# GinZhu/RDST

Hardware: AMD Instinct MI355X
Metric: SR patches/sec fwd+bwd, RDST-E1 x4 64->256 (higher is better)
Workload: dtype bf16; 1 GPU; RDST-E1 x4 (RDST_E1_OASIS_example_SRx4.ini), 1x64x64 LR patches -> 256x256, step = fwd + L1 + bwd + flat-bucket grad all-reduce + Adam; global_batch=32, per_gpu_batch=32, parallelism=dp1, hip_graph=True, grad_bucket_bytes=17859844

## Files before the change

rdst_amd/_lib.py:

```python
from __future__ import annotations

import ctypes as C
import os
import re

_HERE = os.path.dirname(os.path.abspath(__file__))
LIB_PATH = os.environ.get("RDST_HIP_LIB") or os.path.join(_HERE, "librdst_hip.so")
_INCLUDE = os.path.join(os.path.dirname(_HERE), "include")
HEADER_PATH = os.path.join(_INCLUDE, "rdst_hip.h")
_SIDE_HEADERS = {"DATA": os.path.join(_INCLUDE, "rdst_hip_data.h"),
                 "LRC": os.path.join(_INCLUDE, "rdst_hip_consistency.h"),
                 "MSSSIM": os.path.join(_INCLUDE, "rdst_hip_msssim.h"),
                 "NOISE": os.path.join(_INCLUDE, "rdst_hip_noise.h")}

_SCALARS = {"int": C.c_int, "int64_t": C.c_int64, "float": C.c_float, "double": C.c_double, "size_t": C.c_size_t}
_FIELD_SCALARS = {**_SCALARS, "int32_t": C.c_int32}
_RETURNS = {"int": C.c_int, "size_t": C.c_size_t, "const char*": C.c_char_p}
_POINTEES = {*_FIELD_SCALARS, "void", "char", "uint8_t", "unsigned long long"}


def _ctype(text, scalars, structs, where):
    ty = re.sub(r"\s*\*", "*", " ".join(text.split()))
    if ty == "int*":
        return C.POINTER(C.c_int)
    if ty.endswith("*") and ty[:-1].removeprefix("const ") in _POINTEES | set(structs):
        return C.c_void_p
    if ty in scalars or ty in structs:
        return scalars.get(ty) or structs[ty]
    raise RuntimeError(f"rdst_amd: include/rdst_hip.h: type '{ty}' is not in the binding's type map, in: {where}")


def _struct(name, body, structs):
    fields = []
    for stmt in filter(None, (" ".join(s.split()) for s in body.split(";"))):
        first, *more = (d.strip() for d in stmt.split(","))
        m = re.fullmatch(r"(.+?)\s*\b(\w+)\s*(?:\[\s*(\d+)\s*\])?", first)
        rest = [re.fullmatch(r"()(\w+)\s*(?:\[\s*(\d+)\s*\])?", d) for d in more]
        if m is None or None in rest or (more and "*" in m[1]):
            raise RuntimeError(f"rdst_amd: include/rdst_hip.h: cannot read the field '{stmt}' of struct {name}")
        base = _ctype(m[1], _FIELD_SCALARS, structs, f"struct {name} {{ {stmt}; }}")
        fields += [(d[2], base * int(d[3]) if d[3] else base) for d in (m, *rest)]
    return type(name, (C.Structure,), {"_fields_": fields})


def parse_header(text):
    text = re.sub(r"/\*.*?\*/|//[^\n]*", " ", text, flags=re.S)
    constants, lines = {}, []
    for line in text.splitlines():
        if not line.lstrip().startswith("#"):
            lines.append(line)
        elif m := re.fullmatch(r"\s*#\s*define\s+RDST_(\w+)\s+(\d+|\(\s*-\s*\d+\s*\))\s*", line):
            constants[m[1]] = int(re.sub(r"[()\s]", "", m[2]))
    body = re.sub(r'extern\s+"C"\s*\{(.*)\}', r"\1", "\n".join(lines), flags=re.S)
    structs = {}

    def cut(m):
        structs[m[2]] = _struct(m[2], m[1], structs)
        return ""
    body = re.sub(r"typedef\s+struct\s*\w*\s*\{(.*?)\}\s*(\w+)\s*;", cut, body, flags=re.S)
    signatures, params = {}, {}
    for decl in filter(None, (" ".join(d.split()) for d in body.split(";"))):
        m = re.fullmatch(r"(.+?)\s*\b(\w+)\s*\((.*)\)", decl)
        if m is None:
            raise RuntimeError(f"rdst_amd: include/rdst_hip.h: not a function declaration: {decl}")
        ret = re.sub(r"\s*\*", "*", m[1])
        if ret not in _RETURNS:
            raise RuntimeError(f"rdst_amd: include/rdst_hip.h: return type '{ret}' is not in the binding's type map, in: {decl}")
        args = [] if m[3].strip() in ("", "void") else [re.fullmatch(r"(.+?)\s*\b(\w+)", a.strip()) for a in m[3].split(",")]
        if None in args:
            raise RuntimeError(f"rdst_amd: include/rdst_hip.h: a parameter without a name, in: {decl}")
        signatures[m[2]] = (_RETURNS[ret], [_ctype(a[1], _SCALARS, structs, decl) for a in args])
        params[m[2]] = tuple(a[2] for a in args)
    return signatures, params, structs, constants


def _read_header(path=None):
    path = path or HEADER_PATH
    if not os.path.exists(path):
        raise RuntimeError(f"rdst_amd: {path} is missing. The ctypes binding is derived from it "
                           "(it ships beside the package, as in the repository); there is no second copy.")
    with open(path) as f:
        return f.read()


SIGNATURES, PARAMS, _structs, CONSTANTS = parse_header(_read_header())

_BOUND, _side_constants = dict(SIGNATURES), {}
for _prefix, _path in _SIDE_HEADERS.items():
    _sigs, _params, _, _consts = parse_header(_read_header(_path))
    globals().update({_prefix + "_HEADER_PATH": _path, _prefix + "_SIGNATURES": _sigs, _prefix + "_PARAMS": _params})
    _BOUND.update(_sigs)
    _side_constants.update(_consts)
NOISE_HETERO, NOISE_RICIAN = _side_constants["NOISE_HETERO"], _side_constants["NOISE_RICIAN"]

PackJob = _structs["rdst_pack_job"]
LrSchedule = _structs["rdst_lr_schedule"]
# ... 58 lines not shown
```

rdst_amd/build.py:

```python
from __future__ import annotations

import os
import subprocess
import sys
from concurrent.futures import ThreadPoolExecutor

HERE = os.path.dirname(os.path.abspath(__file__))
CSRC = os.path.join(HERE, "csrc")
OBJ = os.path.join(HERE, "csrc", "_obj")
LIB = os.path.join(HERE, "librdst_hip.so")
HIPCC = os.environ.get("HIPCC", "/opt/rocm/bin/hipcc")
FLAGS = ["--offload-arch=gfx950", "-O3", "-std=c++17", "-fPIC", "-Wno-unused-value", "-Wno-unused-result"]



def _newer(src_list, target):
    if not os.path.exists(target):
        return True
    t = os.path.getmtime(target)
    return any(os.path.getmtime(s) > t for s in src_list)


def build(force: bool = False, verbose: bool = True, debug: bool = False) -> str:
    OBJ = os.path.join(HERE, "csrc", "_obj_dbg" if debug else "_obj")
    LIB = os.path.join(HERE, "librdst_hip_dbg.so" if debug else "librdst_hip.so")
    FLAGS = globals()["FLAGS"] + (["-DRDST_DEBUG"] if debug else [])
    os.makedirs(OBJ, exist_ok=True)
    srcs = sorted(f for f in os.listdir(CSRC) if f.endswith(".hip"))
    hdrs = [os.path.join(CSRC, f) for f in os.listdir(CSRC) if f.endswith(".h")]
    hdrs += [os.path.join(os.path.dirname(HERE), "include", h) for h in ("rdst_hip.h", "rdst_hip_data.h", "rdst_hip_consistency.h",
                                                                            "rdst_hip_msssim.h", "rdst_hip_noise.h")]
    jobs = []
    objs = []
    for s in srcs:
        src = os.path.join(CSRC, s)
        obj = os.path.join(OBJ, s[:-4] + ".o")
        objs.append(obj)
        if force or _newer([src] + hdrs, obj):
            jobs.append([HIPCC, *FLAGS, "-c", src, "-o", obj])

    def run(cmd):
        if verbose:
            print("[rdst_amd.build]", " ".join(cmd[-4:]), flush=True)
        r = subprocess.run(cmd, capture_output=True, text=True)
        if r.returncode != 0:
            raise RuntimeError(f"hipcc failed: {' '.join(cmd)}\n{r.stdout}\n{r.stderr}")

    if jobs:
        with ThreadPoolExecutor(max_workers=min(4, len(jobs))) as ex:
            list(ex.map(run, jobs))
    if jobs or force or _newer(objs, LIB):
        run([HIPCC, "--offload-arch=gfx950", "-shared", "-fPIC", "-o", LIB, *objs])
    return LIB


if __name__ == "__main__":
    print(build(force="--force" in sys.argv, debug="--debug" in sys.argv))
```

rdst_amd/csrc/linear.h:

```cpp
#pragma once
#include "common.h"

template <typename T>
int linear_fwd_mfma(const T* X, int64_t ldx, const float* ln_w, const float* ln_b, int in_act, const float* Wt,
                    const float* bias, const T* R, int64_t ldr, T* Y, int64_t ldy, float* stats, int64_t M, int K,
                    int N, float s, bool split, hipStream_t st);
template <typename T>
int linear_dgrad_mfma(const T* X, int64_t ldx, bool has_ln, int in_act, const float* Wt, const T* dY, int64_t lddy,
                      T* dX, int64_t lddx, const T* acc, int64_t ldacc, float* dA, int64_t M, int K, int N, float s,
                      bool split, hipStream_t st);
template <typename T>
int linear_wgrad_mfma(const T* X, int64_t ldx, const float* ln_w, const float* ln_b, const float* stats, int in_act,
                      const T* dY, int64_t lddy, float* dW, float* dbias, const WsSlab& slab, int64_t M, int K, int N, float s,
                      bool split, hipStream_t st);

constexpr int kLinWgradSplits = 96;
inline int linear_wgrad_max_wgs(int N) { return N <= 128 ? 4 * kCUs : N <= 192 ? 2 * kCUs : kCUs; }
struct LinBwdWs {
  float* dA;
  float* G;
  WsSlab slabW;
  WsSlab small;
  size_t bytes;
};
inline LinBwdWs lin_bwd_layout(void* base, int64_t M, int K, int N, bool ln, bool linear) {
  WsCarver c(base);
  LinBwdWs w{};
  const size_t g = (size_t)N * (K + 1), da = ln ? (size_t)M * K : 0;
  w.dA = c.take<float>(da);
  w.G = ln && linear && g <= da ? w.dA : nullptr;
  const int64_t rows = linear ? linear_wgrad_max_wgs(N) : 0;
  const size_t gen = linear ? (size_t)kLinWgradSplits * N * K : 0, per_wg = (size_t)rows * g;
  w.slabW = WsSlab{c.take<float>(gen > per_wg ? gen : per_wg), rows, (int64_t)g};
  w.small = ws_take_slab(c, kSmallBlocks, N > 2 * K ? N : 2 * K);
  c.take<float>(2 * (size_t)K + kWsSlackFloats);
  w.bytes = c.bytes();
  return w;
}

template <typename T>
int linear_dgrad_ln_mfma(const T* X, int64_t ldx, const float* stats, const float* gamma, const float* Wt, const T* dY,
                         int64_t lddy, T* dX, int64_t lddx, const T* acc, int64_t ldacc, const WsSlab& slab, int* nslab,
                         int64_t M, int K, int N, float s, hipStream_t st);
template <typename T>
int linear_wgrad_ln_mfma(const T* X, int64_t ldx, const float* ln_w, const float* ln_b, const float* stats, const float* Wt,
                         const T* dY, int64_t lddy, float* dW, float* dbias, float* dln_w, float* dln_b, const WsSlab& slab,
                         float* G, int64_t M, int K, int N, float s, bool split, hipStream_t st);
template <typename T>
int linear_dgrad_ln2_mfma(const T* X, int64_t ldx, const float* stats, const float* gamma, const float* Wt, const T* dY,
                          int64_t lddy, T* dX, int64_t lddx, const T* acc, int64_t ldacc, int64_t M, int K, int N, float s,
                          bool split, hipStream_t st);
int wgrad_ln_finish_launch(const float* G, const float* Wt, const float* ln_w, const float* ln_b, int N, int K, float s,
                           float* dW, float* dbias, float* dln_w, float* dln_b, hipStream_t st);
int wgrad_sum_launch(const float* slab, int nwg, int tot, float* G, hipStream_t st);
int wgrad_reduce_launch(const float* slab, int nwg, int N, int K, float s, float* dW, float* dbias, hipStream_t st);
int linear_ln_bwd_fused_bf16(const bf16* X, int64_t ldx, const float* ln_w, const float* ln_b, const float* stats,
                             const float* Wt, const bf16* dY, int64_t lddy, bf16* dX, int64_t lddx, const bf16* acc,
                             int64_t ldacc, float* dW, float* dbias, float* dln_w, float* dln_b, const WsSlab& slab, float* G,
                             int64_t M, int K, int N, float s, hipStream_t st, const bf16* acc2 = nullptr, int64_t ldacc2 = 0);
int lnlin3_bwd_bf16(const bf16* X, int64_t ldx, const float* ln_w, const float* stats, const float* Wt, const bf16* dY,
                    int64_t lddy, bf16* dX, int64_t lddx, const bf16* acc, int64_t ldacc, const bf16* acc2, int64_t ldacc2,
                    const WsSlab& slab, int64_t slab_stride, int64_t M, int K, int N, int* grid_out, hipStream_t st);

size_t lin3_pack_bytes(int K, int N);
int lin3_kind(int K, int N, bool ln, bool res, int in_act);
int lin3_fwd_bf16(const bf16* X, int64_t ldx, const float* ln_w, const float* ln_b, int in_act, const float* Wt, const float* bias,
                  const bf16* R, int64_t ldr, bf16* Y, int64_t ldy, float* stats, int64_t M, int K, int N, float s, void* wpack,
                  bool prepacked, hipStream_t st);
int lin3_pack_launch(const float* W, const float* gamma, const float* beta, const float* bias, void* out, int N, int K, float s,
                     hipStream_t st);
size_t mlp3_pack_bytes(int C, int hid);
bool mlp3_fwd_shape(int C, int hid);
int mlp3_fwd_bf16(const bf16* X, int64_t ldx, const float* ln_w, const float* ln_b, const float* W1, const float* b1, const float* W2,
                  const float* b2, bf16* Y, int64_t ldy, float* stats, int64_t M, int C, int hid, void* wpack, bool prepacked,
                  hipStream_t st);

int lin3x_kind(int K, int N, bool ln, bool res, int in_act);
int lin3x_fwd_f32(const float* X, int64_t ldx, const float* ln_w, const float* ln_b, int in_act, const float* Wt, const float* bias,
                  const float* R, int64_t ldr, float* Y, int64_t ldy, float* stats, int64_t M, int K, int N, float s, void* wpack,
                  bool prepacked, hipStream_t st);
int lin3x_pack_launch(const float* W, const float* gamma, const float* beta, const float* bias, void* out, int N, int K, float s,
                      hipStream_t st);
int lnlin3x_bwd_kind(int K, int N, bool ln, int in_act);
int lnlin3x_bwd_f32(const float* X, int64_t ldx, const float* ln_w, const float* ln_b, const float* stats, int in_act, const float* Wt,
                    const float* dY, int64_t lddy, float* dX, int64_t lddx, const float* acc, int64_t ldacc, const float* acc2,
                    int64_t ldacc2, float* dW, float* dbias, float* dln_w, float* dln_b, const WsSlab& slab, float* G, int64_t M, int K, int N,
                    float s, hipStream_t st);
```

rdst_amd/csrc/linear.hip:

```cpp
#include "common.h"
#include "gemm_valu.h"
#include "linear.h"
#include "pack.h"

__global__ void __launch_bounds__(256) slab_reduce_kernel(const float* __restrict__ slab, float* __restrict__ out,
                                                          int S, int64_t n) {
  __shared__ float part[16][17];
  const int o = threadIdx.x & 15, sg = threadIdx.x >> 4;
  const int64_t i = (int64_t)blockIdx.x * 16 + o;
  float a = 0.f;
  if (i < n)
    for (int s = sg; s < S; s += 16) a += slab[(int64_t)s * n + i];
  part[sg][o] = a;
  __syncthreads();
  if (sg == 0 && i < n) {
    float t = 0.f;
#pragma unroll
    for (int k = 0; k < 16; ++k) t += part[k][o];
    out[i] = t;
  }
}

int slab_reduce(const float* slab, float* out, int S, int64_t n, hipStream_t st) {
  if (n <= 0) return 0;
  hipLaunchKernelGGL(slab_reduce_kernel, dim3((unsigned)((n + 15) / 16)), dim3(256), 0, st, slab, out, S, n);
  return rdst_launch_status("slab_reduce");
}

__global__ void __launch_bounds__(256) slab_reduce2_kernel(const float* __restrict__ slab, float* __restrict__ out_a,
                                                           float* __restrict__ out_b, int S, int K) {
  const int lane = threadIdx.x & 63;
  const int i = blockIdx.x * 4 + (threadIdx.x >> 6);
  if (i >= 2 * K) return;
  float a = 0.f;
  for (int s = lane; s < S; s += 64) a += slab[(int64_t)s * 2 * K + i];
  a = wave_sum(a);
  if (lane == 0) {
    if (i < K) { if (out_a) out_a[i] = a; }
    else if (out_b) out_b[i - K] = a;
  }
}

int slab_reduce2(const float* slab, float* out_a, float* out_b, int S, int K, hipStream_t st) {
  if (K <= 0 || (!out_a && !out_b)) return 0;
  hipLaunchKernelGGL(slab_reduce2_kernel, dim3((unsigned)((2 * K + 3) / 4)), dim3(256), 0, st, slab, out_a, out_b, S, K);
  return rdst_launch_status("slab_reduce2");
}

namespace {

constexpr float kLnEps = 1e-5f;

template <typename T>
__global__ void __launch_bounds__(256) row_stats_kernel(const T* __restrict__ X, int64_t ldx, float* __restrict__ stats,
                                                        int64_t M, int K) {
  const int lane = threadIdx.x & 63;
  const int64_t row = (int64_t)blockIdx.x * 4 + (threadIdx.x >> 6);
  if (row >= M) return;
  const T* x = X + row * ldx;
  float s = 0.f;
  for (int k = lane; k < K; k += 64) s += to_f32<T>(x[k]);
  const float mean = wave_sum(s) / (float)K;
  float v = 0.f;
  for (int k = lane; k < K; k += 64) {
    const float d = to_f32<T>(x[k]) - mean;
    v = fmaf(d, d, v);
  }
  const float var = wave_sum(v) / (float)K;
  if (lane == 0) {
    stats[row * 2] = mean;
    stats[row * 2 + 1] = 1.0f / sqrtf(var + kLnEps);
  }
}

template <typename T>
__global__ void __launch_bounds__(256) ln_apply_kernel(const T* __restrict__ X, int64_t ldx, const float* __restrict__ stats,
                                                       const float* __restrict__ g, const float* __restrict__ b,
                                                       const T* R, int64_t ldr, T* Y, int64_t ldy, int64_t M, int K,
                                                       float s) {
  const int64_t i = (int64_t)blockIdx.x * 256 + threadIdx.x;
  if (i >= M * K) return;
  const int64_t m = i / K;
  const int k = (int)(i - m * K);
  float v = (to_f32<T>(X[m * ldx + k]) - stats[2 * m]) * stats[2 * m + 1] * g[k] + b[k];
  v *= s;
  if (R) v += to_f32<T>(R[m * ldr + k]);
// ... 27 lines not shown
}
struct Ln8Lane { int c0, lo; bool on; };
__device__ __forceinline__ Ln8Lane ln8_lane(int grp, int K) {
  Ln8Lane l;
  l.on = 8 * grp < K;
  l.c0 = 8 * grp + 8 <= K ? 8 * grp : K - 8;
  l.lo = 8 * grp - l.c0;
  if (!l.on) { l.c0 = 0; l.lo = 8; }
  return l;
}
__device__ __forceinline__ void ln8_store(float* dst, const float (&o)[8], const Ln8Lane& l) {
  if (!l.on) return;
  if (l.lo == 0) {
    ln8_u32x4 u, v;
    u.x = __float_as_uint(o[0]); u.y = __float_as_uint(o[1]); u.z = __float_as_uint(o[2]); u.w = __float_as_uint(o[3]);
    v.x = __float_as_uint(o[4]); v.y = __float_as_uint(o[5]); v.z = __float_as_uint(o[6]); v.w = __float_as_uint(o[7]);
    *reinterpret_cast<ln8_u32x4*>(dst + l.c0) = u;
    *reinterpret_cast<ln8_u32x4*>(dst + l.c0 + 4) = v;
  } else {
#pragma unroll
    for (int e = 0; e < 8; ++e)
      if (e >= l.lo) dst[l.c0 + e] = o[e];
  }
}
__device__ __forceinline__ void ln8_store(bf16* dst, const float (&o)[8], const Ln8Lane& l) {
  if (!l.on) return;
  if (l.lo == 0) {
    ln8_u32x4 u;
    u.x = ln8_pack2(o[0], o[1]); u.y = ln8_pack2(o[2], o[3]); u.z = ln8_pack2(o[4], o[5]); u.w = ln8_pack2(o[6], o[7]);
    *reinterpret_cast<ln8_u32x4*>(dst + l.c0) = u;
  } else {
#pragma unroll
    for (int e = 0; e < 8; ++e)
      if (e >= l.lo) dst[l.c0 + e] = __float2bfloat16(o[e]);
  }
}

template <typename T>
__global__ void __launch_bounds__(256) ln8_fwd_kernel(const T* __restrict__ X, int64_t ldx, const float* __restrict__ g,
                                                      const float* __restrict__ b, const T* R, int64_t ldr, T* Y, int64_t ldy,
                                                      float* __restrict__ stats, int64_t M, int K, float s) {
  const int lane = threadIdx.x & 63, wave = threadIdx.x >> 6, ps = lane >> 3, grp = lane & 7;
  const Ln8Lane l = ln8_lane(grp, K);
  float gm[8], bt[8];
#pragma unroll
  for (int e = 0; e < 8; ++e) { gm[e] = g[l.c0 + e]; bt[e] = b[l.c0 + e]; }
  const float invK = 1.0f / (float)K;
  for (int64_t r0 = ((int64_t)blockIdx.x * 4 + wave) * 8; r0 < M; r0 += (int64_t)gridDim.x * 32) {
    const int64_t row = r0 + ps < M ? r0 + ps : M - 1;
    const bool valid = r0 + ps < M;
    float f[8];
    ln8_load<T>(X + row * ldx + l.c0, f);
    float sum = 0.f;
#pragma unroll
    for (int e = 0; e < 8; ++e) sum += (l.on && e >= l.lo) ? f[e] : 0.f;
    const float mean = ln8_sum8(sum) * invK;
    float sq = 0.f;
#pragma unroll
    for (int e = 0; e < 8; ++e) {
      f[e] -= mean;
      sq = (l.on && e >= l.lo) ? fmaf(f[e], f[e], sq) : sq;
    }
    const float rstd = 1.0f / sqrtf(ln8_sum8(sq) * invK + kLnEps);
    float o[8];
#pragma unroll
    for (int e = 0; e < 8; ++e) o[e] = (f[e] * rstd * gm[e] + bt[e]) * s;
    if (R) {
      float rr[8];
      ln8_load<T>(R + row * ldr + l.c0, rr);
#pragma unroll
      for (int e = 0; e < 8; ++e) o[e] += rr[e];
    }
    if (valid) {
      ln8_store(Y + row * ldy, o, l);
      if (grp == 0) *reinterpret_cast<float2*>(stats + 2 * row) = make_float2(mean, rstd);
    }
  }
}

template <typename T>
__global__ void __launch_bounds__(256) ln8_bwd_kernel(const T* __restrict__ dY, int64_t lddy, const T* __restrict__ X, int64_t ldx,
                                                      const float* __restrict__ stats, const float* __restrict__ gamma, T* dX,
                                                      int64_t lddx, const T* acc, int64_t ldacc, float* __restrict__ slab, int64_t M,
                                                      int K, float s) {
  __shared__ float red[4][2][64];
  const int lane = threadIdx.x & 63, wave = threadIdx.x >> 6, ps = lane >> 3, grp = lane & 7;
  const Ln8Lane l = ln8_lane(grp, K);
  float gm[8], dg[8], db[8];
#pragma unroll
  for (int e = 0; e < 8; ++e) { gm[e] = gamma[l.c0 + e]; dg[e] = 0.f; db[e] = 0.f; }
  const float invK = 1.0f / (float)K;
  for (int64_t r0 = ((int64_t)blockIdx.x * 4 + wave) * 8; r0 < M; r0 += (int64_t)gridDim.x * 32) {
    const int64_t row = r0 + ps < M ? r0 + ps : M - 1;
    const bool valid = r0 + ps < M;
    const float2 st = *reinterpret_cast<const float2*>(stats + 2 * row);
    float da[8], xh[8], gg[8];
    ln8_load<T>(dY + row * lddy + l.c0, da);
    ln8_load<T>(X + row * ldx + l.c0, xh);
    float s1 = 0.f, s2 = 0.f;
#pragma unroll
    for (int e = 0; e < 8; ++e) {
      const bool mine = l.on && e >= l.lo && valid;
      da[e] = mine ? da[e] * s : 0.f;
      xh[e] = (xh[e] - st.x) * st.y;
      gg[e] = da[e] * gm[e];
      s1 += gg[e];
      s2 = fmaf(gg[e], xh[e], s2);
      dg[e] = fmaf(da[e], xh[e], dg[e]);
      db[e] += da[e];
    }
    s1 = ln8_sum8(s1) * invK;
    s2 = ln8_sum8(s2) * invK;
    if (dX && valid) {
      float o[8];
#pragma unroll
      for (int e = 0; e < 8; ++e) o[e] = st.y * (gg[e] - s1 - xh[e] * s2);
      if (acc) {
        float a[8];
        ln8_load<T>(acc + row * ldacc + l.c0, a);
#pragma unroll
        for (int e = 0; e < 8; ++e) o[e] += a[e];
      }
      ln8_store(dX + row * lddx, o, l);
    }
  }
#pragma unroll
  for (int e = 0; e < 8; ++e) {
    dg[e] += __shfl_xor(dg[e], 8, 64); dg[e] += __shfl_xor(dg[e], 16, 64); dg[e] += __shfl_xor(dg[e], 32, 64);
    db[e] += __shfl_xor(db[e], 8, 64); db[e] += __shfl_xor(db[e], 16, 64); db[e] += __shfl_xor(db[e], 32, 64);
  }
  if (ps == 0 && l.on)
#pragma unroll
    for (int e = 0; e < 8; ++e)
      if (e >= l.lo) { red[wave][0][l.c0 + e] = dg[e]; red[wave][1][l.c0 + e] = db[e]; }
  __syncthreads();
  for (int i = threadIdx.x; i < 2 * K; i += 256) {
    const int which = i / K, k = i - which * K;
    slab[(int64_t)blockIdx.x * 2 * K + i] = red[0][which][k] + red[1][which][k] + red[2][which][k] + red[3][which][k];
  }
}
static inline bool ln8_ok(const void* a, int64_t lda, const void* b, int64_t ldb, const void* c, int64_t ldc, int K, int elt = 2) {
  auto al = [elt](const void* q, int64_t l) { return ((uintptr_t)q & 3) == 0 && (elt == 4 || (l & 1) == 0); };
  return K >= 8 && K <= 64 && (K & 1) == 0 && al(a, lda) && al(b, ldb) && al(c, ldc);
}

template <typename T>
struct LinIn {
  static constexpr bool kFast = true;
  const T* X; int64_t ldx; const float* stats; const float* g; const float* b; int act;
  __device__ __forceinline__ float operator()(int64_t m, int64_t k) const {
    float v = to_f32<T>(X[m * ldx + k]);
    if (g) return (v - stats[2 * m]) * stats[2 * m + 1] * g[k] + b[k];
    return apply_act(v, act);
  }
};
template <typename T>
struct LinInT {
  static constexpr bool kFast = false;
  LinIn<T> f;
  __device__ __forceinline__ float operator()(int64_t m, int k) const { return f(m, k); }
};
struct WtB {
  static constexpr bool kFast = true;
  const float* Wt; int K;
  __device__ __forceinline__ float operator()(int64_t k, int n) const { return Wt[(int64_t)n * K + k]; }
};
struct WtBT {
  static constexpr bool kFast = false;
  const float* Wt; int K;
  __device__ __forceinline__ float operator()(int64_t n_idx, int k_idx) const { return Wt[n_idx * K + k_idx]; }
};
template <typename T>
struct DyA {
  static constexpr bool kFast = true;
  const T* dY; int64_t ld; float s;
  __device__ __forceinline__ float operator()(int64_t m, int64_t n) const { return to_f32<T>(dY[m * ld + n]) * s; }
};
template <typename T>
struct DyAT {
  static constexpr bool kFast = false;
  const T* dY; int64_t ld; float s;
  __device__ __forceinline__ float operator()(int64_t n, int64_t m) const { return to_f32<T>(dY[m * ld + n]) * s; }
};
template <typename T>
struct DyCol {
  const T* dY; int64_t ld; float s;
  __device__ __forceinline__ float operator()(int64_t m, int n) const { return to_f32<T>(dY[m * ld + n]) * s; }
};

template <typename T>
struct FwdEp {
  const float* bias; const T* R; int64_t ldr; T* Y; int64_t ldy; float s;
  __device__ __forceinline__ void operator()(int64_t m, int n, float acc, int) const {
    float v = acc + (bias ? bias[n] : 0.f);
    v *= s;
    if (R) v += to_f32<T>(R[m * ldr + n]);
    Y[m * ldy + n] = from_f32<T>(v);
  }
};
struct SlabEp {
  float* slab; int64_t n_total; int cols;
  __device__ __forceinline__ void operator()(int64_t r, int c, float acc, int z) const {
    slab[(int64_t)z * n_total + r * cols + c] = acc;
  }
// ... 32 lines not shown
  const float invK = 1.0f / (float)K;
  for (int64_t row = (int64_t)blockIdx.x * 4 + wave; row < M; row += (int64_t)gridDim.x * 4) {
    const float mean = stats[2 * row], rstd = stats[2 * row + 1];
    float xh[KC], g[KC];
    float s1 = 0.f, s2 = 0.f;
#pragma unroll
    for (int c = 0; c < KC; ++c) {
      const int k = lane + 64 * c;
      if (k < K) {
        const float da = dA[row * K + k];
        xh[c] = (to_f32<T>(X[row * ldx + k]) - mean) * rstd;
        g[c] = da * gm[c];
        s1 += g[c];
        s2 = fmaf(g[c], xh[c], s2);
        dg[c] = fmaf(da, xh[c], dg[c]);
        db[c] += da;
      } else {
        xh[c] = 0.f;
        g[c] = 0.f;
      }
    }
    s1 = wave_sum(s1) * invK;
    s2 = wave_sum(s2) * invK;
#pragma unroll
    for (int c = 0; c < KC; ++c) {
      const int k = lane + 64 * c;
      if (k < K) {
        float v = rstd * (g[c] - s1 - xh[c] * s2);
        if (dX) {
          if (acc) v += to_f32<T>(acc[row * ldacc + k]);
          dX[row * lddx + k] = from_f32<T>(v);
        }
      }
    }
  }
#pragma unroll
  for (int c = 0; c < KC; ++c) {
    red[wave][0][lane + 64 * c] = dg[c];
    red[wave][1][lane + 64 * c] = db[c];
  }
  __syncthreads();
  for (int i = threadIdx.x; i < 2 * K; i += 256) {
    const int which = i / K, k = i - which * K;
    const float a = red[0][which][k] + red[1][which][k] + red[2][which][k] + red[3][which][k];
    slab[(int64_t)blockIdx.x * 2 * K + i] = a;
  }
}

template <typename T>
int fwd_t(const T* X, int64_t ldx, const float* ln_w, const float* ln_b, int in_act, const float* Wt, const float* bias,
          const T* R, int64_t ldr, T* Y, int64_t ldy, float* stats, int64_t M, int K, int N, float s, bool split, hipStream_t st) {
  auto run_stats = [&]() -> int {
    hipLaunchKernelGGL((row_stats_kernel<T>), dim3((unsigned)((M + 3) / 4)), dim3(256), 0, st, X, ldx, stats, M, K);
    return rdst_launch_status("row_stats");
  };
  if (!Wt) {
    if (ln8_ok(X, ldx, Y, ldy, R, ldr, K, (int)sizeof(T))) {
      const int64_t nb = (M + 31) / 32;
      hipLaunchKernelGGL((ln8_fwd_kernel<T>), dim3((unsigned)(nb < 2048 ? nb : 2048)), dim3(256), 0, st, X, ldx, ln_w, ln_b, R, ldr, Y, ldy,
                         stats, M, K, s);
      return rdst_launch_status("ln8_fwd");
    }
    if (int rc = run_stats()) return rc;
    const int64_t n = M * K;
    hipLaunchKernelGGL((ln_apply_kernel<T>), dim3((unsigned)((n + 255) / 256)), dim3(256), 0, st, X, ldx, stats, ln_w,
                       ln_b, R, ldr, Y, ldy, M, K, s);
    return rdst_launch_status("ln_apply");
  }
  if (int rc = linear_fwd_mfma<T>(X, ldx, ln_w, ln_b, in_act, Wt, bias, R, ldr, Y, ldy, stats, M, K, N, s, split, st);
      rc != RDST_ENOTSUP)
    return rc;
  if (ln_w)
    if (int rc = run_stats()) return rc;
  LinIn<T> la{X, ldx, stats, ln_w, ln_b, in_act};
  WtB lb{Wt, K};
  FwdEp<T> ep{bias, R, ldr, Y, ldy, s};
  return gemm_valu_launch(la, lb, ep, M, N, K, 1, st, "linear_fwd");
}

template <typename T>
int bwd_t(const T* X, int64_t ldx, const float* ln_w, const float* ln_b, const float* stats, int in_act, const float* Wt,
          const T* dY, int64_t lddy, T* dX, int64_t lddx, const T* acc, int64_t ldacc, float* dW, float* dbias,
          float* dln_w,
          float* dln_b, float* wsp, int64_t M, int K, int N, float s, bool split, hipStream_t st, const T* acc2, int64_t ldacc2) {
  const LinBwdWs w = lin_bwd_layout(wsp, M, K, N, ln_w != nullptr, true);
  float* const dA = w.dA;
  const WsSlab& slabW = w.slabW;
  const WsSlab& small = w.small;
  if constexpr (sizeof(T) == 4) {
    if (split && Wt && dX && dW && dbias && (!ln_w || (dln_w && dln_b && w.G)) && !rdst_dbg_getenv("RDST_LBX_OFF")) {
      const int rc = lnlin3x_bwd_f32(X, ldx, ln_w, ln_b, stats, in_act, Wt, dY, lddy, dX, lddx, acc, ldacc, acc2, ldacc2, dW, dbias, dln_w,
                                     dln_b, slabW, w.G, M, K, N, s, st);
      if (rc != RDST_ENOTSUP) return rc;
    }
  }
  if (acc2) {
    if constexpr (sizeof(T) == 2) {
      if (Wt && ln_w && ln_b && dW && dbias && dln_w && dln_b && dX && K <= 128 && w.G)
        return linear_ln_bwd_fused_bf16(X, ldx, ln_w, ln_b, stats, Wt, dY, lddy, dX, lddx, acc, ldacc, dW, dbias, dln_w, dln_b, slabW,
                                        w.G, M, K, N, s, st, acc2, ldacc2);
    }
    return RDST_ENOTSUP;
  }
  LinIn<T> fin{X, ldx, stats, ln_w, ln_b, in_act};
  if (Wt) {
    if (ln_w && ln_b && dW && dbias && dln_w && dln_b && dX && K <= 128 && !rdst_dbg_getenv("RDST_LN_BWD_V1")) {
      if (float* G = w.G) {
        if constexpr (sizeof(T) == 2) {
          const int rcf = linear_ln_bwd_fused_bf16(X, ldx, ln_w, ln_b, stats, Wt, dY, lddy, dX, lddx, acc, ldacc, dW, dbias, dln_w,
                                                   dln_b, slabW, G, M, K, N, s, st);
          if (rcf != RDST_ENOTSUP) return rcf;
        }
        int rc = linear_wgrad_ln_mfma<T>(X, ldx, ln_w, ln_b, stats, Wt, dY, lddy, dW, dbias, dln_w, dln_b, slabW, G, M, K, N,
                                         s, split, st);
        if (rc == 0) {
          rc = linear_dgrad_ln2_mfma<T>(X, ldx, stats, ln_w, Wt, dY, lddy, dX, lddx, acc, ldacc, M, K, N, s, split, st);
          if (rc == 0) return 0;
          if (rc != RDST_ENOTSUP) return rc;
          if (N >= 64) {
            const int N1 = (N / 2 + 3) / 4 * 4;
            rc = linear_dgrad_ln2_mfma<T>(X, ldx, stats, ln_w, Wt, dY, lddy, dX, lddx, acc, ldacc, M, K, N1, s, split, st);
            if (rc == 0) {
              rc = linear_dgrad_ln2_mfma<T>(X, ldx, stats, ln_w, Wt + (int64_t)N1 * K, dY + N1, lddy, dX, lddx, dX, lddx, M, K, N - N1, s, split, st);
              if (rc != RDST_ENOTSUP) return rc;
            } else if (rc != RDST_ENOTSUP) {
              return rc;
            }
          }
          dW = nullptr; dbias = nullptr; dln_w = nullptr; dln_b = nullptr;
        } else if (rc != RDST_ENOTSUP) {
          return rc;
        }
      }
    }
    if constexpr (sizeof(T) == 2) {
      if (!ln_w && !in_act && dW && dbias && dX) {
        const int rcf = linear_ln_bwd_fused_bf16(X, ldx, nullptr, nullptr, nullptr, Wt, dY, lddy, dX, lddx, acc, ldacc, dW, dbias,
                                                 nullptr, nullptr, slabW, nullptr, M, K, N, s, st);
        if (rcf != RDST_ENOTSUP) return rcf;
      }
    }
    bool wgrad_done = false;
    if (dW || dbias) {
      const int rc = linear_wgrad_mfma<T>(X, ldx, ln_w, ln_b, stats, in_act, dY, lddy, dW, dbias, slabW, M, K, N, s, split, st);
      if (rc == 0) wgrad_done = true;
      else if (rc != RDST_ENOTSUP) return rc;
    }
    if (!wgrad_done && dbias) {
      DyCol<T> f{dY, lddy, s};
      if (int rc = colsum_launch(f, M, N, small, dbias, st, "linear_dbias")) return rc;
    }
    if (!wgrad_done && dW) {
      DyAT<T> la{dY, lddy, s};
      LinInT<T> lb{fin};
      SlabEp ep{slabW.p, (int64_t)N * K, K};
      const int z = gemm_valu_splits(M, kLinWgradSplits);
      if (int rc2 = rdst_slab_fits(slabW, z, (int64_t)N * K, "linear_wgrad")) return rc2;
      if (int rc2 = gemm_valu_launch(la, lb, ep, N, K, M, kLinWgradSplits, st, "linear_wgrad")) return rc2;
      if (int rc2 = slab_reduce(slabW.p, dW, z, (int64_t)N * K, st)) return rc2;
    }
    if (dX && ln_w) {
      int nslab = 0;
      const int rc = linear_dgrad_ln_mfma<T>(X, ldx, stats, ln_w, Wt, dY, lddy, dX, lddx, acc, ldacc, small, &nslab, M, K,
                                             N, s, st);
      if (rc == 0) {
        return slab_reduce2(small.p, dln_w, dln_b, nslab, K, st);
      }
      if (rc != RDST_ENOTSUP) return rc;
    }
    if (dX || (ln_w && (dln_w || dln_b))) {
      int rc = linear_dgrad_mfma<T>(X, ldx, ln_w != nullptr, in_act, Wt, dY, lddy, dX, lddx, acc, ldacc, dA, M, K, N, s, split, st);
      if (rc == RDST_ENOTSUP) {
        DyA<T> la{dY, lddy, s};
        WtBT lb{Wt, K};
        if (ln_w) {
          DaEp ep{dA, K};
          rc = gemm_valu_launch(la, lb, ep, M, K, N, 1, st, "linear_dgrad");
        } else {
          DxEp<T> ep{X, ldx, dX, lddx, in_act, acc, ldacc};
          rc = gemm_valu_launch(la, lb, ep, M, K, N, 1, st, "linear_dgrad");
        }
      }
      if (rc) return rc;
    }
  }
  if (ln_w) {
    const float* dAsrc = dA;
    if (!dX && !dln_w && !dln_b) return 0;
    if (K > 512) return rdst_fail(RDST_ENOTSUP, "rdst_ln_linear_bwd: LayerNorm width %d > 512", K);
    const int blocks = (int)small.cap((M + 3) / 4 < kSmallBlocks ? (M + 3) / 4 : kSmallBlocks, 2 * K);
    if (int rc = rdst_slab_fits(small, blocks, 2 * K, "ln_bwd_rows")) return rc;
    const int kc = (K + 63) / 64;
#define RDST_LNB(KC)                                                                                              \
  hipLaunchKernelGGL((ln_bwd_rows_kernel<T, KC>), dim3(blocks), dim3(256), 0, st, dAsrc, X, ldx, stats, ln_w, dX, \
                     lddx, acc, ldacc, small.p, M, K)
    if (kc <= 1) RDST_LNB(1); else if (kc <= 2) RDST_LNB(2); else if (kc <= 4) RDST_LNB(4); else RDST_LNB(8);
#undef RDST_LNB
    if (int rc = rdst_launch_status("ln_bwd_rows")) return rc;
    if (int rc = slab_reduce2(small.p, dln_w, dln_b, blocks, K, st)) return rc;
  }
  return 0;
}

template <typename T>
__global__ void __launch_bounds__(256) scale_to_f32_kernel(const T* __restrict__ dY, int64_t ld, float* __restrict__ dA,
                                                           int64_t M, int K, float s) {
  const int64_t i = (int64_t)blockIdx.x * 256 + threadIdx.x;
  if (i >= M * K) return;
  const int64_t m = i / K;
  dA[i] = to_f32<T>(dY[m * ld + (i - m * K)]) * s;
}

template <typename T>
int ln_only_bwd(const T* X, int64_t ldx, const float* ln_w, const float* stats, const T* dY, int64_t lddy, T* dX,
                int64_t lddx, const T* acc, int64_t ldacc, float* dln_w, float* dln_b, float* wsp, int64_t M, int K, float s,
                hipStream_t st) {
  const LinBwdWs w = lin_bwd_layout(wsp, M, K, K, true, false);
  float* const dA = w.dA;
  const WsSlab& small = w.small;
  const int64_t n = M * K;
  if (K <= 64 && ln8_ok(X, ldx, dY, lddy, dX, lddx, K, (int)sizeof(T)) && ln8_ok(acc, ldacc, nullptr, 0, nullptr, 0, K, (int)sizeof(T))) {
    const int64_t nb = (M + 31) / 32;
    const int blocks = (int)small.cap(nb < kSmallBlocks ? nb : kSmallBlocks, 2 * K);
    if (int rc = rdst_slab_fits(small, blocks, 2 * K, "ln8_bwd")) return rc;
    hipLaunchKernelGGL((ln8_bwd_kernel<T>), dim3(blocks), dim3(256), 0, st, dY, lddy, X, ldx, stats, ln_w, dX, lddx, acc, ldacc, small.p, M, K, s);
    if (int rc = rdst_launch_status("ln8_bwd")) return rc;
    return slab_reduce2(small.p, dln_w, dln_b, blocks, K, st);
  }
  hipLaunchKernelGGL((scale_to_f32_kernel<T>), dim3((unsigned)((n + 255) / 256)), dim3(256), 0, st, dY, lddy, dA, M, K, s);
  if (int rc = rdst_launch_status("scale_to_f32")) return rc;
  if (K > 512) return rdst_fail(RDST_ENOTSUP, "rdst_ln_linear_bwd: LayerNorm width %d > 512", K);
  const int blocks = (int)small.cap((M + 3) / 4 < kSmallBlocks ? (M + 3) / 4 : kSmallBlocks, 2 * K);
  if (int rc = rdst_slab_fits(small, blocks, 2 * K, "ln_bwd_rows")) return rc;
  const int kc = (K + 63) / 64;
#define RDST_LNB(KC)                                                                                           \
  hipLaunchKernelGGL((ln_bwd_rows_kernel<T, KC>), dim3(blocks), dim3(256), 0, st, dA, X, ldx, stats, ln_w, dX, \
                     lddx, acc, ldacc, small.p, M, K)
  if (kc <= 1) RDST_LNB(1); else if (kc <= 2) RDST_LNB(2); else if (kc <= 4) RDST_LNB(4); else RDST_LNB(8);
#undef RDST_LNB
  if (int rc = rdst_launch_status("ln_bwd_rows")) return rc;
  return slab_reduce2(small.p, dln_w, dln_b, blocks, K, st);
}

}

extern "C" int rdst_ln_linear_fwd_packable(int K, int N, int has_ln, int has_residual, int in_act, int dtype) {
  bool split;
  if (rdst_dtype(dtype, split, "rdst_ln_linear_fwd_packable")) return 0;
  if (split) return lin3x_kind(K, N, has_ln != 0, has_residual != 0, in_act) != 0;
  return dtype == RDST_BF16 && lin3_kind(K, N, has_ln != 0, has_residual != 0, in_act) != 0;
}

extern "C" size_t rdst_ln_linear_fwd_workspace(int K, int N) {
  if (K <= 0 || N <= 0) return 16;
  return lin3_pack_bytes(K, N);
}

extern "C" size_t rdst_ln_linear_fwd_workspace2(int K, int N, int dtype) {
  if (K <= 0 || N <= 0) return 16;
  return dtype == RDST_F32X3 ? lin3x_pack_bytes(K, N) : lin3_pack_bytes(K, N);
}

extern "C" int rdst_ln_linear_fwd(const void* X, int64_t ld_x, const float* ln_w, const float* ln_b, int in_act,
                                  const float* Wt, const float* bias, const void* R, int64_t ld_r, void* Y, int64_t ld_y,
                                  float* stats, void* workspace, size_t workspace_bytes, int64_t M, int K, int N,
                                  float out_scale, int dtype, void* stream) {
  bool split;
  if (int rc = rdst_dtype(dtype, split, "rdst_ln_linear_fwd")) return rc;
  if (!X || !Y) return rdst_fail(RDST_EINVAL, "rdst_ln_linear_fwd: null pointer");
  if (M < 0 || K <= 0 || N <= 0) return rdst_fail(RDST_EINVAL, "rdst_ln_linear_fwd: bad dimensions");
  if ((ln_w == nullptr) != (ln_b == nullptr)) return rdst_fail(RDST_EINVAL, "rdst_ln_linear_fwd: ln_w/ln_b must come together");
  if (ln_w && !stats) return rdst_fail(RDST_EINVAL, "rdst_ln_linear_fwd: LayerNorm needs a stats buffer");
  if (ln_w && in_act) return rdst_fail(RDST_EINVAL, "rdst_ln_linear_fwd: LayerNorm and in_act are exclusive");
  if (!Wt && (!ln_w || N != K)) return rdst_fail(RDST_EINVAL, "rdst_ln_linear_fwd: Wt == NULL means LayerNorm only (N == K)");
  if (ld_x < K || ld_y < N || (R && ld_r < N)) return rdst_fail(RDST_EINVAL, "rdst_ln_linear_fwd: leading dimension too small");
  if (M == 0) return 0;
  hipStream_t st = (hipStream_t)stream;
  if (dtype == RDST_BF16 && workspace && workspace_bytes >= rdst_ln_linear_fwd_workspace(K, N)) {
    const int rc = lin3_fwd_bf16((const bf16*)X, ld_x, ln_w, ln_b, in_act, Wt, bias, (const bf16*)R, ld_r, (bf16*)Y, ld_y, stats, M,
                                 K, N, out_scale, workspace, workspace_bytes == RDST_PREPACKED, st);
    if (rc != RDST_ENOTSUP) return rc;
  }
  if (split && workspace && workspace_bytes >= lin3x_pack_bytes(K, N)) {
    const int rc = lin3x_fwd_f32((const float*)X, ld_x, ln_w, ln_b, in_act, Wt, bias, (const float*)R, ld_r, (float*)Y, ld_y, stats, M,
                                 K, N, out_scale, workspace, workspace_bytes == RDST_PREPACKED, st);
    if (rc != RDST_ENOTSUP) return rc;
  }
  if (dtype == RDST_F32)
    return fwd_t<float>((const float*)X, ld_x, ln_w, ln_b, in_act, Wt, bias, (const float*)R, ld_r, (float*)Y, ld_y, stats, M, K, N, out_scale, split, st);
  return fwd_t<bf16>((const bf16*)X, ld_x, ln_w, ln_b, in_act, Wt, bias, (const bf16*)R, ld_r, (bf16*)Y, ld_y, stats, M, K, N, out_scale, false, st);
}

extern "C" size_t rdst_ln_linear_bwd_workspace(int64_t M, int K, int N) {
  if (M <= 0 || K <= 0 || N <= 0) return 0;
  return lin_bwd_layout(nullptr, M, K, N, true, true).bytes;
}

namespace {
int ln_linear_bwd(const void* X, int64_t ld_x, const float* ln_w, const float* ln_b, const float* stats, int in_act, const float* Wt,
                  const void* dY, int64_t ld_dy, void* dX, int64_t ld_dx, const void* dX_add, int64_t ld_dx_add, float* dW, float* dbias,
                  float* dln_w, float* dln_b, void* workspace, size_t workspace_bytes, int64_t M, int K, int N, float out_scale,
                  int dtype, bool split, hipStream_t st, const void* dX_add2, int64_t ld_dx_add2) {
  if (!X || !dY || !workspace) return rdst_fail(RDST_EINVAL, "rdst_ln_linear_bwd: null pointer");
  if (M < 0 || K <= 0 || N <= 0) return rdst_fail(RDST_EINVAL, "rdst_ln_linear_bwd: bad dimensions");
  if (ln_w && !stats) return rdst_fail(RDST_EINVAL, "rdst_ln_linear_bwd: LayerNorm needs the forward's stats");
  if (!Wt && (!ln_w || N != K)) return rdst_fail(RDST_EINVAL, "rdst_ln_linear_bwd: Wt == NULL means LayerNorm only (N == K)");
  if (ld_x < K || ld_dy < N || (dX && ld_dx < K)) return rdst_fail(RDST_EINVAL, "rdst_ln_linear_bwd: leading dimension too small");
  if (workspace_bytes < rdst_ln_linear_bwd_workspace(M, K, N)) return rdst_fail(RDST_EINVAL, "rdst_ln_linear_bwd: workspace too small");
  if (M == 0) return 0;
  float* wsp = (float*)workspace;
  if (dX_add2 && (!Wt || (dtype != RDST_BF16 && !(split && lnlin3x_bwd_kind(K, N, ln_w != nullptr, in_act))))) return RDST_ENOTSUP;
  if (!Wt) {
    if (dtype == RDST_F32)
      return ln_only_bwd<float>((const float*)X, ld_x, ln_w, stats, (const float*)dY, ld_dy, (float*)dX, ld_dx, (const float*)dX_add, ld_dx_add, dln_w, dln_b, wsp, M, K, out_scale, st);
    return ln_only_bwd<bf16>((const bf16*)X, ld_x, ln_w, stats, (const bf16*)dY, ld_dy, (bf16*)dX, ld_dx, (const bf16*)dX_add, ld_dx_add, dln_w, dln_b, wsp, M, K, out_scale, st);
  }
  if (dtype == RDST_F32)
    return bwd_t<float>((const float*)X, ld_x, ln_w, ln_b, stats, in_act, Wt, (const float*)dY, ld_dy, (float*)dX, ld_dx, (const float*)dX_add, ld_dx_add, dW, dbias, dln_w, dln_b, wsp, M, K, N, out_scale, split, st,
                      (const float*)dX_add2, ld_dx_add2);
  return bwd_t<bf16>((const bf16*)X, ld_x, ln_w, ln_b, stats, in_act, Wt, (const bf16*)dY, ld_dy, (bf16*)dX, ld_dx, (const bf16*)dX_add, ld_dx_add, dW, dbias, dln_w, dln_b, wsp, M, K, N, out_scale, false, st,
                     (const bf16*)dX_add2, ld_dx_add2);
}
}

extern "C" int rdst_ln_linear_bwd2(const void* X, int64_t ld_x, const float* ln_w, const float* ln_b, const float* stats,
                                  int in_act, const float* Wt, const void* dY, int64_t ld_dy, void* dX, int64_t ld_dx,
                                  const void* dX_add, int64_t ld_dx_add, float* dW, float* dbias, float* dln_w, float* dln_b,
                                  void* workspace,
                                  size_t workspace_bytes, int64_t M, int K, int N, float out_scale, int dtype,
                                  void* stream, const void* dX_add2, int64_t ld_dx_add2) {
  bool split;
  if (int rc = rdst_dtype(dtype, split, "rdst_ln_linear_bwd")) return rc;
  return ln_linear_bwd(X, ld_x, ln_w, ln_b, stats, in_act, Wt, dY, ld_dy, dX, ld_dx, dX_add, ld_dx_add, dW, dbias, dln_w, dln_b, workspace,
                       workspace_bytes, M, K, N, out_scale, dtype, split, (hipStream_t)stream, dX_add2, ld_dx_add2);
}

extern "C" int rdst_ln_linear_bwd(const void* X, int64_t ld_x, const float* ln_w, const float* ln_b, const float* stats,
                                  int in_act, const float* Wt, const void* dY, int64_t ld_dy, void* dX, int64_t ld_dx,
                                  const void* dX_add, int64_t ld_dx_add, float* dW, float* dbias, float* dln_w, float* dln_b,
                                  void* workspace, size_t workspace_bytes, int64_t M, int K, int N, float out_scale, int dtype,
                                  void* stream) {
  bool split;
  if (int rc = rdst_dtype(dtype, split, "rdst_ln_linear_bwd")) return rc;
  return ln_linear_bwd(X, ld_x, ln_w, ln_b, stats, in_act, Wt, dY, ld_dy, dX, ld_dx, dX_add, ld_dx_add, dW, dbias, dln_w, dln_b, workspace,
                       workspace_bytes, M, K, N, out_scale, dtype, split, (hipStream_t)stream, nullptr, 0);
}
```

rdst_amd/csrc/lnlin3_mfma.hip:

```cpp
#include "linear.h"
#include "lds_dma.h"
#include "mfma.h"
#include "wattn_hd.h"
#include <stdlib.h>

#ifndef LB3_LOADW_SHAPE
#define LB3_LOADW_SHAPE(K, N) (((K) == 60 && (N) == 180) || ((K) == 90 && (N) == 270) || ((K) == 120 && (N) == 120))
#endif
#ifndef LB3_ABL
#define LB3_ABL 0
#endif

#ifdef LB3_STAMPS
constexpr bool LB3_TICKS = true;
#else
constexpr bool LB3_TICKS = false;
#endif
constexpr const char* LB3_LEGEND = "stash fetch barrier compute finish - - -";

namespace {
using namespace wahd;
using MM = Mma<bf16>;

struct LB3Args {
  const bf16* X; int64_t ldx; const float* stats; const float* lnw; const float* W;
  const bf16* dY; int64_t lddy; bf16* dX; int64_t lddx; const bf16* Acc; int64_t ldacc;
  const bf16* Acc2; int64_t ldacc2;
  float* slab; int64_t slab_stride;
  int64_t M; int64_t ntiles; int tiles_per_wg;
};

template <int K_, int N_>
struct LB3 {
  static constexpr int K = K_, N = N_;
  static constexpr int NCT = (K + 1 + 31) / 32, NW = (N + 31) / 32, KN = (N + 15) / 16;
  static constexpr bool WIDE = N >= 180;
  static constexpr int TN = WIDE ? 3 : 1;
  static constexpr int TC = (K == 120 && N == 360) ? 2 : WIDE ? 1 : NCT;
  static_assert(NW % TN == 0 && NCT % TC == 0, "blocking");
  static constexpr int NGN = NW / TN, NGC = NCT / TC, NWG = NGN * NGC;
  static constexpr int NDG = NCT;
  static constexpr int NWV = NWG + NDG, NT = 64 * NWV;
  static constexpr int PKX = (K * 2 + 15) / 16, PKY = (N * 2 + 15) / 16;
  static constexpr int NY = 32 * PKY, NX = 32 * PKX;
  static constexpr bool LOADW = LB3_LOADW_SHAPE(K_, N_);
  static constexpr bool SPLITR = WIDE || LOADW;
  static constexpr int NTW = SPLITR ? 64 * NWG : NT, NTD = SPLITR ? 64 * NDG : NT;
  static constexpr int cdiv(int a, int b) { return (a + b - 1) / b; }
  static constexpr bool ACC_BY_W = K == 120 && N == 360;
  static constexpr int W_SY = cdiv(NY, NTW), W_SX = cdiv(NX, NTW), W_SA = (WIDE && !ACC_BY_W && !LOADW) ? 0 : cdiv(NX, NTW);
  static constexpr int D_SY = SPLITR ? 0 : W_SY, D_SX = SPLITR ? 0 : W_SX, D_SA = (ACC_BY_W || LOADW) ? 0 : cdiv(NX, NTD);
  static constexpr int CP = 32 * NCT;
  static constexpr int LDX = NCT == 4 ? 336 : CP * 2 + 16;
  static constexpr int LDY = lds_plane_stride(32 * NW);
  static constexpr int OFF_AC = 32 * LDX, OFF_DY = 64 * LDX, OFF_SM = OFF_DY + 32 * LDY, BUF = OFF_SM + 128;
  static constexpr int OFF_RED = 2 * BUF;
  static constexpr int SMEM = OFF_RED + 2 * NCT * 256;
  static constexpr int PERCU0 = 12 / NWV < 1 ? 1 : 12 / NWV;
  static constexpr int PERCU1 = WIDE ? 1 : PERCU0 > 2 ? 2 : PERCU0;
  static constexpr int PERCU = PERCU1 * SMEM > 160 * 1024 ? 1 : PERCU1;
  static constexpr int WPS = (NWV * PERCU + 3) / 4;
};

template <class CF, bool LN, int SY, int SX, int SA>
struct LB3Loader {
  static constexpr int NS = SY + SX + SA;
  int meta[NS > 0 ? NS : 1];
  u32x4_a4 rd[NS > 0 ? NS : 1];
  u32x4_a4 rd2[SA > 0 ? SA : 1];
  float2 rst[SX > 0 ? SX : 1];
  static __device__ __forceinline__ int kind(int u) { return u < SY ? 0 : u < SY + SX ? 1 : 2; }
  __device__ __forceinline__ void setup(int tid_r, int ntr, bool has_acc) {
#pragma unroll
    for (int u = 0; u < NS; ++u) {
      const int kd = kind(u);
      const int idx = tid_r + ntr * (kd == 0 ? u : kd == 1 ? u - SY : u - SY - SX);
      const int per = kd == 0 ? CF::PKY : CF::PKX, rowbytes = kd == 0 ? CF::N * 2 : CF::K * 2;
      const bool on = idx < 32 * per && (kd != 2 || has_acc);
      const int row = on ? idx / per : 0, chk = on ? idx - row * per : 0;
      int o = chk * 16;
      if (o + 16 > rowbytes) o = rowbytes - 16;
      meta[u] = o | (row << 16) | ((on ? 1 : 0) << 24) | (((o & 15) == 0 ? 1 : 0) << 28);
    }
  }
  __device__ __forceinline__ void fetch(const LB3Args& p, int64_t tile) {
    const uint32_t Mu = (uint32_t)p.M;
#pragma unroll
    for (int u = 0; u < NS; ++u) {
      const int kd = kind(u);
      uint32_t row = (uint32_t)(tile * 32) + (uint32_t)((meta[u] >> 16) & 31);
      row = row < Mu ? row : Mu - 1;
      const char* base = reinterpret_cast<const char*>(kd == 0 ? p.dY : kd == 1 ? p.X : (p.Acc ? p.Acc : p.X));
      const uint32_t ldb = (uint32_t)((kd == 0 ? p.lddy : kd == 1 ? p.ldx : p.ldacc) * 2);
      rd[u] = *reinterpret_cast<const u32x4_a4*>(base + (size_t)(row * ldb + (uint32_t)(meta[u] & 0xffff)));
      if (kd == 2 && p.Acc2)
        rd2[u - SY - SX] = *reinterpret_cast<const u32x4_a4*>(reinterpret_cast<const char*>(p.Acc2) +
                                                              (size_t)(row * (uint32_t)(p.ldacc2 * 2) + (uint32_t)(meta[u] & 0xffff)));
      if (LN && kd == 1) rst[u - SY] = *reinterpret_cast<const float2*>(p.stats + 2 * (size_t)row);
    }
  }
  __device__ __forceinline__ void stash(const LB3Args& p, int64_t tile, char* buf) {
    const uint32_t Mu = (uint32_t)p.M;
#pragma unroll
    for (int u = 0; u < NS; ++u) {
      const int kd = kind(u);
      if (!((meta[u] >> 24) & 1)) continue;
      const int mrow = (meta[u] >> 16) & 31;
      const bool valid = (uint32_t)(tile * 32) + (uint32_t)mrow < Mu;
      Pack16 v;
      v.w[0] = valid ? rd[u].x : 0u; v.w[1] = valid ? rd[u].y : 0u; v.w[2] = valid ? rd[u].z : 0u; v.w[3] = valid ? rd[u].w : 0u;
      if (kd == 2 && p.Acc2) {
        const u32x4_a4 a = rd[u], b2 = rd2[u - SY - SX];
        const bool h1 = p.Acc != nullptr;
        float f[8];
        f[0] = bf16lo(b2.x) + (h1 ? bf16lo(a.x) : 0.f); f[1] = bf16hi(b2.x) + (h1 ? bf16hi(a.x) : 0.f);
        f[2] = bf16lo(b2.y) + (h1 ? bf16lo(a.y) : 0.f); f[3] = bf16hi(b2.y) + (h1 ? bf16hi(a.y) : 0.f);
        f[4] = bf16lo(b2.z) + (h1 ? bf16lo(a.z) : 0.f); f[5] = bf16hi(b2.z) + (h1 ? bf16hi(a.z) : 0.f);
        f[6] = bf16lo(b2.w) + (h1 ? bf16lo(a.w) : 0.f); f[7] = bf16hi(b2.w) + (h1 ? bf16hi(a.w) : 0.f);
#pragma unroll
        for (int e = 0; e < 8; ++e) f[e] = valid ? f[e] : 0.f;
        v = MM::pack(f);
      }
      if (LN && kd == 1) {
        const float2 st2 = rst[u - SY];
        float f[8];
        f[0] = bf16lo(rd[u].x); f[1] = bf16hi(rd[u].x); f[2] = bf16lo(rd[u].y); f[3] = bf16hi(rd[u].y);
        f[4] = bf16lo(rd[u].z); f[5] = bf16hi(rd[u].z); f[6] = bf16lo(rd[u].w); f[7] = bf16hi(rd[u].w);
#pragma unroll
        for (int e = 0; e < 8; ++e) f[e] = valid ? (f[e] - st2.x) * st2.y : 0.f;
        v = MM::pack(f);
        if ((meta[u] & 0xffff) == 0) reinterpret_cast<float*>(buf + CF::OFF_SM)[mrow] = st2.y;
      }
      int mt = meta[u];
      asm volatile("" : "+v"(mt));
      const int lrow = (mt >> 16) & 31, lo = mt & 0xffff;
      char* dst = buf + (kd == 0 ? CF::OFF_DY + lrow * CF::LDY : (kd == 2 ? CF::OFF_AC : 0) + lrow * CF::LDX) + lo;
      if ((meta[u] >> 28) & 1) *reinterpret_cast<Pack16*>(dst) = v;
      else {
        uint32_t* d = reinterpret_cast<uint32_t*>(dst);
        d[0] = v.w[0]; d[1] = v.w[1]; d[2] = v.w[2]; d[3] = v.w[3];
      }
    }
  }
};

template <int K, int N, bool LN>
__global__ void __launch_bounds__((LB3<K, N>::NT), (LB3<K, N>::WPS)) lnlin3_bwd_kernel(const LB3Args p) {
  extern __shared__ __attribute__((aligned(16))) char smem[];
  using CF = LB3<K, N>;
  constexpr int NCT = CF::NCT, NW = CF::NW, KN = CF::KN, TN = CF::TN, TC = CF::TC, NGC = CF::NGC, NWG = CF::NWG, NT = CF::NT;
  constexpr int LDX = CF::LDX, LDY = CF::LDY;
  const int tid = threadIdx.x, lane = tid & 63, wave = __builtin_amdgcn_readfirstlane(tid >> 6), r = lane & 31, hh = lane >> 5;
  const bool has_acc = p.Acc != nullptr || p.Acc2 != nullptr;

  if (!(LB3_ABL & 16)) lds_zero16(smem, CF::SMEM, tid, NT);
  __syncthreads();
  if (tid < 64) *reinterpret_cast<uint16_t*>(smem + (tid >> 5) * CF::BUF + (tid & 31) * LDX + K * 2) = 0x3f80;

  const int q = (lane & 15) >> 2, pp = lane & 3, gq1 = (lane >> 4) & 1;
  const int trc = (16 * gq1 + 4 * pp) * 2;
  const int tro_y = CF::OFF_DY + (8 * hh + q) * LDY + trc;
  const int tro_x = (8 * hh + q) * LDX + trc;

  const bool is_wg = wave < NWG;
  const int gn = wave / NGC, gc = wave - gn * NGC;
  const int dct = wave - NWG;

  const int64_t t0 = (int64_t)blockIdx.x * p.tiles_per_wg;
  const int64_t t1 = t0 + p.tiles_per_wg < p.ntiles ? t0 + p.tiles_per_wg : p.ntiles;
  __syncthreads();

  if (is_wg) {
    LB3Loader<CF, LN, CF::W_SY, CF::W_SX, CF::W_SA> ld;
    ld.setup(tid, CF::NTW, has_acc);
    if (t0 < t1) ld.fetch(p, t0);
    f32x16 G[TN][TC];
#pragma unroll
    for (int i = 0; i < TN; ++i)
#pragma unroll
      for (int j = 0; j < TC; ++j)
#pragma unroll
        for (int v = 0; v < 16; ++v) G[i][j][v] = 0.f;
    int b = 0;
    WaveTicks<LB3_TICKS> wt;
    for (int64_t tile = t0; tile < t1; ++tile, b ^= 1) {
      char* buf = smem + b * CF::BUF;
      ld.stash(p, tile, buf);
      wt.add(0);
      ld.fetch(p, tile + 1 < t1 ? tile + 1 : tile);
      wt.add(1);
      __syncthreads();
      wt.add(2);
#pragma unroll
      for (int s = 0; s < 2; ++s) {
        Pack16 ya[TN], xb[TC];
#pragma unroll
        for (int i = 0; i < TN; ++i) {
          const lds_cp yp = (lds_cp)(buf + tro_y + 16 * s * LDY) + (gn * TN + i) * 64;
          ya[i] = lds_tr_pack(yp, yp + 4 * LDY);
        }
#pragma unroll
        for (int j = 0; j < TC; ++j) {
          const lds_cp xp = (lds_cp)(buf + tro_x + 16 * s * LDX) + (gc * TC + j) * 64;
          xb[j] = lds_tr_pack(xp, xp + 4 * LDX);
        }
#pragma unroll
        for (int i = 0; i < TN; ++i)
#pragma unroll
          for (int j = 0; j < TC; ++j) {
#if !(LB3_ABL & 1)
            MM::mma(G[i][j], ya[i], xb[j]);
#else
            G[i][j][0] += __uint_as_float(ya[i].w[0] ^ xb[j].w[0]);
#endif
          }
      }
      wt.add(3);
    }
    wt.print(wave, lane, "wgrad", LB3_LEGEND);
    if (LN) __syncthreads();
    uint2* my = reinterpret_cast<uint2*>(p.slab) + (int64_t)blockIdx.x * p.slab_stride;
#pragma unroll
    for (int i = 0; i < TN; ++i)
#pragma unroll
      for (int j = 0; j < TC; ++j) {
        const int c = 32 * (gc * TC + j) + r;
#pragma unroll
        for (int g4 = 0; g4 < 4; ++g4) {
          const int n0 = 32 * (gn * TN + i) + 8 * g4 + 4 * hh;
          if (n0 < N && c <= K && !(LB3_ABL & 8))
            my[(int64_t)(n0 >> 2) * (K + 1) + c] =
                make_uint2(pack_bf16x2(G[i][j][4 * g4], G[i][j][4 * g4 + 1]), pack_bf16x2(G[i][j][4 * g4 + 2], G[i][j][4 * g4 + 3]));
        }
      }
    return;
  }

  LB3Loader<CF, LN, CF::D_SY, CF::D_SX, CF::D_SA> ld;
  ld.setup(CF::SPLITR ? tid - 64 * NWG : tid, CF::NTD, has_acc);
  if (t0 < t1) ld.fetch(p, t0);
  Pack16 wf[KN];
  {
    const int c = 32 * dct + r;
    const int cc = c < K ? c : K - 1;
    const float gm = (c < K) ? (LN ? p.lnw[cc] : 1.0f) : 0.f;
#pragma unroll
    for (int ks = 0; ks < KN; ++ks) {
      float f[8];
#pragma unroll
      for (int e = 0; e < 8; ++e) {
        const int n = 16 * ks + 8 * hh + e;
#if LB3_ABL & 4
        const float w = 0.01f * (float)(n + cc);
#else
        const float w = p.W[(size_t)(n < N ? n : N - 1) * K + cc];
#endif
        f[e] = n < N ? w * gm : 0.f;
      }
      wf[ks] = MM::pack(f);
    }
  }
  constexpr float invK = 1.0f / (float)K;
  float* red = reinterpret_cast<float*>(smem + CF::OFF_RED);
  f32x16 dx;
  u32x2_t xs[4], as[4];
  float rstd = 0.f;
  int64_t prow = -1;
  auto finish = [&](int pb) {
    float s1 = 0.f, s2 = 0.f;
    if (LN) {
#pragma unroll
      for (int w = 0; w < NCT; ++w) {
        const float2 v = *reinterpret_cast<const float2*>(red + ((pb * NCT + w) * 32 + r) * 2);
        s1 += v.x; s2 += v.y;
      }
      s1 *= invK; s2 *= invK;
    }
    float o[16];
#pragma unroll
    for (int g4 = 0; g4 < 4; ++g4) {
      const float xh[4] = {bf16lo(xs[g4].x), bf16hi(xs[g4].x), bf16lo(xs[g4].y), bf16hi(xs[g4].y)};
      const float ac[4] = {bf16lo(as[g4].x), bf16hi(as[g4].x), bf16lo(as[g4].y), bf16hi(as[g4].y)};
#pragma unroll
      for (int e = 0; e < 4; ++e) o[4 * g4 + e] = LN ? fmaf(rstd, dx[4 * g4 + e] - s1 - xh[e] * s2, ac[e]) : dx[4 * g4 + e] + ac[e];
    }
    if (prow < p.M) {
      bf16* drow = p.dX + prow * p.lddx;
#pragma unroll
      for (int gp2 = 0; gp2 < 2; ++gp2) {
        float c8[8];
#pragma unroll
        for (int e = 0; e < 4; ++e) {
          const auto sw = __builtin_amdgcn_permlane32_swap(__float_as_uint(o[8 * gp2 + e]), __float_as_uint(o[8 * gp2 + 4 + e]), false, false);
          c8[e] = __uint_as_float(sw[0]);
          c8[4 + e] = __uint_as_float(sw[1]);
        }
        const int cb = 32 * dct + 8 * (2 * gp2 + hh);
        if (cb + 8 <= K) {
          u32x4_a4 u;
          u.x = pack_bf16x2(c8[0], c8[1]); u.y = pack_bf16x2(c8[2], c8[3]);
          u.z = pack_bf16x2(c8[4], c8[5]); u.w = pack_bf16x2(c8[6], c8[7]);
          *reinterpret_cast<u32x4_a4*>(drow + cb) = u;
        } else {
#pragma unroll
          for (int e = 0; e < 8; ++e)
            if (cb + e < K) drow[cb + e] = __float2bfloat16(c8[e]);
        }
      }
    }
  };
  int b = 0;
  WaveTicks<LB3_TICKS> wt;
  for (int64_t tile = t0; tile < t1; ++tile, b ^= 1) {
    char* buf = smem + b * CF::BUF;
    ld.stash(p, tile, buf);
    wt.add(0);
    ld.fetch(p, tile + 1 < t1 ? tile + 1 : tile);
    wt.add(1);
    __syncthreads();
    wt.add(2);
    if (LN && prow >= 0) finish(b ^ 1);
    wt.add(4);
    const lds_cp yrow = (lds_cp)(buf + CF::OFF_DY + r * LDY + hh * 16);
#pragma unroll
    for (int v = 0; v < 16; ++v) dx[v] = 0.f;
    if constexpr (KN > 12) {
#pragma unroll
      for (int ks = 0; ks < KN; ++ks) {
#if !(LB3_ABL & 2)
        MM::mma(dx, wf[ks], lds_pack(yrow + 32 * ks));
#else
        dx[0] += __uint_as_float(lds_pack(yrow + 32 * ks).w[0]);
#endif
      }
    } else {
      f32x16 d2;
#pragma unroll
      for (int v = 0; v < 16; ++v) d2[v] = 0.f;
#pragma unroll
      for (int ks = 0; ks < KN; ++ks) {
        const Pack16 yb = lds_pack(yrow + 32 * ks);
        if (ks & 1) MM::mma(d2, wf[ks], yb);
        else MM::mma(dx, wf[ks], yb);
      }
#pragma unroll
      for (int v = 0; v < 16; ++v) dx[v] += d2[v];
    }
    const lds_cp xrow = (lds_cp)(buf + r * LDX) + (32 * dct + 4 * hh) * 2;
#pragma unroll
    for (int g4 = 0; g4 < 4; ++g4) {
      xs[g4] = *reinterpret_cast<const LDS_AS u32x2_t*>(xrow + 16 * g4);
      as[g4] = *reinterpret_cast<const LDS_AS u32x2_t*>(xrow + CF::OFF_AC + 16 * g4);
    }
    prow = tile * 32 + r;
    if (LN) {
      rstd = reinterpret_cast<const float*>(buf + CF::OFF_SM)[r];
      float s1 = 0.f, s2 = 0.f;
#pragma unroll
      for (int g4 = 0; g4 < 4; ++g4) {
        const float xh[4] = {bf16lo(xs[g4].x), bf16hi(xs[g4].x), bf16lo(xs[g4].y), bf16hi(xs[g4].y)};
#pragma unroll
        for (int e = 0; e < 4; ++e) {
          s1 += dx[4 * g4 + e];
          s2 = fmaf(dx[4 * g4 + e], xh[e], s2);
        }
      }
      s1 = half_swap_sum(s1);
      s2 = half_swap_sum(s2);
      if (hh == 0) *reinterpret_cast<float2*>(red + ((b * NCT + dct) * 32 + r) * 2) = make_float2(s1, s2);
    } else {
      wt.add(3);
      finish(b);
      wt.add(4);
    }
    wt.add(3);
  }
  wt.print(wave, lane, "dgrad", LB3_LEGEND);
  if (LN) {
    __syncthreads();
    if (prow >= 0) finish(b ^ 1);
  }
}

template <int K, int N, bool LN>
int lb3_launch(LB3Args& p, const WsSlab& slab, int* grid_out, hipStream_t st) {
  using CF = LB3<K, N>;
  auto kern = lnlin3_bwd_kernel<K, N, LN>;
  static int percu_env = -1;
  if (percu_env < 0) { const char* e = rdst_dbg_getenv("RDST_LB3_PERCU"); percu_env = e ? atoi(e) : 0; }
  int per_cu = CF::PERCU;
  if (percu_env > 0 && percu_env < per_cu) per_cu = percu_env;
  const int64_t grid = rdst_tile_grid(p.ntiles, slab.cap((int64_t)kCUs * per_cu, 2 * p.slab_stride), &p.tiles_per_wg);
  if (int rc = rdst_slab_fits(slab, grid, 2 * p.slab_stride, "lnlin3_bwd")) return rc;
  *grid_out = (int)grid;
  return rdst_launch(kern, dim3((unsigned)grid), dim3(CF::NT), CF::SMEM, st, "lnlin3_bwd", p);
}

}

int lnlin3_bwd_bf16(const bf16* X, int64_t ldx, const float* ln_w, const float* stats, const float* Wt, const bf16* dY,
                    int64_t lddy, bf16* dX, int64_t lddx, const bf16* acc, int64_t ldacc, const bf16* acc2, int64_t ldacc2,
                    const WsSlab& slab, int64_t slab_stride, int64_t M, int K, int N, int* grid_out, hipStream_t st) {
  static int off = -1;
  if (off < 0) { const char* e = rdst_dbg_getenv("RDST_LB3_OFF"); off = e ? atoi(e) : 0; }
  if (off) return RDST_ENOTSUP;
  const bool ln = ln_w != nullptr;
  LB3Args p{};
  p.X = X; p.ldx = ldx; p.stats = stats; p.lnw = ln_w; p.W = Wt; p.dY = dY; p.lddy = lddy; p.dX = dX; p.lddx = lddx;
  p.Acc = acc; p.ldacc = ldacc; p.Acc2 = acc2; p.ldacc2 = ldacc2; p.slab = slab.p; p.slab_stride = slab_stride; p.M = M;
  p.ntiles = (M + 31) / 32;
#define RDST_LB3(KK, NN, LL) if (K == KK && N == NN && ln == LL) return lb3_launch<KK, NN, LL>(p, slab, grid_out, st);
  RDST_LB3(60, 180, true) RDST_LB3(90, 270, true) RDST_LB3(120, 360, true)
  RDST_LB3(60, 30, true) RDST_LB3(90, 30, true) RDST_LB3(120, 30, true)
  RDST_LB3(60, 60, false) RDST_LB3(90, 90, false) RDST_LB3(120, 120, false)
#undef RDST_LB3
  return RDST_ENOTSUP;
}
```

rdst_amd/csrc/lnlin_mfma.hip:

```cpp
#include "linear.h"
#include "mfma.h"
#include "reduce_batch.h"
#include "wattn_hd.h"
#include <stdlib.h>

namespace {
using namespace wahd;
using MM = Mma<bf16>;

typedef __attribute__((address_space(1))) const char* gcp;
__device__ __forceinline__ u32x4_a4 gload16(gcp q) {
  const u32x4_a4 v = *reinterpret_cast<__attribute__((address_space(1))) const u32x4_a4*>(q);
  return v;
}
__device__ __forceinline__ float2 gload8(gcp q) {
  const float x = *reinterpret_cast<__attribute__((address_space(1))) const float*>(q);
  const float y = *reinterpret_cast<__attribute__((address_space(1))) const float*>(q + 4);
  return make_float2(x, y);
}

__host__ __device__ inline int lnlin_ldy(int NP) {
  const int b = NP * 2 + 16;
  return (b & 255) < 48 ? b + 64 : b;
}
// ... 236 lines not shown
      float s1 = 0.f, s2 = 0.f;
      if (LN) {
#pragma unroll
      for (int w = 0; w < NCT; ++w) {
        const float2 v = *reinterpret_cast<const float2*>(red + (w * 32 + r) * 2);
        s1 += v.x; s2 += v.y;
      }
      s1 *= invK; s2 *= invK;
      }
      float o[16];
#pragma unroll
      for (int g4 = 0; g4 < 4; ++g4) {
        const int cb = (32 * wave + 8 * g4 + 4 * hh) * 2;
        const u32x2_t xv = *reinterpret_cast<const LDS_AS u32x2_t*>((lds_cp)(smem + OFF_XH + r * LDX) + cb);
        const u32x2_t av = *reinterpret_cast<const LDS_AS u32x2_t*>((lds_cp)(smem + OFF_AC + r * LDX) + cb);
        const float xh[4] = {bf16lo(xv.x), bf16hi(xv.x), bf16lo(xv.y), bf16hi(xv.y)};
        const float ac[4] = {bf16lo(av.x), bf16hi(av.x), bf16lo(av.y), bf16hi(av.y)};
#pragma unroll
        for (int e = 0; e < 4; ++e) o[4 * g4 + e] = LN ? fmaf(rstd, dx[4 * g4 + e] - s1 - xh[e] * s2, ac[e]) : dx[4 * g4 + e] + ac[e];
      }
      const int64_t row = tile * 32 + r;
      if (row < p.M) {
        bf16* drow = p.dX + row * p.lddx;
#pragma unroll
        for (int gp2 = 0; gp2 < 2; ++gp2) {
          float c8[8];
#pragma unroll
          for (int e = 0; e < 4; ++e) {
            const auto sw = __builtin_amdgcn_permlane32_swap(__float_as_uint(o[8 * gp2 + e]), __float_as_uint(o[8 * gp2 + 4 + e]), false, false);
            c8[e] = __uint_as_float(sw[0]);
            c8[4 + e] = __uint_as_float(sw[1]);
          }
          const int cb = 32 * wave + 8 * (2 * gp2 + hh);
          if (cb + 8 <= K) {
            u32x4_a4 u;
            u.x = pack_bf16x2(c8[0], c8[1]); u.y = pack_bf16x2(c8[2], c8[3]);
            u.z = pack_bf16x2(c8[4], c8[5]); u.w = pack_bf16x2(c8[6], c8[7]);
            *reinterpret_cast<u32x4_a4*>(drow + cb) = u;
          } else {
#pragma unroll
            for (int e = 0; e < 8; ++e)
              if (cb + e < K) drow[cb + e] = __float2bfloat16(c8[e]);
          }
        }
      }
    }
    __syncthreads();
    stamp();
  }
  if (RDST_DBGV(p.stamps) && tid == 0) p.stamps[(size_t)blockIdx.x * 16 + 14] = __builtin_readcyclecounter();
  uint2* my = reinterpret_cast<uint2*>(p.slab) + (int64_t)blockIdx.x * p.slab_stride;
  if (wave < NW)
#pragma unroll
  for (int ct = 0; ct < NCT; ++ct) {
    const int c = 32 * ct + r;
#pragma unroll
    for (int g4 = 0; g4 < 4; ++g4) {
      const int n0 = 32 * wave + 8 * g4 + 4 * hh;
      if (n0 < N && c <= K)
        my[(int64_t)(n0 >> 2) * (K + 1) + c] = make_uint2(pack_bf16x2(G[ct][4 * g4], G[ct][4 * g4 + 1]), pack_bf16x2(G[ct][4 * g4 + 2], G[ct][4 * g4 + 3]));
    }
  }
  if (RDST_DBGV(p.stamps) && tid == 0) p.stamps[(size_t)blockIdx.x * 16 + 15] = __builtin_readcyclecounter();
}
}

static int lnlin_bwd_reduce(float* slab, int grid, int64_t slab_stride, bool ln, const float* Wt, const float* ln_w,
                            const float* ln_b, float* dW, float* dbias, float* dln_w, float* dln_b, float* G, int N, int K,
                            hipStream_t st) {
  rbatch::SumJob sj{};
  sj.slab = slab; sj.nwg = grid; sj.stride = slab_stride; sj.g4 = 1; sj.a2 = N; sj.b2 = K + 1; sj.tot = ((N + 3) / 4) * (K + 1);
  if (!ln) {
    sj.map = rbatch::MAP_LINEAR; sj.out = dW; sj.out2 = dbias; sj.a = K; sj.b = K + 1; sj.s = 1.0f;
    return rbatch::sum(sj, st);
  }
  sj.map = rbatch::MAP_COPY; sj.out = G;
  if (int rc = rbatch::sum(sj, st)) return rc;
  return wgrad_ln_finish_launch(G, Wt, ln_w, ln_b, N, K, 1.0f, dW, dbias, dln_w, dln_b, st);
}

int linear_ln_bwd_fused_bf16(const bf16* X, int64_t ldx, const float* ln_w, const float* ln_b, const float* stats,
                             const float* Wt, const bf16* dY, int64_t lddy, bf16* dX, int64_t lddx, const bf16* acc,
                             int64_t ldacc, float* dW, float* dbias, float* dln_w, float* dln_b, const WsSlab& slab, float* G,
                             int64_t M, int K, int N, float s, hipStream_t st, const bf16* acc2, int64_t ldacc2) {
  static int off = -1;
  if (off < 0) { const char* e = rdst_dbg_getenv("RDST_LNLIN_V1"); off = e ? atoi(e) : 0; }
  const bool ln = ln_w != nullptr;
  if (off == 1 || (off == 2 && !ln) || s != 1.0f || M <= 0) return RDST_ENOTSUP;
  const int nct = (K + 1 + 31) / 32;
  if (nct < 2 || nct > 4 || (K & 1) || K < 8 || (N & 1) || N < 8) return RDST_ENOTSUP;
  const int NW = (N + 31) / 32;
  if (NW > 12) return RDST_ENOTSUP;
  const int PK = 4 * nct, PKY = (N * 2 + 15) / 16;
  int NWV = NW > nct ? NW : nct;
  if (ln && NWV < 2 * nct) NWV = 2 * nct;
  const int NT = 64 * NWV;
  if (4 * NT < 32 * (PKY + PK * (acc ? 2 : 1))) return RDST_ENOTSUP;
  if (ln && (NT < 32 * PK || 2 * NT < 32 * PKY)) return RDST_ENOTSUP;
  if (((uintptr_t)X & 3) || ((uintptr_t)dY & 3) || ((uintptr_t)dX & 3) || ((uintptr_t)acc & 3) || (ldx & 1) || (lddy & 1) ||
      (lddx & 1) || (ldacc & 1))
    return RDST_ENOTSUP;
  if ((uint64_t)M * (uint64_t)(lddy > ldx ? (lddy > ldacc ? lddy : ldacc) : (ldx > ldacc ? ldx : ldacc)) * 2 >= (1ull << 31)) return RDST_ENOTSUP;
  const int64_t slab_stride = (int64_t)((N + 3) / 4) * (K + 1);
  {
    int g3 = 0;
    if (acc2 && (((uintptr_t)acc2 & 3) || (ldacc2 & 1) || (uint64_t)M * (uint64_t)ldacc2 * 2 >= (1ull << 31))) return RDST_ENOTSUP;
    const int rc3 = lnlin3_bwd_bf16(X, ldx, ln_w, stats, Wt, dY, lddy, dX, lddx, acc, ldacc, acc2, ldacc2, slab, slab_stride, M, K,
                                    N, &g3, st);
    if (rc3 == 0) return lnlin_bwd_reduce(slab.p, g3, slab_stride, ln, Wt, ln_w, ln_b, dW, dbias, dln_w, dln_b, G, N, K, st);
    if (rc3 != RDST_ENOTSUP || acc2) return rc3;
  }
  const int CP = 32 * nct, LDW = nct == 4 ? 288 : CP * 2 + 16, LDX = nct == 4 ? 336 : CP * 2 + 16, NP = 32 * NW, LDY = lnlin_ldy(NP);
  const int smem = NP * LDW + 2 * 32 * LDX + 32 * LDY + 128 + nct * 32 * 8;
  if (smem > 160 * 1024) return RDST_ENOTSUP;
  LnLinArgs p{};
  p.X = X; p.ldx = ldx; p.stats = stats; p.lnw = ln_w; p.W = Wt; p.dY = dY; p.lddy = lddy; p.dX = dX; p.lddx = lddx;
  p.Acc = acc; p.ldacc = ldacc; p.M = M; p.K = K; p.N = N; p.NW = NW; p.NWV = NWV;
  p.ntiles = (M + 31) / 32;
  int per_cu = ln ? 1 : 12 / NWV;
  if (per_cu > 160 * 1024 / smem) per_cu = 160 * 1024 / smem;
  if (per_cu < 1) per_cu = 1;
  if (per_cu > 2) per_cu = 2;
  { const char* e = rdst_dbg_getenv("RDST_LNLIN_PERCU"); if (e && atoi(e) > 0) per_cu = atoi(e); }
  p.slab = slab.p;
  p.slab_stride = slab_stride;
  const int64_t grid = rdst_tile_grid(p.ntiles, slab.cap((int64_t)kCUs * per_cu, 2 * slab_stride), &p.tiles_per_wg);
  if (int rc = rdst_slab_fits(slab, grid, 2 * slab_stride, "lnlin_bwd")) return rc;
  int rc = 0;
#define RDST_LNLIN(NC)                                                                                               \
  {                                                                                                                  \
    auto kern = ln ? lnlin_bwd_kernel<NC, true> : lnlin_bwd_kernel<NC, false>;                                       \
    rc = rdst_launch(kern, dim3((unsigned)grid), dim3(NT), smem, st, "lnlin_bwd", p);                                 \
  }
  p.stamps = rdst_stamps_begin("RDST_LNLIN_STAMPS", grid, 16, st);
  if (nct == 2) RDST_LNLIN(2) else if (nct == 3) RDST_LNLIN(3) else RDST_LNLIN(4)
#undef RDST_LNLIN
  rdst_stamps_end(p.stamps, grid, 16, RDST_STAMPS_TICKS, st, "lnlin_bwd K=%d N=%d ln=%d", K, N, (int)ln);
  if (rc) return rc;
  return lnlin_bwd_reduce(slab.p, (int)grid, p.slab_stride, ln, Wt, ln_w, ln_b, dW, dbias, dln_w, dln_b, G, N, K, st);
}
```

rdst_amd/networks/common.py:

```python
from __future__ import annotations

import math

import torch
from torch import nn

from .. import ops


class Conv2d(nn.Conv2d):

    def forward_rows(self, x, *, in_act=ops.ACT_NONE, residual=None, out_scale=1.0, shuffle=1, out_slot=None):
        k = self.kernel_size[0]
        if (self.kernel_size[0] != self.kernel_size[1] or k not in (1, 3) or self.stride != (1, 1)
                or self.padding != (k // 2, k // 2) or self.dilation != (1, 1) or self.groups != 1):
            raise NotImplementedError("rdst_amd Conv2d: only k in {1,3}, stride 1, padding k//2, groups 1")
        return ops.conv_rows(x, self.weight, self.bias, in_act=in_act, residual=residual, out_scale=out_scale,
                             shuffle=shuffle, out_slot=out_slot)

    def forward(self, x):
        return ops.rows_to_nchw(self.forward_rows(ops.nchw_to_rows(x, torch.float32)))


def default_conv(in_channels, out_channels, kernel_size, bias=True):
    return Conv2d(in_channels, out_channels, kernel_size, padding=(kernel_size // 2), bias=bias)


class UpSampler(nn.Sequential):

    def __init__(self, conv, scale, n_feats, bn=False, act=None, bias=True):
        if bn:
            raise NotImplementedError("rdst_amd UpSampler: BatchNorm is not on the RDST path (bn_in_conv = None)")
        m = []
        if (scale & (scale - 1)) == 0:
            for _ in range(int(math.log(scale, 2))):
                m.append(conv(n_feats, 4 * n_feats, 3, bias))
                m.append(nn.PixelShuffle(2))
                if act is not None:
                    m.append(act)
        elif scale == 3:
            m.append(conv(n_feats, 9 * n_feats, 3, bias))
            m.append(nn.PixelShuffle(3))
            if act is not None:
                m.append(act)
        else:
            raise NotImplementedError('SR scale {} is not valid.'.format(scale))
        super().__init__(*m)

    def forward_rows(self, x):
        mods = list(self)
        i = 0
        while i < len(mods):
            m = mods[i]
            if isinstance(m, Conv2d) and i + 1 < len(mods) and isinstance(mods[i + 1], nn.PixelShuffle):
                x = m.forward_rows(x, shuffle=mods[i + 1].upscale_factor)
                i += 2
            elif isinstance(m, Conv2d):
                x = m.forward_rows(x)
                i += 1
            else:
                raise NotImplementedError(f"rdst_amd UpSampler: {type(m).__name__} inside the upsampler")
        return x

    def forward(self, x):
        return ops.rows_to_nchw(self.forward_rows(ops.nchw_to_rows(x, torch.float32)))


class MeanShift(Conv2d):

    def __init__(self, mean=(0.,), std=(1.0,), mode='sub'):
        if len(mean) != len(std):
            raise ValueError('Size of means and stds should be the same')
        nc = len(mean)
        super().__init__(nc, nc, kernel_size=1)
        std = torch.Tensor(std)
        mean = torch.Tensor(mean)
        if mode == 'sub':
            self.weight.data = torch.eye(nc).view(nc, nc, 1, 1) / std.view(nc, 1, 1, 1)
            self.bias.data = -1 * mean / std
        elif mode == 'add':
            self.weight.data = torch.eye(nc).view(nc, nc, 1, 1) * std.view(nc, 1, 1, 1)
            self.bias.data = 1 * mean
        for p in self.parameters():
            p.requires_grad = False
```

rdst_amd/networks/rdst_variations.py:

```python
from __future__ import annotations

import torch
import torch.nn as nn

from .. import ops
from .common import Conv2d, MeanShift, UpSampler, default_conv
from .swin_transformer_sr import (BasicLayer, Mlp, PatchEmbed, PatchUnEmbed, SwinTransformerBlock,
                                  WindowAttention, _drop_p, _ln_params, _norm_only, trunc_normal_, window_partition,
                                  window_reverse)


def _dim_modifier(input_dim, growth_rate, norm_layer, pre_norm):
    if pre_norm:
        return nn.Sequential(norm_layer(input_dim), nn.Linear(input_dim, growth_rate))
    return nn.Sequential(nn.Linear(input_dim, growth_rate), norm_layer(growth_rate))


def _apply_dim_modifier(seq, x, out_scale=1.0, out_slot=None):
    if isinstance(seq, nn.Identity):
        if out_slot is not None:
            raise NotImplementedError("rdst_amd: dense slot behind an Identity tail")
        return x if out_scale == 1.0 else x * out_scale
    a, b = seq[0], seq[1]
    if isinstance(b, nn.Linear):
        w, bb = _ln_params(a)
        return ops.ln_linear(x, w, bb, b.weight, b.bias, out_scale=out_scale, out_slot=out_slot)
    y = ops.ln_linear(x, None, None, a.weight, a.bias)
    return _norm_only(y, b, out_scale=out_scale, out_slot=out_slot)


def _slot_ok(seq):
    if isinstance(seq, nn.Identity):
        return False
    b = seq[1]
    return isinstance(b, nn.Linear) or isinstance(b, nn.LayerNorm)


class DenseSTLayer(nn.Module):

    def __init__(self, input_dim, input_resolution, depth=2, num_heads=6, window_size=2,
                 mlp_ratio=4., qkv_bias=True, qk_scale=None, drop=0., attn_drop=0.,
                 drop_path=30., norm_layer=nn.LayerNorm, downsample=None, use_checkpoint=False,
                 growth_rate=60, dense_scale=1., dim_modify_mode='tail',
                 pre_norm=False):
        super().__init__()
        assert growth_rate % num_heads == 0, 'growth_rate % num_heads should be 0'
        assert input_dim % num_heads == 0, 'token dim % num_heads should be 0'
        if dim_modify_mode == 'head':
            self.head = (_dim_modifier(input_dim, growth_rate, norm_layer, pre_norm)
                         if input_dim != growth_rate else nn.Identity())
            hidden_dim = growth_rate
            self.tail = nn.Identity()
        elif dim_modify_mode == 'tail':
            self.head = nn.Identity()
            hidden_dim = input_dim
            self.tail = (_dim_modifier(hidden_dim, growth_rate, norm_layer, pre_norm)
                         if hidden_dim != growth_rate else nn.Identity())
        else:
            raise ValueError(f"dim_modify_mode {dim_modify_mode!r} (head or tail)")
        self.body = BasicLayer(hidden_dim, input_resolution, depth, num_heads, window_size, mlp_ratio, qkv_bias,
                               qk_scale, drop, attn_drop, drop_path, norm_layer, downsample, use_checkpoint)
        self.input_dim = input_dim
        self.hidden_dim = hidden_dim
        self.input_resolution = input_resolution
        self.dense_scale = dense_scale
        self.growth_rate = hidden_dim
        self.growth_rate_out = growth_rate
        self.depth = depth
        self.pre_norm = pre_norm

    def new_features(self, x, x_size, out_slot=None, sink=None):
        y = _apply_dim_modifier(self.head, x)
        y = self.body(y, x_size, sink=sink) if sink is not None else self.body(y, x_size)
        return _apply_dim_modifier(self.tail, y, out_scale=self.dense_scale, out_slot=out_slot)

    def _grad_sink(self, x):
        blocks = self.body.blocks
        if isinstance(self.head, nn.Identity) and len(blocks) > 0 and blocks[0].fuses_input_gradient() \
                and x.requires_grad and torch.is_grad_enabled():
            return ops.GradSink()
        return None

    def forward(self, x, x_size):
        return torch.cat((x, self.new_features(x, x_size)), 2)

    def forward_dense(self, x, x_size, buf):
        sink = self._grad_sink(x)
        if not _slot_ok(self.tail):
            new = self.new_features(x, x_size, sink=sink)
            buf.fill(x.shape[-1], new)
            return ops.dense_join(x, new, buf, sink)
        new = self.new_features(x, x_size, out_slot=(buf, x.shape[-1]), sink=sink)
        return ops.dense_join(x, new, buf, sink)


def _res_connection(resi_connection, cin, cout):
    if resi_connection == '1conv':
        return Conv2d(cin, cout, 3, 1, 1)
    if resi_connection == '3conv':
        return nn.Sequential(Conv2d(cin, cin // 4, 3, 1, 1),
                             nn.LeakyReLU(negative_slope=0.2, inplace=True),
                             Conv2d(cin // 4, cin // 4, 1, 1, 0),
                             nn.LeakyReLU(negative_slope=0.2, inplace=True),
                             Conv2d(cin // 4, cout, 3, 1, 1))
    return None


def _apply_res_connection(conv, x, residual=None, out_scale=1.0, out_slot=None):
    if isinstance(conv, Conv2d):
        return conv.forward_rows(x, residual=residual, out_scale=out_scale, out_slot=out_slot)
    y = conv[0].forward_rows(x)
    y = conv[2].forward_rows(y, in_act=ops.ACT_LEAKY02)
    return conv[4].forward_rows(y, in_act=ops.ACT_LEAKY02, residual=residual, out_scale=out_scale, out_slot=out_slot)


class RDSTB(nn.Module):

    def __init__(self, input_dim, input_resolution, layer_depth, num_heads=6, window_size=2,
                 mlp_ratio=4., qkv_bias=True, qk_scale=None, drop=0., attn_drop=0.,
                 drop_path=0., norm_layer=nn.LayerNorm, downsample=None, use_checkpoint=False,
                 img_size=224, patch_size=4, resi_connection='1conv',
                 growth_rate=0, dense_scale=1., dim_modify_mode='tail',
                 num_blocks=3, residual_scale=1.,
                 pre_norm=False):
        super().__init__()
        self.input_dim = input_dim
        self.input_resolution = input_resolution
        self.residual_scale = residual_scale
        idim = input_dim
        self.body = nn.ModuleList([])
        for _ in range(int(num_blocks)):
            self.body.append(DenseSTLayer(
                input_dim=idim, input_resolution=input_resolution, depth=layer_depth, num_heads=num_heads,
                window_size=window_size, mlp_ratio=mlp_ratio, qkv_bias=qkv_bias, qk_scale=qk_scale, drop=drop,
                attn_drop=attn_drop, drop_path=drop_path, norm_layer=norm_layer, downsample=downsample,
                use_checkpoint=use_checkpoint, growth_rate=growth_rate, dense_scale=dense_scale,
                dim_modify_mode=dim_modify_mode, pre_norm=pre_norm))
            idim += growth_rate
        conv = _res_connection(resi_connection, idim, input_dim)
        if conv is not None:
            self.conv = conv
        self.patch_embed = PatchEmbed(img_size=img_size, patch_size=patch_size, in_chans=0, embed_dim=input_dim,
                                      norm_layer=None)
        self.patch_unembed = PatchUnEmbed(img_size=img_size, patch_size=patch_size, in_chans=0, embed_dim=idim,
                                          norm_layer=None)

    def dense_width(self):
        return self.input_dim + sum(m.growth_rate_out for m in self.body)

    def make_buffer(self, B, L, dtype, device):
        return ops.DenseBuffer((B, L), self.dense_width(), dtype, device)

    def forward(self, x, x_size, buf=None, out_slot=None):
        B, L, C = x.shape
        H, W = x_size
        if x.is_cuda and len(self.body) > 0:
            if buf is None:
                buf = self.make_buffer(B, L, x.dtype, x.device)
            y = ops.into_dense(x, buf)
            for m in self.body:
                y = m.forward_dense(y, x_size, buf)
        else:
            y = x
            for m in self.body:
                y = m(y, x_size)
        out = _apply_res_connection(self.conv, y.view(B, H, W, y.shape[-1]), residual=x.view(B, H, W, C),
                                    out_scale=self.residual_scale, out_slot=out_slot)
        return out.view(B, L, C)


class RDSTSR(nn.Module):

    def __init__(self, img_size=48, patch_size=1, in_chans=1, sr_scale=2, embed_dim=60,
                 dense_layer_depths=[2, 2, 2, 2], num_heads=[6, 6, 6, 6],
                 window_size=[4, 4, 4, 4], rdb_depths=[3, 3, 3, 3],
                 mlp_ratio=4., qkv_bias=True, qk_scale=None,
                 drop_rate=0., attn_drop=0., drop_path_rate=0.,
                 norm_layer=nn.LayerNorm, ape=False, patch_norm=True,
                 use_checkpoint=False, resi_connection='1conv',
                 growth_rate=30, dense_scale=1., dim_modify_mode='tail',
                 rdb_residual_scale=1.,
                 global_res_scale=1.,
                 mean=None, std=None,
                 act_in_conv='leaky_relu', bn_in_conv=None,
                 scale_free=False,
                 scale_embedding=False,
                 pre_norm=False,
                 feature_last_operation=False):
        super().__init__()
        self.input_resolution = img_size
        self.patch_size = patch_size
        self.input_channel = in_chans
        self.num_blocks = len(rdb_depths)
        assert len(rdb_depths) == len(window_size) == len(num_heads) == len(dense_layer_depths)
        self.n_feats = embed_dim
        self.patch_norm = patch_norm
        self.ape = ape
        self.use_checkpoint = use_checkpoint
        self.drop_path_rate = drop_path_rate
        self.drop_rate = drop_rate
        self.resi_connection = resi_connection
        self.global_res_scale = global_res_scale
        self.window_size = window_size
        self.mlp_ratio = mlp_ratio
        self.qkv_bias = qkv_bias
        self.qk_scale = qk_scale
        self.norm_layer = norm_layer
        self.num_heads = num_heads
        self.dense_layer_depths = dense_layer_depths
        self.dense_scale = dense_scale
        self.growth_rate = growth_rate
        self.dim_modify_mode = dim_modify_mode
        self.rdb_depths = rdb_depths
        self.rdb_residual_scale = rdb_residual_scale

        if act_in_conv == 'relu':
            self.act_in_conv = nn.ReLU(True)
        elif act_in_conv == 'leaky_relu':
            self.act_in_conv = nn.LeakyReLU(negative_slope=0.2, inplace=True)
        elif act_in_conv == 'prelu':
            self.act_in_conv = nn.PReLU()
        else:
            raise ValueError('Invalid activation {}, should be one of [relu, leaky_relu, prelu]'.format(act_in_conv))
        self.bn_in_conv = bn_in_conv
        self.sr_scale = sr_scale
        self.scale_free = scale_free
        self.scale_embedding = scale_embedding
        if scale_embedding:
            self.scale_embedding = nn.Identity()
            self.scale_embed_layer = nn.Linear(1, 1)
        if scale_free:
            raise NotImplementedError("rdst_amd RDSTSR: scale_free=True (MetaUpSampler) is outside the hot path; "
                                      "every shipped config has scale_free = False")

        if mean is None:
            mean = [0. for _ in range(self.input_channel)]
        if std is None:
            std = [1. for _ in range(self.input_channel)]
        if len(mean) != len(std) or len(mean) != self.input_channel:
            raise ValueError('Dimension of mean {} / std {} should fit input channels {}'.format(
                len(mean), len(std), self.input_channel))
        self.mean = mean
        self.std = std
        self.add_mean = MeanShift(mean, std, 'add')
        self.sub_mean = MeanShift(mean, std, 'sub')

        self.head = default_conv(in_chans, embed_dim, 3)
        self.patch_embed = PatchEmbed(img_size=img_size, patch_size=patch_size, in_chans=embed_dim,
                                      embed_dim=embed_dim, norm_layer=norm_layer if self.patch_norm else None)
        num_patches = self.patch_embed.num_patches
        patches_resolution = self.patch_embed.patches_resolution
        self.patches_resolution = patches_resolution
        self.patch_unembed = PatchUnEmbed(img_size=img_size, patch_size=patch_size, in_chans=embed_dim,
                                          embed_dim=embed_dim, norm_layer=norm_layer if self.patch_norm else None)
        if self.ape:
            self.absolute_pos_embed = nn.Parameter(torch.zeros(1, num_patches, embed_dim))
            trunc_normal_(self.absolute_pos_embed, std=.02)
        self.pos_drop = nn.Dropout(p=_drop_p(drop_rate, "drop_rate"))

        self.body = nn.ModuleList()
        for i_block in range(self.num_blocks):
            self.body.append(RDSTB(
                input_dim=embed_dim, input_resolution=(patches_resolution[0], patches_resolution[1]),
                layer_depth=self.dense_layer_depths[i_block], num_heads=self.num_heads[i_block],
                window_size=self.window_size[i_block], mlp_ratio=self.mlp_ratio, qkv_bias=self.qkv_bias,
                qk_scale=self.qk_scale, drop=self.drop_rate, attn_drop=attn_drop, norm_layer=norm_layer,
                img_size=self.input_resolution, patch_size=self.patch_size, resi_connection=self.resi_connection,
                growth_rate=self.growth_rate, dense_scale=self.dense_scale, dim_modify_mode=self.dim_modify_mode,
                num_blocks=self.rdb_depths[i_block], residual_scale=self.rdb_residual_scale, pre_norm=pre_norm))
        self.norm = norm_layer(self.n_feats)

        self.feature_last_operation = feature_last_operation
        cab = _res_connection(resi_connection, embed_dim, embed_dim)
        if cab is not None:
            self.conv_after_body = cab

        m_tail = []
        if self.sr_scale > 1:
            m_tail.append(UpSampler(default_conv, self.sr_scale, self.n_feats, act=None, bn=self.bn_in_conv))
        m_tail.append(default_conv(self.n_feats, self.input_channel, 3))
        self.tail = nn.Sequential(*m_tail)

        self.compute_dtype, self.compute_code = torch.float32, ops.F32
        self.apply(self._init_weights)

    def _init_weights(self, m):
        if isinstance(m, nn.Linear):
            trunc_normal_(m.weight, std=.02)
            if m.bias is not None:
                nn.init.constant_(m.bias, 0)
        elif isinstance(m, nn.LayerNorm):
            nn.init.constant_(m.bias, 0)
            nn.init.constant_(m.weight, 1.0)

    @torch.jit.ignore
    def no_weight_decay(self):
        return {'absolute_pos_embed'}

    @torch.jit.ignore
    def no_weight_decay_keywords(self):
        return {'relative_position_bias_table'}

    def set_compute_dtype(self, dtype):
        self.compute_dtype, self.compute_code = ops.resolve_compute_dtype(dtype)
        return self

    def forward_features_rows(self, feat):
        B, H, W, E = feat.shape
        x_size = (H, W)
        t = feat.view(B, H * W, E)
        blocks = list(self.body)
        chain = t.is_cuda and len(blocks) > 0 and all(isinstance(b, RDSTB) and len(b.body) > 0 and hasattr(b, "conv")
                                                      and b.input_dim == E for b in blocks)
        bufs = [b.make_buffer(B, H * W, t.dtype, t.device) for b in blocks] if chain else [None] * len(blocks)
        pos_drop = self.training and self.pos_drop.p > 0.
        if self.patch_embed.norm is not None:
            first = (bufs[0], 0) if (chain and not self.ape and not pos_drop and isinstance(self.patch_embed.norm, nn.LayerNorm)) else None
            t = _norm_only(t, self.patch_embed.norm, out_slot=first)
        if self.ape:
            t = t + self.absolute_pos_embed.to(t.dtype)
        if pos_drop:
            t = self.pos_drop(t)
        for i, blk in enumerate(blocks):
            if chain:
                t = blk(t, x_size, buf=bufs[i], out_slot=(bufs[i + 1], 0) if i + 1 < len(blocks) else None)
            else:
                t = blk(t, x_size)
        return t

    def forward_features(self, x):
        with ops.compute_scope(self.compute_code):
            rows = ops.nchw_to_rows(x, self.compute_dtype)
            t = self.forward_features_rows(rows)
            B, H, W, E = rows.shape
            return ops.rows_to_nchw(_norm_only(t, self.norm).view(B, H, W, E))

    def forward(self, x, sr_scale=None):
        with ops.compute_scope(self.compute_code), ops.pack_scope(self):
            return self._forward(x, sr_scale)

    def _forward(self, x, sr_scale=None):
        rows = ops.nchw_to_rows(x, self.compute_dtype)
        rows = self.sub_mean.forward_rows(rows)
        feat = self.head.forward_rows(rows)
        B, H, W, E = feat.shape
        t = self.forward_features_rows(feat)
        if self.feature_last_operation:
            t = _norm_only(t, self.norm, out_scale=self.global_res_scale)
            res = _apply_res_connection(self.conv_after_body, t.view(B, H, W, E), residual=feat)
        else:
            res = _norm_only(t, self.norm, out_scale=self.global_res_scale, residual=feat.view(B, H * W, E))
            res = res.view(B, H, W, E)
        y = res
        for m in self.tail:
            y = m.forward_rows(y)
        y = self.add_mean.forward_rows(y)
        return ops.rows_to_nchw(y)

    def extra_repr(self):
        return ''

    def flops(self):
        return None


class RDSTSR_N(RDSTSR):

    def __init__(self, img_size=48, patch_size=1, in_chans=1, sr_scale=2, embed_dim=60,
                 dense_layer_depths=[2, 2, 2, 2], num_heads=[6, 6, 6, 6],
                 window_size=[4, 4, 4, 4], rdb_depths=[3, 3, 3, 3],
                 mlp_ratio=4., qkv_bias=True, qk_scale=None,
                 drop_rate=0., attn_drop=0., drop_path_rate=0.,
                 norm_layer=nn.LayerNorm, ape=False, patch_norm=True,
                 use_checkpoint=False, resi_connection='1conv',
                 growth_rate=30, dense_scale=1., dim_modify_mode='tail',
                 rdb_residual_scale=1., global_res_scale=1., mean=None, std=None,
                 act_in_conv='leaky_relu', bn_in_conv=None, scale_free=False, scale_embedding=False,
                 pre_norm=False, global_bottleneck=True, global_bottleneck_ratio=1., global_bottleneck_mode='mlp'):
        super().__init__(img_size=img_size, patch_size=patch_size, in_chans=in_chans, sr_scale=sr_scale,
                         embed_dim=embed_dim, dense_layer_depths=dense_layer_depths, num_heads=num_heads,
                         window_size=window_size, rdb_depths=rdb_depths, mlp_ratio=mlp_ratio, qkv_bias=qkv_bias,
                         qk_scale=qk_scale, drop_rate=drop_rate, attn_drop=attn_drop, drop_path_rate=drop_path_rate,
                         norm_layer=norm_layer, ape=ape, patch_norm=patch_norm, use_checkpoint=use_checkpoint,
                         resi_connection=resi_connection, growth_rate=growth_rate, dense_scale=dense_scale,
                         dim_modify_mode=dim_modify_mode, rdb_residual_scale=rdb_residual_scale,
                         global_res_scale=global_res_scale, mean=mean, std=std, act_in_conv=act_in_conv,
                         bn_in_conv=bn_in_conv, scale_free=scale_free, scale_embedding=scale_embedding,
                         pre_norm=pre_norm, feature_last_operation=False)
        del self.feature_last_operation
        cab = self._modules.pop('conv_after_body', None)
        tail = self._modules.pop('tail')
        self.global_bottleneck_mode = global_bottleneck_mode
        self.do_global_bottleneck = global_bottleneck
        if self.do_global_bottleneck:
            cin = self.n_feats * self.num_blocks
            cf = int(self.n_feats * global_bottleneck_ratio)
            if global_bottleneck_mode == 'mlp':
                self.bottleneck = nn.Sequential(nn.Linear(cin, cf), nn.Linear(cf, cf))
            elif global_bottleneck_mode == 'conv':
                self.bottleneck = nn.Sequential(default_conv(cin, cf, 1), default_conv(cf, cf, 3))
            else:
                raise ValueError(f"global_bottleneck_mode {global_bottleneck_mode!r} (mlp or conv)")
        else:
            cf = self.n_feats
            self.bottleneck = None
        if cab is not None:
            self.conv_after_body = cab
        if cf != self.n_feats:
            m_tail = []
            if self.sr_scale > 1:
                m_tail.append(UpSampler(default_conv, self.sr_scale, cf, act=None, bn=self.bn_in_conv))
            m_tail.append(default_conv(cf, self.input_channel, 3))
            tail = nn.Sequential(*m_tail)
        self.tail = tail
        if self.bottleneck is not None:
            self.bottleneck.apply(self._init_weights)

    def forward(self, x, sr_scale=None):
        with ops.compute_scope(self.compute_code):
            return self._forward_n(x, sr_scale)

    def _forward_n(self, x, sr_scale=None):
        rows = ops.nchw_to_rows(x, self.compute_dtype)
        rows = self.sub_mean.forward_rows(rows)
        feat = self.head.forward_rows(rows)
        B, H, W, E = feat.shape
        t = feat.view(B, H * W, E)
        if self.patch_embed.norm is not None:
            t = _norm_only(t, self.patch_embed.norm)
        if self.ape:
            t = t + self.absolute_pos_embed.to(t.dtype)
        t = self.pos_drop(t)
# ... 52 lines not shown
```

rdst_amd/networks/swin_transformer_sr.py:

```python
from __future__ import annotations

import torch
import torch.nn as nn
import torch.nn.functional as F

from .. import ops


def to_2tuple(x):
    return tuple(x) if isinstance(x, (tuple, list)) else (x, x)


def trunc_normal_(tensor, mean=0., std=1., a=-2., b=2.):
    return nn.init.trunc_normal_(tensor, mean=mean, std=std, a=a, b=b)


def _drop_p(p, what):
    p = float(p or 0.)
    if not (0. <= p < 1.):
        raise ValueError(f"rdst_amd: {what}={p} must be in [0, 1)")
    return p


class DropPath(nn.Module):

    def __init__(self, drop_prob=0., scale_by_keep=True):
        super().__init__()
        self.drop_prob = float(drop_prob)
        self.scale_by_keep = scale_by_keep

    def mask(self, x):
        keep = 1.0 - self.drop_prob
        m = torch.empty((x.shape[0],) + (1,) * (x.ndim - 1), dtype=torch.float32, device=x.device).bernoulli_(keep)
        if keep > 0.0 and self.scale_by_keep:
            m.div_(keep)
        return m

    def forward(self, x):
        if self.drop_prob == 0. or not self.training:
            return x
        return (x.float() * self.mask(x)).to(x.dtype)

    def extra_repr(self):
        return f"drop_prob={round(self.drop_prob, 3):0.3f}"


def _ln_params(norm):
    if isinstance(norm, nn.LayerNorm):
        if abs(norm.eps - 1e-5) > 0 or not norm.elementwise_affine:
            raise NotImplementedError("rdst_amd: LayerNorm must be affine with eps 1e-5")
        return norm.weight, norm.bias
    if isinstance(norm, nn.Identity) or norm is None:
        return None, None
    raise NotImplementedError(f"rdst_amd: norm layer {type(norm).__name__} (nn.LayerNorm or nn.Identity)")


def _norm_only(x, norm, out_scale=1.0, residual=None, out_slot=None):
    w, b = _ln_params(norm)
    if w is None:
        y = x if out_scale == 1.0 else x * out_scale
        y = y if residual is None else y + residual
        if out_slot is not None:
            raise NotImplementedError("rdst_amd: dense slot without a LayerNorm")
        return y
    return ops.ln_linear(x, w, b, None, None, out_scale=out_scale, residual=residual, out_slot=out_slot)


class Mlp(nn.Module):

    def __init__(self, in_features, hidden_features=None, out_features=None, act_layer=nn.GELU, drop=0.):
        super().__init__()
        out_features = out_features or in_features
        hidden_features = hidden_features or in_features
        if act_layer is not nn.GELU:
            raise NotImplementedError("rdst_amd Mlp: only nn.GELU (exact erf form)")
        self.fc1 = nn.Linear(in_features, hidden_features)
        self.act = act_layer()
        self.fc2 = nn.Linear(hidden_features, out_features)
        self.drop = nn.Dropout(_drop_p(drop, "drop"))

    def forward(self, x, norm=None, residual=None):
        w, b = _ln_params(norm)
        h = ops.ln_linear(x, w, b, self.fc1.weight, self.fc1.bias)
        if self.training and self.drop.p > 0.:
            h = self.drop(F.gelu(h))
            y = self.drop(ops.ln_linear(h, None, None, self.fc2.weight, self.fc2.bias))
            return y if residual is None else y + residual
        return ops.ln_linear(h, None, None, self.fc2.weight, self.fc2.bias, in_act=ops.ACT_GELU, residual=residual)


def window_partition(x, window_size):
    B, H, W, C = x.shape
    x = x.view(B, H // window_size, window_size, W // window_size, window_size, C)
    return x.permute(0, 1, 3, 2, 4, 5).contiguous().view(-1, window_size, window_size, C)


def window_reverse(windows, window_size, H, W):
    B = int(windows.shape[0] / (H * W / window_size / window_size))
    x = windows.view(B, H // window_size, W // window_size, window_size, window_size, -1)
    return x.permute(0, 1, 3, 2, 4, 5).contiguous().view(B, H, W, -1)


def _relative_position_index(wh, ww):
    ys, xs = torch.meshgrid(torch.arange(wh), torch.arange(ww), indexing="ij")
    y, x = ys.reshape(-1), xs.reshape(-1)
    return (y[:, None] - y[None, :] + wh - 1) * (2 * ww - 1) + (x[:, None] - x[None, :] + ww - 1)


class WindowAttention(nn.Module):

    def __init__(self, dim, window_size, num_heads, qkv_bias=True, qk_scale=None, attn_drop=0., proj_drop=0.):
        super().__init__()
        self.dim = dim
        self.window_size = window_size
        self.num_heads = num_heads
        head_dim = dim // num_heads
        self.scale = qk_scale or head_dim ** -0.5
        if window_size[0] != window_size[1]:
            raise NotImplementedError("rdst_amd WindowAttention: square windows only")
        self.relative_position_bias_table = nn.Parameter(
            torch.zeros((2 * window_size[0] - 1) * (2 * window_size[1] - 1), num_heads))
        self.register_buffer("relative_position_index", _relative_position_index(window_size[0], window_size[1]))
        self.qkv = nn.Linear(dim, dim * 3, bias=qkv_bias)
        self.attn_drop = nn.Dropout(_drop_p(attn_drop, "attn_drop"))
        self.proj = nn.Linear(dim, dim)
        self.proj_drop = nn.Dropout(_drop_p(proj_drop, "proj_drop"))
        trunc_normal_(self.relative_position_bias_table, std=.02)
        self.softmax = nn.Softmax(dim=-1)

    def forward(self, x, mask=None):
        B_, N, C = x.shape
        ws = self.window_size[0]
        qkv = ops.ln_linear(x, None, None, self.qkv.weight, self.qkv.bias)
        a = ops.window_attention(qkv.view(B_, ws, ws, 3 * C), self.relative_position_bias_table, ws, ws,
                                 self.num_heads, ws, 0, self.scale, mask=mask, attn_drop=self.active_attn_drop())
        return self.proj_drop(ops.ln_linear(a.view(B_, N, C), None, None, self.proj.weight, self.proj.bias))

    def active_attn_drop(self):
        return self.attn_drop.p if self.training else 0.

    def extra_repr(self) -> str:
        return f'dim={self.dim}, window_size={self.window_size}, num_heads={self.num_heads}'


class SwinTransformerBlock(nn.Module):

    def __init__(self, dim, input_resolution, num_heads, window_size=7, shift_size=0,
                 mlp_ratio=4., qkv_bias=True, qk_scale=None, drop=0., attn_drop=0., drop_path=0.,
# ... 389 lines not shown
```

rdst_amd/ops.py:

```python
from __future__ import annotations

import os
import threading
import weakref

from typing import Optional

import torch

from . import _lib, side
from ._lib import ACT_GELU, ACT_LEAKY001, ACT_LEAKY02, ACT_NONE, BF16, F32, F32X3


F32_SPLIT = False
_scope_tls = threading.local()


def set_f32_split(on: bool) -> None:
    global F32_SPLIT
    F32_SPLIT = bool(on)


class compute_scope:

    def __init__(self, code: Optional[int]):
        if code not in (None, F32, _lib.F32X3, BF16):
            raise ValueError(f"rdst_amd: bad compute code {code!r}")
        self.code = code

    def __enter__(self):
        self.prev = getattr(_scope_tls, "code", None)
        if self.code is not None:
            _scope_tls.code = self.code
        return self

    def __exit__(self, *exc):
        _scope_tls.code = self.prev
        return False


def resolve_compute_dtype(dtype):
    if dtype == "fp32x3":
        return torch.float32, _lib.F32X3
    if dtype in ("fp32", torch.float32):
        return torch.float32, F32
    if dtype in ("bf16", torch.bfloat16):
        return torch.bfloat16, BF16
    raise ValueError("compute dtype must be torch.float32 ('fp32'), 'fp32x3' or torch.bfloat16 ('bf16')")


def _dtype_code(t: torch.Tensor) -> int:
    if t.dtype == torch.float32:
        sc = getattr(_scope_tls, "code", None)
        if sc is None or sc == BF16:
            return _lib.F32X3 if (sc is None and F32_SPLIT) else F32
        return sc
    if t.dtype == torch.bfloat16:
        return BF16
    raise TypeError(f"rdst_amd: unsupported activation dtype {t.dtype} (float32 or bfloat16)")


def _elt_code(t: torch.Tensor) -> int:
    if t.dtype == torch.float32:
        return F32
    if t.dtype == torch.bfloat16:
        return BF16
    raise TypeError(f"rdst_amd: unsupported activation dtype {t.dtype} (float32 or bfloat16)")


def _need_gpu(*ts: Optional[torch.Tensor]) -> None:
    for t in ts:
        if t is not None and not t.is_cuda:
            raise RuntimeError(
                "rdst_amd: the HIP path needs GPU tensors; there is no CPU fallback "
                "(the CPU oracle lives in oracle/ and is test-only)")


def _stream() -> int:
    return torch.cuda.current_stream().cuda_stream


def _rows(t: torch.Tensor) -> tuple[torch.Tensor, int]:
    if t.dim() == 1:
        t = t.unsqueeze(0)
    C = t.shape[-1]
    if C != 1 and t.stride(-1) != 1:
        t = t.contiguous()
    ld = None
    exp = 0
    for d in range(t.dim() - 2, -1, -1):
        if t.shape[d] == 1:
            continue
        if ld is None:
# ... 200 lines not shown


def _wattn_fwd(lib, qkv, ld, tab, msk, out, geom, attn_drop=0.0, seed=None, try_lse=False):
    B, H, W, C, heads = geom[:5]
    if try_lse:
        nlse = torch.empty((B * H * W, heads), dtype=torch.float32, device=qkv.device)
        rc = lib.rdst_wattn_fwd_lse(qkv.data_ptr(), ld, tab.data_ptr(), out.data_ptr(), C, nlse.data_ptr(), *geom, _stream())
        if rc != _lib.ENOTSUP:
            _lib.check(rc, "rdst_wattn_fwd_lse")
            return nlse
    args = (qkv.data_ptr(), ld, tab.data_ptr(), _ptr(msk), 0 if msk is None else msk.shape[0], out.data_ptr(), C, *geom)
    if attn_drop > 0.0:
        _lib.check(lib.rdst_wattn_fwd_drop(*args, attn_drop, seed.data_ptr(), _stream()), "rdst_wattn_fwd_drop")
    else:
        _lib.check(lib.rdst_wattn_fwd(*args, _stream()), "rdst_wattn_fwd")
    return None


def _wattn_bwd(lib, qkv, ld, tab, msk, dout, ldd, dqkv, dtable, wsp, nbytes, geom, attn_drop=0.0, seed=None, saved=None):
    C = geom[3]
    grads = (dqkv.data_ptr(), 3 * C, dtable.data_ptr(), wsp.data_ptr(), nbytes, *geom)
    if saved is not None:
        rc = lib.rdst_wattn_bwd_lse(qkv.data_ptr(), ld, tab.data_ptr(), dout.data_ptr(), ldd, saved[0].data_ptr(), C,
                                    saved[1].data_ptr(), *grads, _stream())
        if rc != _lib.ENOTSUP:
            _lib.check(rc, "rdst_wattn_bwd_lse")
            return
    args = (qkv.data_ptr(), ld, tab.data_ptr(), _ptr(msk), 0 if msk is None else msk.shape[0], dout.data_ptr(), ldd, *grads)
    if attn_drop > 0.0:
        _lib.check(lib.rdst_wattn_bwd_drop(*args, attn_drop, seed.data_ptr(), _stream()), "rdst_wattn_bwd_drop")
    else:
        _lib.check(lib.rdst_wattn_bwd(*args, _stream()), "rdst_wattn_bwd")


class _WindowAttention(torch.autograd.Function):
    @staticmethod
    def forward(ctx, qkv, table, mask, H, W, heads, ws, shift, scale, attn_drop=0.0, seed=None):
        _need_gpu(qkv, table, mask)
        C = qkv.shape[-1] // 3
        B = qkv.numel() // (H * W * 3 * C)
        qkv_r, ld = _rows(qkv)
        tab, msk = _param(table), _param(mask)
        out = torch.empty(qkv.shape[:-1] + (C,), dtype=qkv.dtype, device=qkv.device)
        ctx.geom = (B, H, W, C, heads, ws, shift, float(scale), _dtype_code(qkv))
        ctx.ld, ctx.attn_drop = ld, float(attn_drop)
        _wattn_fwd(_lib.load(), qkv_r, ld, tab, msk, out, ctx.geom, ctx.attn_drop, seed)
        ctx.save_for_backward(qkv_r, tab, msk, seed)
        return out

    @staticmethod
    def backward(ctx, dout):
        qkv, tab, msk, seed = ctx.saved_tensors
        B, H, W, C, heads, ws = ctx.geom[:6]
        lib = _lib.load()
        dout_r, ldd = _rows(dout)
        dqkv = torch.empty(qkv.shape[:-1] + (3 * C,), dtype=qkv.dtype, device=qkv.device)
        dtable = _grad_like(tab)
        nbytes = lib.rdst_wattn_bwd_workspace(B, H, W, C, heads, ws)
        wsp = _workspace(nbytes, qkv.device)
        if _ReduceBatch.depth > 0:
            _ReduceBatch.keep.append(wsp)
        _wattn_bwd(lib, qkv, ctx.ld, tab, msk, dout_r, ldd, dqkv, dtable, wsp, nbytes, ctx.geom, ctx.attn_drop, seed)
        _ReduceBatch.settle(lib)
        return dqkv, dtable, None, None, None, None, None, None, None, None, None


def draw_seed(device) -> torch.Tensor:
    return torch.randint(0, 2 ** 62, (1,), dtype=torch.int64, device=device)


def window_attention(qkv: torch.Tensor, table: torch.Tensor, H: int, W: int, heads: int, ws: int, shift: int,
                     scale: float, mask: Optional[torch.Tensor] = None, attn_drop: float = 0.0,
                     seed: Optional[torch.Tensor] = None) -> torch.Tensor:
    if attn_drop and attn_drop > 0.0:
        if not (0.0 < attn_drop < 1.0):
            raise ValueError(f"window_attention: attn_drop={attn_drop} must be in [0, 1)")
        if seed is None:
            seed = draw_seed(qkv.device)
        return _WindowAttention.apply(qkv, table, mask, H, W, heads, ws, shift, scale, float(attn_drop), seed)
    return _WindowAttention.apply(qkv, table, mask, H, W, heads, ws, shift, scale)


def _linear_bwd_call(lib, x, ldx, lw, lb, stats, in_act, w, dy, lddy, dx, lddx, dx_add, ld_add, dw, db, dlw, dlb,
                     M, K, N, out_scale, code, dev, keep=None, dx_add2=None, ld_add2=0):
    if all(t is None for t in (dx, dlw, dlb, dw, db)):
        return
    nbytes = lib.rdst_ln_linear_bwd_workspace(M, K, N)
    wsp = _workspace(nbytes, dev)
    if keep is not None:
        keep.append(wsp)
    args = (x.data_ptr(), ldx, _ptr(lw), _ptr(lb), _ptr(stats), in_act, _ptr(w), dy.data_ptr(), lddy, _ptr(dx), lddx,
            _ptr(dx_add), ld_add, _ptr(dw), _ptr(db), _ptr(dlw), _ptr(dlb), wsp.data_ptr(), nbytes, M, K, N, out_scale, code,
            _stream())
    if dx_add2 is not None and dx is not None:
        rc = lib.rdst_ln_linear_bwd2(*args, dx_add2.data_ptr(), ld_add2)
        if rc != _lib.ENOTSUP:
            _lib.check(rc, "rdst_ln_linear_bwd2")
            return
    _lib.check(lib.rdst_ln_linear_bwd(*args), "rdst_ln_linear_bwd")
    if dx_add2 is not None and dx is not None:
        dx.add_(dx_add2)


def _ln_linear_fwd(lib, x, ldx, lw, lb, in_act, w, b, res, ldr, y, ldy, stats, M, K, N, out_scale, code):
    wsp, wptr, nws = None, None, 0
    if w is not None and (X3_STREAM or code != F32X3) and lib.rdst_ln_linear_fwd_packable(
            K, N, int(lw is not None), int(res is not None), int(in_act), code):
        nb = lib.rdst_ln_linear_fwd_workspace2(K, N, code)
        wsp, wptr, nws = _packed_workspace([(_linear_pack_kind(code), w, lw, lb, b, N, K, out_scale, nb)], nb, x.device)
    _lib.check(lib.rdst_ln_linear_fwd(x.data_ptr(), ldx, _ptr(lw), _ptr(lb), int(in_act), _ptr(w), _ptr(b), _ptr(res), ldr,
                                      y.data_ptr(), ldy, _ptr(stats), wptr, nws, M, K, N, float(out_scale), code, _stream()),
               "rdst_ln_linear_fwd")


def _bias_grad(ctx, wanted: bool) -> Optional[torch.Tensor]:
    return _grad_like(ctx.bias_ref) if (ctx.bias_ref is not None and wanted) else None


class _LnLinear(torch.autograd.Function):
    @staticmethod
    def forward(ctx, x, ln_w, ln_b, weight, bias, residual, in_act, out_scale, out_slot=None):
        _need_gpu(x, ln_w, ln_b, weight, bias, residual)
        lib = _lib.load()
        K = x.shape[-1]
        N = K if weight is None else weight.shape[0]
        M = x.numel() // K
        x_r, ldx = _rows(x)
        lw, lb, w, b = _param(ln_w), _param(ln_b), _param(weight), _param(bias)
        if out_slot is None:
            y = torch.empty(x.shape[:-1] + (N,), dtype=x.dtype, device=x.device)
            ldy = N
        else:
            y = out_slot[0].slot(out_slot[1], N)
            ldy = out_slot[0].width
            if y.shape[:-1] != x.shape[:-1] or y.dtype != x.dtype:
                raise ValueError("rdst_amd.ln_linear: out_slot does not match the input's rows / dtype")
        r_r, ldr = (None, 0)
        if residual is not None:
            if residual.dtype != x.dtype:
                raise TypeError("rdst_amd.ln_linear: residual dtype differs from the activation dtype")
            r_r, ldr = _rows(residual)
        stats = torch.empty((M, 2), dtype=torch.float32, device=x.device) if lw is not None else None
        code = _dtype_code(x)
        _ln_linear_fwd(lib, x_r, ldx, lw, lb, in_act, w, b, r_r, ldr, y, ldy, stats, M, K, N, out_scale, code)
        ctx.save_for_backward(x_r, lw, lb, w, stats)
        ctx.bias_ref = b
        ctx.meta = (M, K, N, ldx, int(in_act), float(out_scale), residual is not None, code)
        return y

    @staticmethod
    def backward(ctx, dy):
        x, lw, lb, w, stats = ctx.saved_tensors
        M, K, N, ldx, in_act, out_scale, has_res, code = ctx.meta
        lib = _lib.load()
        dy_r, lddy = _rows(dy)
        need = ctx.needs_input_grad
        dev = x.device
        dx = torch.empty(x.shape[:-1] + (K,), dtype=x.dtype, device=dev) if need[0] else None
        dlw = _grad_like(lw) if (lw is not None and need[1]) else None
        dlb = _grad_like(lb) if (lb is not None and need[2]) else None
        dw = _grad_like(w) if (w is not None and need[3]) else None
        db = _bias_grad(ctx, need[4])
        _linear_bwd_call(lib, x, ldx, lw, lb, stats, in_act, w, dy_r, lddy, dx, K, None, 0, dw, db, dlw, dlb, M, K, N,
                         out_scale, code, dev, keep=_ReduceBatch.keep if _ReduceBatch.depth > 0 else None)
        _ReduceBatch.settle(lib)
        dres = dy if (has_res and need[5]) else None
        return dx, dlw, dlb, dw, db, dres, None, None, None


class DenseBuffer:

    def __init__(self, lead, width, dtype, device):
        self.width = int(width)
        self.t = torch.empty(tuple(lead) + (self.width,), dtype=dtype, device=device)

    def slot(self, c0, n):
        return self.t[..., c0:c0 + n]

    def fill(self, c0, src):
        self.t.data[..., c0:c0 + src.shape[-1]].copy_(src.detach())


class _IntoDense(torch.autograd.Function):

    @staticmethod
    def forward(ctx, x, buf):
        v = buf.slot(0, x.shape[-1])
        v.copy_(x)
        return v


    @staticmethod
    def backward(ctx, g):
        return g, None


class _ReduceBatchState(threading.local):

    EPOCH = 0

    def __init__(self):
        self.depth, self.keep, self.fresh = 0, [], 0
        self.owner, self.mixed = -1, False
        self.epoch = type(self).EPOCH

    @staticmethod
    def _task():
        return torch._C._current_graph_task_id()

    def _foreign(self):
        if self.depth > 0 and self._task() != self.owner:
            self.mixed = True
        return self.mixed

    def _drop_stale(self, lib):
        if self.epoch != type(self).EPOCH:
            self.abandon(lib)
            self.epoch = type(self).EPOCH

    def _flush(self, lib, join=False):
        on_side = side.enabled()
        try:
            _lib.check(lib.rdst_reduce_batch_end(_stream()), "rdst_reduce_batch_end")
        finally:
            if on_side:
                side.park(self.keep)
            self.keep = []
            self.fresh = 0
        if on_side:
            from . import dp
            side.release_older()
            if join or not dp._OFFERED:
                side.join()

    def begin(self, lib):
        self._drop_stale(lib)
        if self.depth == 0:
            _lib.check(lib.rdst_reduce_batch_begin(), "rdst_reduce_batch_begin")
            self.owner = self._task()
            self.mixed = False
        self.depth += 1

    def begin_layer(self, lib):
        self._drop_stale(lib)
        if self.depth > 0:
            if self.owner == self._task():
                self.abandon(lib)
            else:
                self.mixed = True
        self.begin(lib)

    def end(self, lib, keep=None):
        if keep:
            self.keep.extend(keep)
        self.depth -= 1
        if self.depth == 0:
            self._flush(lib)

    def settle(self, lib):
        self._drop_stale(lib)
        if self.depth > 0 and (self.fresh or self._foreign()):
            self._flush(lib, join=True)
            _lib.check(lib.rdst_reduce_batch_begin(), "rdst_reduce_batch_begin")
        elif self.depth == 0:
            self.fresh = 0

    def abandon(self, lib):
        if self.depth > 0:
            _lib.check(lib.rdst_reduce_batch_abort(), "rdst_reduce_batch_abort")
        self.depth = 0
        self.keep = []
        self.fresh = 0
        self.mixed = False


_ReduceBatch = _ReduceBatchState()


def reset_backward_state() -> None:
    type(_ReduceBatch).EPOCH += 1
    if _lib.loaded():
        _ReduceBatch._drop_stale(_lib.load())
    side.reset()


class GradSink:

    def __init__(self):
        self.extra = None
        self.batch_open = False

    def take(self):
        e, self.extra = self.extra, None
        return e

    def take_batch(self):
        b, self.batch_open = self.batch_open, False
        return b


class _DenseJoin(torch.autograd.Function):

    @staticmethod
    def forward(ctx, prefix, new, buf, sink=None):
        ctx.c = prefix.shape[-1]
        ctx.sink = sink
        return buf.slot(0, prefix.shape[-1] + new.shape[-1])

    @staticmethod
    def backward(ctx, g):
        if ctx.sink is not None and ctx.needs_input_grad[0]:
            ctx.sink.extra = g[..., :ctx.c]
            if g.is_cuda:
                lib = _lib.load()
                _ReduceBatch.begin_layer(lib)
                ctx.sink.batch_open = True
            return None, g[..., ctx.c:], None, None
        return g[..., :ctx.c], g[..., ctx.c:], None, None


def into_dense(x: torch.Tensor, buf: DenseBuffer) -> torch.Tensor:
    if x.data_ptr() == buf.t.data_ptr() and x.stride()[:-1] == buf.t.stride()[:-1] and x.shape[:-1] == buf.t.shape[:-1]:
        return x
    return _IntoDense.apply(x, buf)


def dense_join(prefix: torch.Tensor, new: torch.Tensor, buf: DenseBuffer, sink: "GradSink" = None) -> torch.Tensor:
    return _DenseJoin.apply(prefix, new, buf, sink)


def ln_linear(x: torch.Tensor, ln_w: Optional[torch.Tensor], ln_b: Optional[torch.Tensor],
              weight: Optional[torch.Tensor], bias: Optional[torch.Tensor], *, in_act: int = ACT_NONE,
              residual: Optional[torch.Tensor] = None, out_scale: float = 1.0, out_slot=None) -> torch.Tensor:
    return _LnLinear.apply(x, ln_w, ln_b, weight, bias, residual, in_act, out_scale, out_slot)


class _SwinBlock(torch.autograd.Function):

    @staticmethod
    def forward(ctx, x, n1w, n1b, qkvw, qkvb, table, projw, projb, n2w, n2b, fc1w, fc1b, fc2w, fc2b, H, W, heads, ws,
                shift, scale, sink=None):
        ctx.sink = sink
        _need_gpu(x, qkvw, table, projw, fc1w, fc2w)
        lib = _lib.load()
        C = x.shape[-1]
        M = x.numel() // C
        B = M // (H * W)
        hid = fc1w.shape[0]
        code = _dtype_code(x)
        dev, dt = x.device, x.dtype
        x_r, ldx = _rows(x)
        P = [_param(t) for t in (n1w, n1b, qkvw, qkvb, table, projw, projb, n2w, n2b, fc1w, fc1b, fc2w, fc2b)]
        n1w_, n1b_, qkvw_, qkvb_, tab_, projw_, projb_, n2w_, n2b_, fc1w_, fc1b_, fc2w_, fc2b_ = P
        lead = x.shape[:-1]
        st = _stream()
        stats1 = torch.empty((M, 2), dtype=torch.float32, device=dev) if n1w_ is not None else None
        qkv = torch.empty(lead + (3 * C,), dtype=dt, device=dev)
        a = torch.empty(lead + (C,), dtype=dt, device=dev)
        x1 = torch.empty(lead + (C,), dtype=dt, device=dev)
        fused_attn = (ATTN_FUSED and n1w_ is not None and n1b_ is not None
                      and bool(lib.rdst_swin_attn_fwd_supported(C, heads, ws, code)))
        if fused_attn:
            nbytes, nbp = lib.rdst_swin_attn_fwd_workspace(C), lib.rdst_ln_linear_fwd_workspace(C, C)
            _wsp, wptr, nws = _packed_workspace([(PACK_LINEAR_SEC3, qkvw_, n1w_, n1b_, qkvb_, 3 * C, C, 1.0, nbytes - nbp),
                                                 (PACK_LINEAR, projw_, None, None, projb_, C, C, 1.0, nbp)], nbytes, dev)
            rc = lib.rdst_swin_attn_fwd(x_r.data_ptr(), ldx, n1w_.data_ptr(), n1b_.data_ptr(), qkvw_.data_ptr(), _ptr(qkvb_),
                                        tab_.data_ptr(), projw_.data_ptr(), _ptr(projb_), qkv.data_ptr(), 3 * C, a.data_ptr(), C,
                                        x1.data_ptr(), C, stats1.data_ptr(), wptr, nws, B, H, W, C, heads, ws, shift,
                                        float(scale), code, st)
            if rc == _lib.ENOTSUP:
                fused_attn = False
            else:
                _lib.check(rc, "rdst_swin_attn_fwd")
        nlse = None
        if not fused_attn:
            _ln_linear_fwd(lib, x_r, ldx, n1w_, n1b_, ACT_NONE, qkvw_, qkvb_, None, 0, qkv, 3 * C, stats1, M, C, 3 * C, 1.0, code)
            nlse = _wattn_fwd(lib, qkv, 3 * C, tab_, None, a, (B, H, W, C, heads, ws, shift, float(scale), code),
                              try_lse=ATTN_LSE and ws == 16 and code == BF16)
            _ln_linear_fwd(lib, a, C, None, None, ACT_NONE, projw_, projb_, x_r, ldx, x1, C, None, M, C, C, 1.0, code)
        stats2 = torch.empty((M, 2), dtype=torch.float32, device=dev) if n2w_ is not None else None
        y = torch.empty(lead + (C,), dtype=dt, device=dev)
        h = None
        fused_mlp = MLP_FUSED and n2w_ is not None and bool(lib.rdst_mlp_fused_supported(C, hid, code))
        if fused_mlp:
            _wsp, wptr, nws = None, None, 0
            if lib.rdst_mlp_fwd_packable(C, hid, code):
                _wsp, wptr, nws = _packed_workspace(
                    [(PACK_LINEAR, fc1w_, n2w_, n2b_, fc1b_, hid, C, 1.0, lib.rdst_ln_linear_fwd_workspace(C, hid)),
                     (PACK_LINEAR, fc2w_, None, None, fc2b_, C, hid, 1.0, lib.rdst_ln_linear_fwd_workspace(hid, C))],
                    lib.rdst_mlp_fwd_workspace(C, hid), dev)
            rc = lib.rdst_mlp_fwd(x1.data_ptr(), C, n2w_.data_ptr(), n2b_.data_ptr(), fc1w_.data_ptr(), _ptr(fc1b_),
                                  fc2w_.data_ptr(), _ptr(fc2b_), y.data_ptr(), C, stats2.data_ptr(), wptr, nws, M, C, hid, code, st)
            if rc == _lib.ENOTSUP:
                fused_mlp = False
            else:
                _lib.check(rc, "rdst_mlp_fwd")
        if not fused_mlp:
            h = torch.empty(lead + (hid,), dtype=dt, device=dev)
            _ln_linear_fwd(lib, x1, C, n2w_, n2b_, ACT_NONE, fc1w_, fc1b_, None, 0, h, hid, stats2, M, C, hid, 1.0, code)
            _ln_linear_fwd(lib, h, hid, None, None, ACT_GELU, fc2w_, fc2b_, x1, C, y, C, None, M, hid, C, 1.0, code)
        ctx.save_for_backward(x_r, stats1, qkv, a, x1, stats2, h, nlse, *P)
        ctx.meta = (M, B, H, W, C, hid, heads, ws, shift, float(scale), ldx, code)
        return y

    @staticmethod
    def backward(ctx, dy):
        (x, stats1, qkv, a, x1, stats2, h, nlse, n1w, n1b, qkvw, qkvb, tab, projw, projb, n2w, n2b, fc1w, fc1b, fc2w,
         fc2b) = ctx.saved_tensors
        M, B, H, W, C, hid, heads, ws, shift, scale, ldx, code = ctx.meta
        lib = _lib.load()
        dev, dt = x.device, x.dtype
        need = ctx.needs_input_grad
        dy_r, lddy = _rows(dy)

        def g(t, flag):
            return _grad_like(t) if (t is not None and flag) else None

        dn1w, dn1b, dqkvw, dqkvb = g(n1w, need[1]), g(n1b, need[2]), g(qkvw, need[3]), g(qkvb, need[4])
        dprojw, dprojb = g(projw, need[6]), g(projb, need[7])
        dn2w, dn2b, dfc1w, dfc1b = g(n2w, need[8]), g(n2b, need[9]), g(fc1w, need[10]), g(fc1b, need[11])
        dfc2w, dfc2b = g(fc2w, need[12]), g(fc2b, need[13])
        keep = []
        outer = ctx.sink is not None and ctx.sink.take_batch()
        _ReduceBatch.begin(lib)
        try:
            return _SwinBlock._backward_body(ctx, lib, dy_r, lddy, need, keep, dn1w, dn1b, dqkvw, dqkvb, dprojw, dprojb, dn2w,
                                             dn2b, dfc1w, dfc1b, dfc2w, dfc2b)
        finally:
            _ReduceBatch.end(lib, keep)
            if outer:
                _ReduceBatch.end(lib)
            _ReduceBatch.settle(lib)

    @staticmethod
    def _backward_body(ctx, lib, dy_r, lddy, need, keep, dn1w, dn1b, dqkvw, dqkvb, dprojw, dprojb, dn2w, dn2b, dfc1w, dfc1b,
                       dfc2w, dfc2b):
        (x, stats1, qkv, a, x1, stats2, h, nlse, n1w, n1b, qkvw, qkvb, tab, projw, projb, n2w, n2b, fc1w, fc1b, fc2w,
         fc2b) = ctx.saved_tensors
        M, B, H, W, C, hid, heads, ws, shift, scale, ldx, code = ctx.meta
        dev, dt = x.device, x.dtype
        dx1 = torch.empty_like(x1)
        fused_mlp = h is None or (MLP_FUSED and all(t is not None for t in (dn2w, dn2b, dfc1w, dfc1b, dfc2w, dfc2b))
                                  and bool(lib.rdst_mlp_fused_supported(C, hid, code)))
        if fused_mlp:
            def out(t, like, n=None):
                if t is not None:
                    return t
                t = torch.empty_like(like) if like is not None else torch.empty(n, dtype=torch.float32, device=dev)
                keep.append(t)
                return t
            o = [out(dfc1w, fc1w), out(dfc1b, fc1b, hid), out(dfc2w, fc2w), out(dfc2b, fc2b, C), out(dn2w, n2w),
                 out(dn2b, n2b)]
            nb = lib.rdst_mlp_bwd_workspace(M, C, hid)
            wsp_m = _workspace(nb, dev)
            keep.append(wsp_m)

            def mlp_bwd(dy_, ld_):
                return lib.rdst_mlp_bwd(x1.data_ptr(), C, n2w.data_ptr(), n2b.data_ptr(), stats2.data_ptr(), fc1w.data_ptr(),
                                        _ptr(fc1b), fc2w.data_ptr(), dy_.data_ptr(), ld_, dx1.data_ptr(), C,
                                        o[0].data_ptr(), o[1].data_ptr(), o[2].data_ptr(), o[3].data_ptr(), o[4].data_ptr(),
                                        o[5].data_ptr(), wsp_m.data_ptr(), nb, M, C, hid, code, _stream())
            rc = mlp_bwd(dy_r, lddy)
            if rc == _lib.ENOTSUP and h is None:
                dy_c = dy_r.clone(memory_format=torch.contiguous_format)
                keep.append(dy_c)
                rc = mlp_bwd(dy_c, C)
            if rc == _lib.ENOTSUP and h is not None:
                fused_mlp = False
            else:
                _lib.check(rc, "rdst_mlp_bwd")
        if not fused_mlp:
            dh = torch.empty_like(h)
            _linear_bwd_call(lib, h, hid, None, None, None, ACT_GELU, fc2w, dy_r, lddy, dh, hid, None, 0, dfc2w, dfc2b,
                             None, None, M, hid, C, 1.0, code, dev, keep=keep)
            _linear_bwd_call(lib, x1, C, n2w, n2b, stats2, ACT_NONE, fc1w, dh, hid, dx1, C, dy_r, lddy, dfc1w, dfc1b,
                             dn2w, dn2b, M, C, hid, 1.0, code, dev, keep=keep)
        da = torch.empty_like(a)
        _linear_bwd_call(lib, a, C, None, None, None, ACT_NONE, projw, dx1, C, da, C, None, 0, dprojw, dprojb, None, None,
                         M, C, C, 1.0, code, dev, keep=keep)
        dqkv = torch.empty_like(qkv)
        dtab = _grad_like(tab)
        nbytes = lib.rdst_wattn_bwd_workspace(B, H, W, C, heads, ws)
        wsp = _workspace(nbytes, dev)
        keep.append(wsp)
        _wattn_bwd(lib, qkv, 3 * C, tab, None, da, C, dqkv, dtab, wsp, nbytes, (B, H, W, C, heads, ws, shift, scale, code),
                   saved=None if nlse is None else (a, nlse))
        dx = torch.empty(x.shape, dtype=dt, device=dev) if need[0] else None
        extra = ctx.sink.take() if ctx.sink is not None else None
        if extra is not None and need[0]:
            extra, ld_extra = _rows(extra)
            keep.append(extra)
        else:
            extra, ld_extra = None, 0
        _linear_bwd_call(lib, x, ldx, n1w, n1b, stats1, ACT_NONE, qkvw, dqkv, 3 * C, dx, C, dx1 if need[0] else None, C,
                         dqkvw, dqkvb, dn1w, dn1b, M, C, 3 * C, 1.0, code, dev, keep=keep, dx_add2=extra,
                         ld_add2=ld_extra)
        if not need[5]:
            dtab = None
        return (dx, dn1w, dn1b, dqkvw, dqkvb, dtab, dprojw, dprojb, dn2w, dn2b, dfc1w, dfc1b, dfc2w, dfc2b,
                None, None, None, None, None, None, None)


def swin_block(x, n1w, n1b, qkvw, qkvb, table, projw, projb, n2w, n2b, fc1w, fc1b, fc2w, fc2b, H, W, heads, ws, shift,
               scale, sink=None):
    return _SwinBlock.apply(x, n1w, n1b, qkvw, qkvb, table, projw, projb, n2w, n2b, fc1w, fc1b, fc2w, fc2b, H, W, heads,
                            ws, shift, scale, sink)


class _ConvRows(torch.autograd.Function):
    @staticmethod
    def forward(ctx, x, weight, bias, residual, in_act, out_scale, shuffle, out_slot=None):
        _need_gpu(x, weight, bias, residual)
        lib = _lib.load()
        if x.dim() != 4:
            raise ValueError("rdst_amd.conv_rows: x must be (B, H, W, Cin) token-major")
        B, H, W, Cin = x.shape
        Cout, cin_w, k, k2 = weight.shape
        if cin_w != Cin or k != k2:
            raise ValueError(f"rdst_amd.conv_rows: weight {tuple(weight.shape)} does not fit Cin={Cin}")
        r = int(shuffle)
        x_r, ldx = _rows(x)
        w, b = _param(weight), _param(bias)
        cy = Cout // (r * r)
        if out_slot is None:
            y, ldy = torch.empty((B, H * r, W * r, cy), dtype=x.dtype, device=x.device), cy
        else:
            y = out_slot[0].slot(out_slot[1], cy).view(B, H * r, W * r, cy)
            ldy = out_slot[0].width
        r_r, ldr = (None, 0)
        if residual is not None:
            if residual.dtype != x.dtype or tuple(residual.shape) != tuple(y.shape):
                raise ValueError("rdst_amd.conv_rows: residual must match the output shape/dtype")
            r_r, ldr = _rows(residual)
        code = _dtype_code(x)
        _wsp, wptr, nws = None, None, 0
        if (X3_STREAM or code != F32X3) and lib.rdst_conv_fwd_packable(Cin, Cout, k, r, int(r_r is not None), int(in_act), code):
            nb = lib.rdst_conv_fwd_workspace2(Cin, Cout, k, code)
            _wsp, wptr, nws = _packed_workspace([(PACK_CONV3_FWD_X3 if code == F32X3 else PACK_CONV3_FWD, w, None, None, None, Cout,
                                                  Cin, out_scale, nb)], nb, x.device)
        _lib.check(lib.rdst_conv_fwd(x_r.data_ptr(), ldx, int(in_act), w.data_ptr(), _ptr(b), _ptr(r_r), ldr,
                                     y.data_ptr(), ldy, wptr, nws, B, H, W, Cin, Cout, k, float(out_scale), r,
                                     code, _stream()), "rdst_conv_fwd")
        ctx.bias_ref = b
        ctx.save_for_backward(x_r, w)
        ctx.meta = (B, H, W, Cin, Cout, k, ldx, int(in_act), float(out_scale), r, residual is not None, code)
        return y

    @staticmethod
    def backward(ctx, dy):
        x, w = ctx.saved_tensors
        B, H, W, Cin, Cout, k, ldx, in_act, out_scale, r, has_res, code = ctx.meta
        lib = _lib.load()
        dy_r, lddy = _rows(dy)
        need = ctx.needs_input_grad
        dev = x.device
        dx = torch.empty((B, H, W, Cin), dtype=x.dtype, device=dev) if need[0] else None
        dw = _grad_like(w) if need[1] else None
        db = _bias_grad(ctx, need[2])
        nbytes = lib.rdst_conv_bwd_workspace(B, H, W, Cin, Cout, k)
        wsp = _workspace(nbytes, dev)
        forked = side.conv_enabled() and dx is not None and (dw is not None or db is not None)
        fresh = _ReduceBatch.fresh
        _lib.check(lib.rdst_conv_bwd(x.data_ptr(), ldx, in_act, w.data_ptr(), dy_r.data_ptr(), lddy, _ptr(dx), Cin,
                                     None, 0, _ptr(dw), _ptr(db), wsp.data_ptr(), nbytes, B, H, W, Cin, Cout, k,
                                     out_scale, r, code, _stream()), "rdst_conv_bwd")
        if forked:
            from . import dp
            side.park_current([x, dy_r, wsp])
            if fresh or not dp._OFFERED:
                side.join()
        _ReduceBatch.settle(lib)
        dres = dy if (has_res and need[3]) else None
        return dx, dw, db, dres, None, None, None, None


def conv_rows(x: torch.Tensor, weight: torch.Tensor, bias: Optional[torch.Tensor], *, in_act: int = ACT_NONE,
              residual: Optional[torch.Tensor] = None, out_scale: float = 1.0, shuffle: int = 1, out_slot=None) -> torch.Tensor:
    return _ConvRows.apply(x, weight, bias, residual, in_act, out_scale, shuffle, out_slot)


class _NchwToRows(torch.autograd.Function):
    @staticmethod
    def forward(ctx, x, dtype):
        _need_gpu(x)
        lib = _lib.load()
        B, C, H, W = x.shape
        xs = x.detach().float().contiguous()
        rows = torch.empty((B, H, W, C), dtype=dtype, device=x.device)
        _lib.check(lib.rdst_nchw_to_rows(xs.data_ptr(), rows.data_ptr(), C, B, C, H, W, _elt_code(rows), _stream()),
                   "rdst_nchw_to_rows")
        return rows

    @staticmethod
    def backward(ctx, drows):
        return _RowsToNchw.apply(drows), None


class _RowsToNchw(torch.autograd.Function):
    @staticmethod
    def forward(ctx, rows):
        _need_gpu(rows)
        lib = _lib.load()
        B, H, W, C = rows.shape
        r, ld = _rows(rows)
        ctx.dtype = rows.dtype
        out = torch.empty((B, C, H, W), dtype=torch.float32, device=rows.device)
        _lib.check(lib.rdst_rows_to_nchw(r.data_ptr(), ld, out.data_ptr(), B, C, H, W, _elt_code(rows), _stream()),
                   "rdst_rows_to_nchw")
        return out

    @staticmethod
    def backward(ctx, dout):
        return _NchwToRows.apply(dout, ctx.dtype)


class _Upsample2(torch.autograd.Function):
    @staticmethod
    def forward(ctx, rows):
        _need_gpu(rows)
        lib = _lib.load()
        B, H, W, C = rows.shape
        r, ld = _rows(rows)
        out = torch.empty((B, 2 * H, 2 * W, C), dtype=rows.dtype, device=rows.device)
        _lib.check(lib.rdst_upsample2_fwd(r.data_ptr(), ld, out.data_ptr(), C, B, H, W, C, _elt_code(rows), _stream()),
                   "rdst_upsample2_fwd")
        ctx.geom = (B, H, W, C)
        return out

    @staticmethod
    def backward(ctx, dy):
        lib = _lib.load()
        B, H, W, C = ctx.geom
        d, ld = _rows(dy)
        dx = torch.empty((B, H, W, C), dtype=dy.dtype, device=dy.device)
        _lib.check(lib.rdst_upsample2_bwd(d.data_ptr(), ld, dx.data_ptr(), C, B, H, W, C, _elt_code(dy), _stream()),
                   "rdst_upsample2_bwd")
        return dx


def upsample_nearest2(rows: torch.Tensor) -> torch.Tensor:
    return _Upsample2.apply(rows)


def nchw_to_rows(x: torch.Tensor, dtype: torch.dtype = torch.float32) -> torch.Tensor:
    return _NchwToRows.apply(x, dtype)


def rows_to_nchw(rows: torch.Tensor) -> torch.Tensor:
    return _RowsToNchw.apply(rows)
```

rdst_amd/trainer.py:

```python
from __future__ import annotations

import contextlib
import math
import time
from typing import Callable, Dict, Optional, Sequence

import torch
import torch.distributed as dist
import torch.nn.functional as F

from . import dp, side
from .optim import FlatAdam

GUARD_OFF = 1e8


class DPTrainStep:

    RECORD_FLUSH = 4096

    def __init__(self, net: torch.nn.Module, lr: float = 1e-4, betas=(0.9, 0.99), eps: float = 1e-8,
                 weight_decay: float = 0.0, milestones: Optional[Sequence[int]] = None, gamma: float = 0.5,
                 loss_threshold: float = GUARD_OFF, loss_fn: Optional[Callable] = None, group=None,
                 graph: bool = False, graph_warmup: int = 2, device_guard: bool = False,
                 max_grad_norm: Optional[float] = None, skip_nonfinite: bool = False,
                 ema_decay: Optional[float] = None, ema_warmup: bool = False):
        self.device_guard = bool(device_guard)
        self.max_grad_norm = None if max_grad_norm is None else float(max_grad_norm)
        self.skip_nonfinite = bool(skip_nonfinite)
        if self.device_guard and not all(p.is_cuda for p in net.parameters()):
            raise ValueError("DPTrainStep(device_guard=True): the guard is a HIP kernel, the network must be on a GPU")
        if not self.device_guard and (self.max_grad_norm is not None or self.skip_nonfinite):
            raise ValueError("DPTrainStep: max_grad_norm and skip_nonfinite need device_guard=True")
        self.net = net
        self.group = group
        dp.broadcast_parameters(net, group=group)
        self.bucket = dp.FlatGradBucket(net.parameters())
        self.optimizer = FlatAdam(self.bucket.params, lr=lr, betas=betas, eps=eps, weight_decay=weight_decay,
                                  bucket=self.bucket, device_state=self.device_guard, ema_decay=ema_decay,
                                  ema_warmup=ema_warmup)
        self.scheduler = (torch.optim.lr_scheduler.MultiStepLR(self.optimizer, milestones=list(milestones), gamma=gamma)
                          if milestones else None)
        if self.device_guard and self.scheduler is not None:
            self.optimizer.set_schedule(list(milestones), gamma)
            self.optimizer.attach_scheduler(self.scheduler)
        self._peer_skip = None
        self._graph_has_update = False
        self.loss_fn = loss_fn if loss_fn is not None else F.l1_loss
        self.loss_module = loss_fn if hasattr(loss_fn, "state_dict") else torch.nn.Module()
        self.loss_threshold = float(loss_threshold)
        self.last_report = None
        self.last_batch = None
        self.use_graph = bool(graph)
        self.graph_warmup = int(graph_warmup)
        self.graph = None
        self._graph_report = None
        self._static = None
        self._eager_seen = 0
        self._loss_buf = None
        self.capture_hook = None
        self.training_loss_names = ["L1"] if loss_fn is None else list(getattr(loss_fn, "loss_components", ["loss"]))
        self.training_loss_records: Dict[str, list] = {n: [] for n in self.training_loss_names}
        self._pending: Dict[str, list] = {}
        self._pending_keep: Dict[str, list] = {}
        self.quick_validation_reports: list = []
        self.current_training_state_id = 0
        self.current_epoch = 0
        self.training_epoch_costs: list = []

    def _refuse_averaged(self, what: str) -> None:
        if self.optimizer.ema_active:
            raise RuntimeError(f"DPTrainStep.{what}: inside ema_scope() the network holds the averaged weights; "
                               "it must not train on them")

    def _keep_step(self, loss: torch.Tensor) -> bool:
        skip = torch.logical_not(loss.detach() < self.loss_threshold).to(torch.float32).reshape(1)
        if dist.is_available() and dist.is_initialized() and dist.get_world_size(self.group) > 1:
            dist.all_reduce(skip, op=dist.ReduceOp.MAX, group=self.group)
        return float(skip.item()) == 0.0

    def _loss(self, out, targets):
        r = self.loss_fn(out, targets)
        if isinstance(r, tuple):
            self.last_report = r[1]
            return r[0]
        return r

    def _record(self, loss: torch.Tensor) -> None:
        rep = self.last_report
        keep = self.optimizer.state_field("last_keep").clone() if self.device_guard else None
        if isinstance(rep, dict) and rep:
            for n in self.training_loss_names:
                if n in rep:
                    v = rep.raw(n) if hasattr(rep, "raw") else dict.__getitem__(rep, n)
                    self._pending.setdefault(n, []).append(v.detach().clone() if torch.is_tensor(v) else float(v))
                    self._pending_keep.setdefault(n, []).append(keep)
        elif len(self.training_loss_names) == 1:
            self._pending.setdefault(self.training_loss_names[0], []).append(loss.detach().clone())
            self._pending_keep.setdefault(self.training_loss_names[0], []).append(keep)
        if sum(len(v) for v in self._pending.values()) >= self.RECORD_FLUSH:
            self._flush_records()

    @staticmethod
    def _filter_records(vals: list, keeps: list) -> list:
        ts = [v for v in vals if torch.is_tensor(v)]
        host = torch.stack([t.reshape(()).float() for t in ts]).cpu().tolist() if ts else []
        ks = [k for k in keeps if torch.is_tensor(k)]
        flags = iter(torch.stack([k.reshape(()) for k in ks]).cpu().tolist() if ks else [])
        it = iter(host)
        out = []
        for v, k in zip(vals, keeps):
            x = next(it) if torch.is_tensor(v) else v
            if (next(flags) if torch.is_tensor(k) else (1 if k is None else k)) != 0:
                out.append(x)
        return out

    def _flush_records(self) -> None:
        for n, vals in self._pending.items():
            if not vals:
                continue
            keeps = self._pending_keep.get(n) or [None] * len(vals)
            self.training_loss_records.setdefault(n, []).extend(self._filter_records(vals, keeps))
        self._pending = {}
        self._pending_keep = {}

    def loss_records(self) -> Dict[str, list]:
        self._flush_records()
        return self.training_loss_records

    def fwd_bwd(self, inputs: torch.Tensor, targets: torch.Tensor) -> torch.Tensor:
        self._refuse_averaged("fwd_bwd")
        self.bucket.detach_grads()
        out = self.net(inputs)
        loss = self._loss(out, targets)
        if self._loss_buf is None:
            self._loss_buf = torch.zeros((), dtype=torch.float32, device=inputs.device)
        self._loss_buf.copy_(loss.detach())
        side.enable()
        try:
            loss.backward()
        finally:
            try:
                side.join()
            finally:
                side.disable()
        self.bucket.gather()
        return self._loss_buf

    def capture(self, inputs: torch.Tensor, targets: torch.Tensor) -> bool:
        self._refuse_averaged("capture")
        self._static = (inputs.detach().clone(), targets.detach().clone())
        torch.cuda.synchronize()
        g = torch.cuda.CUDAGraph()
        try:
            with (self.capture_hook() if self.capture_hook is not None else contextlib.nullcontext()):
                with torch.cuda.graph(g):
                    self.fwd_bwd(*self._static)
                    if self._update_in_graph():
                        self._finish_step()
        except Exception as e:
            import warnings
            warnings.warn(f"rdst_amd.trainer: HIP-graph capture failed ({type(e).__name__}: {e}); running eagerly")
            torch.cuda.synchronize()
            from . import ops
            ops.reset_backward_state()
            dp._OFFERED = {}
            self.bucket.gather()
            self.use_graph, self.graph, self._static, self._graph_report = False, None, None, None
            self._graph_has_update = False
            return False
        if not self.bucket.check_views():
            self.use_graph, self.graph, self._static, self._graph_report = False, None, None, None
            return False
        self.graph = g
        self._graph_has_update = self._update_in_graph()
        self._graph_report = self.last_report
        return True

    def _graph_fits(self, inputs, targets) -> bool:
        return (self._static is not None and inputs.shape == self._static[0].shape and targets.shape == self._static[1].shape
                and inputs.dtype == self._static[0].dtype and targets.dtype == self._static[1].dtype)

    def step(self, inputs: torch.Tensor, targets: torch.Tensor) -> torch.Tensor:
        self._refuse_averaged("step")
        t0 = time.time()
        self.current_epoch += 1
        self.net.train()
        guarded = self.loss_threshold < GUARD_OFF and not self.device_guard
        if guarded:
            self.bucket.detach_grads()
            out = self.net(inputs)
            loss = self._loss(out, targets)
            if self._keep_step(loss):
                self._record(loss)
                loss.backward()
                self.bucket.gather()
                self._finish_step()
            else:
                self.bucket.gather()
            self.training_epoch_costs.append(time.time() - t0)
            return loss.detach()
        if self.use_graph and self.graph is None and self._eager_seen >= self.graph_warmup:
            self.capture(inputs, targets)
        if self.graph is not None and self._graph_fits(inputs, targets):
            if inputs.data_ptr() != self._static[0].data_ptr():
                self._static[0].copy_(inputs)
            if targets.data_ptr() != self._static[1].data_ptr():
                self._static[1].copy_(targets)
            self.graph.replay()
            self.last_report = self._graph_report
            loss = self._loss_buf
            in_graph = self._graph_has_update
        else:
            loss = self.fwd_bwd(inputs, targets)
            self._eager_seen += 1
            in_graph = False
        if self.device_guard:
            if not in_graph:
                self._finish_step()
            self._record(loss)
        else:
            self._record(loss)
            self._finish_step()
# ... 156 lines not shown
```

Before: 1859 patches/s.

## Fuse residual gradient adds into LN-linear backward and add fused L1 loss kernel

Adds a third residual-gradient input (dX_add3) to the bf16 LayerNorm-linear backward and LN-only backward kernels. A conv_rows residual gradient is handed through a sink object to the downstream LN-linear backward, so it is added inside that kernel rather than returned to autograd and accumulated separately. It also adds a custom L1 loss kernel that computes the loss and its sign gradient in one pass, and seeds backward with that gradient. The aim is fewer elementwise launches and less memory traffic per step. The cost is extra plumbing, an env-var off switch, and fallback paths that still do a separate add.

```diff
diff --git a/include/rdst_hip_fold.h b/include/rdst_hip_fold.h
--- /dev/null
+++ b/include/rdst_hip_fold.h
@@ -0,0 +1,26 @@
+#ifndef RDST_HIP_FOLD_H
+#define RDST_HIP_FOLD_H
+
+#include <stddef.h>
+#include <stdint.h>
+
+#ifdef __cplusplus
+extern "C" {
+#endif
+
+int rdst_ln_linear_bwd3(const void* X, int64_t ld_x, const float* ln_w, const float* ln_b,
+                        const float* stats, int in_act, const float* Wt, const void* dY,
+                        int64_t ld_dy, void* dX, int64_t ld_dx, const void* dX_add, int64_t ld_dx_add,
+                        float* dW, float* dbias, float* dln_w, float* dln_b, void* workspace,
+                        size_t workspace_bytes, int64_t M, int K, int N, float out_scale, int dtype,
+                        void* stream, const void* dX_add2, int64_t ld_dx_add2, const void* dX_add3,
+                        int64_t ld_dx_add3);
+
+size_t rdst_l1_loss_workspace(int64_t n);
+int rdst_l1_loss(const float* y, const float* target, int64_t n, float* grad, float* loss, void* workspace,
+                 size_t workspace_bytes, void* stream);
+
+#ifdef __cplusplus
+}
+#endif
+#endif
diff --git a/rdst_amd/_lib.py b/rdst_amd/_lib.py
--- a/rdst_amd/_lib.py
+++ b/rdst_amd/_lib.py
@@ -11,7 +11,8 @@
 _SIDE_HEADERS = {"DATA": os.path.join(_INCLUDE, "rdst_hip_data.h"),
                  "LRC": os.path.join(_INCLUDE, "rdst_hip_consistency.h"),
                  "MSSSIM": os.path.join(_INCLUDE, "rdst_hip_msssim.h"),
-                 "NOISE": os.path.join(_INCLUDE, "rdst_hip_noise.h")}
+                 "NOISE": os.path.join(_INCLUDE, "rdst_hip_noise.h"),
+                 "FOLD": os.path.join(_INCLUDE, "rdst_hip_fold.h")}
 
 _SCALARS = {"int": C.c_int, "int64_t": C.c_int64, "float": C.c_float, "double": C.c_double, "size_t": C.c_size_t}
 _FIELD_SCALARS = {**_SCALARS, "int32_t": C.c_int32}
diff --git a/rdst_amd/build.py b/rdst_amd/build.py
--- a/rdst_amd/build.py
+++ b/rdst_amd/build.py
@@ -29,7 +29,7 @@
     srcs = sorted(f for f in os.listdir(CSRC) if f.endswith(".hip"))
     hdrs = [os.path.join(CSRC, f) for f in os.listdir(CSRC) if f.endswith(".h")]
     hdrs += [os.path.join(os.path.dirname(HERE), "include", h) for h in ("rdst_hip.h", "rdst_hip_data.h", "rdst_hip_consistency.h",
-                                                                            "rdst_hip_msssim.h", "rdst_hip_noise.h")]
+                                                                            "rdst_hip_msssim.h", "rdst_hip_noise.h", "rdst_hip_fold.h")]
     jobs = []
     objs = []
     for s in srcs:
diff --git a/rdst_amd/csrc/l1_loss.hip b/rdst_amd/csrc/l1_loss.hip
--- /dev/null
+++ b/rdst_amd/csrc/l1_loss.hip
@@ -0,0 +1,93 @@
+#include "common.h"
+#include "../../include/rdst_hip_fold.h"
+
+namespace {
+
+constexpr int kL1Threads = 256, kL1MaxBlocks = 1024;
+
+int l1_blocks(int64_t n) {
+  const int64_t nv = (n + 3) / 4, b = (nv + kL1Threads - 1) / kL1Threads;
+  return (int)(b < kL1MaxBlocks ? b : kL1MaxBlocks);
+}
+
+__device__ __forceinline__ double l1_block_sum(double a, double* sh) {
+#pragma unroll
+  for (int m = 32; m >= 1; m >>= 1) a += __shfl_xor(a, m, 64);
+  if ((threadIdx.x & 63) == 0) sh[threadIdx.x >> 6] = a;
+  __syncthreads();
+  return sh[0] + sh[1] + sh[2] + sh[3];
+}
+
+template <bool VEC>
+__global__ void __launch_bounds__(kL1Threads) l1_loss_kernel(const float* __restrict__ y, const float* __restrict__ t, int64_t n,
+                                                             float inv_n, float* __restrict__ grad, double* __restrict__ part) {
+  __shared__ double sh[4];
+  const int64_t nv = (n + 3) / 4, stride = (int64_t)gridDim.x * kL1Threads;
+  double acc = 0.0;
+  for (int64_t v = (int64_t)blockIdx.x * kL1Threads + threadIdx.x; v < nv; v += stride) {
+    const int64_t i0 = 4 * v;
+    float a[4], b[4], g[4];
+    const bool whole = i0 + 4 <= n;
+    if (VEC && whole) {
+      const float4 ya = *reinterpret_cast<const float4*>(y + i0), tb = *reinterpret_cast<const float4*>(t + i0);
+      a[0] = ya.x; a[1] = ya.y; a[2] = ya.z; a[3] = ya.w;
+      b[0] = tb.x; b[1] = tb.y; b[2] = tb.z; b[3] = tb.w;
+    } else {
+#pragma unroll
+      for (int e = 0; e < 4; ++e) {
+        const bool in = i0 + e < n;
+        a[e] = in ? y[i0 + e] : 0.f;
+        b[e] = in ? t[i0 + e] : 0.f;
+      }
+    }
+#pragma unroll
+    for (int e = 0; e < 4; ++e) {
+      const float d = a[e] - b[e];
+      acc += (double)fabsf(d);
+      g[e] = inv_n * (float)((d > 0.f) - (d < 0.f));
+    }
+    if (grad) {
+      if (VEC && whole) {
+        *reinterpret_cast<float4*>(grad + i0) = make_float4(g[0], g[1], g[2], g[3]);
+      } else {
+#pragma unroll
+        for (int e = 0; e < 4; ++e)
+          if (i0 + e < n) grad[i0 + e] = g[e];
+      }
+    }
+  }
+  const double s = l1_block_sum(acc, sh);
+  if (threadIdx.x == 0) part[blockIdx.x] = s;
+}
+
+__global__ void __launch_bounds__(kL1Threads) l1_loss_finish_kernel(const double* __restrict__ part, int nparts, int64_t n,
+                                                                    float* __restrict__ loss) {
+  __shared__ double sh[4];
+  double acc = 0.0;
+  for (int k = threadIdx.x; k < nparts; k += kL1Threads) acc += part[k];
+  const double s = l1_block_sum(acc, sh);
+  if (threadIdx.x == 0) *loss = (float)(s / (double)n);
+}
+
+}
+
+extern "C" size_t rdst_l1_loss_workspace(int64_t n) { return n > 0 ? (size_t)l1_blocks(n) * sizeof(double) : 0; }
+
+extern "C" int rdst_l1_loss(const float* y, const float* target, int64_t n, float* grad, float* loss, void* workspace,
+                            size_t workspace_bytes, void* stream) {
+  if (!y || !target || !loss || !workspace || n <= 0) return rdst_fail(RDST_EINVAL, "rdst_l1_loss: bad arguments");
+  if (((uintptr_t)workspace & 7) || workspace_bytes < rdst_l1_loss_workspace(n))
+    return rdst_fail(RDST_EINVAL, "rdst_l1_loss: workspace too small or misaligned");
+  if (((uintptr_t)y & 3) || ((uintptr_t)target & 3) || ((uintptr_t)grad & 3) || ((uintptr_t)loss & 3))
+    return rdst_fail(RDST_EINVAL, "rdst_l1_loss: misaligned pointer");
+  hipStream_t st = (hipStream_t)stream;
+  const int blocks = l1_blocks(n);
+  const float inv_n = 1.0f / (float)n;
+  double* part = (double*)workspace;
+  const bool vec = !(((uintptr_t)y | (uintptr_t)target | (uintptr_t)grad) & 15);
+  if (vec) hipLaunchKernelGGL(l1_loss_kernel<true>, dim3(blocks), dim3(kL1Threads), 0, st, y, target, n, inv_n, grad, part);
+  else hipLaunchKernelGGL(l1_loss_kernel<false>, dim3(blocks), dim3(kL1Threads), 0, st, y, target, n, inv_n, grad, part);
+  if (int rc = rdst_launch_status("l1_loss")) return rc;
+  hipLaunchKernelGGL(l1_loss_finish_kernel, dim3(1), dim3(kL1Threads), 0, st, part, blocks, n, loss);
+  return rdst_launch_status("l1_loss_finish");
+}
diff --git a/rdst_amd/csrc/linear.h b/rdst_amd/csrc/linear.h
--- a/rdst_amd/csrc/linear.h
+++ b/rdst_amd/csrc/linear.h
@@ -57,10 +57,12 @@
 int linear_ln_bwd_fused_bf16(const bf16* X, int64_t ldx, const float* ln_w, const float* ln_b, const float* stats,
                              const float* Wt, const bf16* dY, int64_t lddy, bf16* dX, int64_t lddx, const bf16* acc,
                              int64_t ldacc, float* dW, float* dbias, float* dln_w, float* dln_b, const WsSlab& slab, float* G,
-                             int64_t M, int K, int N, float s, hipStream_t st, const bf16* acc2 = nullptr, int64_t ldacc2 = 0);
+                             int64_t M, int K, int N, float s, hipStream_t st, const bf16* acc2 = nullptr, int64_t ldacc2 = 0,
+                             const bf16* acc3 = nullptr, int64_t ldacc3 = 0);
 int lnlin3_bwd_bf16(const bf16* X, int64_t ldx, const float* ln_w, const float* stats, const float* Wt, const bf16* dY,
                     int64_t lddy, bf16* dX, int64_t lddx, const bf16* acc, int64_t ldacc, const bf16* acc2, int64_t ldacc2,
-                    const WsSlab& slab, int64_t slab_stride, int64_t M, int K, int N, int* grid_out, hipStream_t st);
+                    const WsSlab& slab, int64_t slab_stride, int64_t M, int K, int N, int* grid_out, hipStream_t st,
+                    const bf16* acc3 = nullptr, int64_t ldacc3 = 0);
 
 size_t lin3_pack_bytes(int K, int N);
 int lin3_kind(int K, int N, bool ln, bool res, int in_act);
diff --git a/rdst_amd/csrc/linear.hip b/rdst_amd/csrc/linear.hip
--- a/rdst_amd/csrc/linear.hip
+++ b/rdst_amd/csrc/linear.hip
@@ -2,6 +2,7 @@
 #include "gemm_valu.h"
 #include "linear.h"
 #include "pack.h"
+#include "../../include/rdst_hip_fold.h"
 
 __global__ void __launch_bounds__(256) slab_reduce_kernel(const float* __restrict__ slab, float* __restrict__ out,
                                                           int S, int64_t n) {
@@ -195,7 +196,7 @@
 __global__ void __launch_bounds__(256) ln8_bwd_kernel(const T* __restrict__ dY, int64_t lddy, const T* __restrict__ X, int64_t ldx,
                                                       const float* __restrict__ stats, const float* __restrict__ gamma, T* dX,
                                                       int64_t lddx, const T* acc, int64_t ldacc, float* __restrict__ slab, int64_t M,
-                                                      int K, float s) {
+                                                      int K, float s, const T* acc3 = nullptr, int64_t ldacc3 = 0) {
   __shared__ float red[4][2][64];
   const int lane = threadIdx.x & 63, wave = threadIdx.x >> 6, ps = lane >> 3, grp = lane & 7;
   const Ln8Lane l = ln8_lane(grp, K);
@@ -233,6 +234,12 @@
         ln8_load<T>(acc + row * ldacc + l.c0, a);
 #pragma unroll
         for (int e = 0; e < 8; ++e) o[e] += a[e];
+      }
+      if (acc3) {
+        float a[8];
+        ln8_load<T>(acc3 + row * ldacc3 + l.c0, a);
+#pragma unroll
+        for (int e = 0; e < 8; ++e) o[e] = to_f32<T>(from_f32<T>(o[e])) + a[e];
       }
       ln8_store(dX + row * lddx, o, l);
     }
@@ -431,11 +438,20 @@
 int bwd_t(const T* X, int64_t ldx, const float* ln_w, const float* ln_b, const float* stats, int in_act, const float* Wt,
           const T* dY, int64_t lddy, T* dX, int64_t lddx, const T* acc, int64_t ldacc, float* dW, float* dbias,
           float* dln_w,
-          float* dln_b, float* wsp, int64_t M, int K, int N, float s, bool split, hipStream_t st, const T* acc2, int64_t ldacc2) {
+          float* dln_b, float* wsp, int64_t M, int K, int N, float s, bool split, hipStream_t st, const T* acc2, int64_t ldacc2,
+          const T* acc3 = nullptr, int64_t ldacc3 = 0) {
   const LinBwdWs w = lin_bwd_layout(wsp, M, K, N, ln_w != nullptr, true);
   float* const dA = w.dA;
   const WsSlab& slabW = w.slabW;
   const WsSlab& small = w.small;
+  if (acc3) {
+    if constexpr (sizeof(T) == 2) {
+      if (Wt && ln_w && ln_b && dW && dbias && dln_w && dln_b && dX && K <= 128 && w.G)
+        return linear_ln_bwd_fused_bf16(X, ldx, ln_w, ln_b, stats, Wt, dY, lddy, dX, lddx, acc, ldacc, dW, dbias, dln_w, dln_b, slabW,
+                                        w.G, M, K, N, s, st, acc2, ldacc2, acc3, ldacc3);
+    }
+    return RDST_ENOTSUP;
+  }
   if constexpr (sizeof(T) == 4) {
     if (split && Wt && dX && dW && dbias && (!ln_w || (dln_w && dln_b && w.G)) && !rdst_dbg_getenv("RDST_LBX_OFF")) {
       const int rc = lnlin3x_bwd_f32(X, ldx, ln_w, ln_b, stats, in_act, Wt, dY, lddy, dX, lddx, acc, ldacc, acc2, ldacc2, dW, dbias, dln_w,
@@ -563,16 +579,19 @@
 template <typename T>
 int ln_only_bwd(const T* X, int64_t ldx, const float* ln_w, const float* stats, const T* dY, int64_t lddy, T* dX,
                 int64_t lddx, const T* acc, int64_t ldacc, float* dln_w, float* dln_b, float* wsp, int64_t M, int K, float s,
-                hipStream_t st) {
+                hipStream_t st, const T* acc3 = nullptr, int64_t ldacc3 = 0) {
   const LinBwdWs w = lin_bwd_layout(wsp, M, K, K, true, false);
   float* const dA = w.dA;
   const WsSlab& small = w.small;
   const int64_t n = M * K;
-  if (K <= 64 && ln8_ok(X, ldx, dY, lddy, dX, lddx, K, (int)sizeof(T)) && ln8_ok(acc, ldacc, nullptr, 0, nullptr, 0, K, (int)sizeof(T))) {
+  const bool rows8 = K <= 64 && ln8_ok(X, ldx, dY, lddy, dX, lddx, K, (int)sizeof(T)) && ln8_ok(acc, ldacc, acc3, ldacc3, nullptr, 0, K, (int)sizeof(T));
+  if (acc3 && !(rows8 && dX)) return RDST_ENOTSUP;
+  if (rows8) {
     const int64_t nb = (M + 31) / 32;
     const int blocks = (int)small.cap(nb < kSmallBlocks ? nb : kSmallBlocks, 2 * K);
     if (int rc = rdst_slab_fits(small, blocks, 2 * K, "ln8_bwd")) return rc;
-    hipLaunchKernelGGL((ln8_bwd_kernel<T>), dim3(blocks), dim3(256), 0, st, dY, lddy, X, ldx, stats, ln_w, dX, lddx, acc, ldacc, small.p, M, K, s);
+    hipLaunchKernelGGL((ln8_bwd_kernel<T>), dim3(blocks), dim3(256), 0, st, dY, lddy, X, ldx, stats, ln_w, dX, lddx, acc, ldacc, small.p, M, K, s,
+                       acc3, ldacc3);
     if (int rc = rdst_launch_status("ln8_bwd")) return rc;
     return slab_reduce2(small.p, dln_w, dln_b, blocks, K, st);
   }
@@ -646,10 +665,16 @@
 }
 
 namespace {
+bool small_launches_off() {
+  static int off = -1;
+  if (off < 0) { const char* e = rdst_dbg_getenv("RDST_RES_ADD3"); off = (e && atoi(e) == 0) ? 1 : 0; }
+  return off != 0;
+}
 int ln_linear_bwd(const void* X, int64_t ld_x, const float* ln_w, const float* ln_b, const float* stats, int in_act, const float* Wt,
                   const void* dY, int64_t ld_dy, void* dX, int64_t ld_dx, const void* dX_add, int64_t ld_dx_add, float* dW, float* dbias,
                   float* dln_w, float* dln_b, void* workspace, size_t workspace_bytes, int64_t M, int K, int N, float out_scale,
-                  int dtype, bool split, hipStream_t st, const void* dX_add2, int64_t ld_dx_add2) {
+                  int dtype, bool split, hipStream_t st, const void* dX_add2, int64_t ld_dx_add2, const void* dX_add3 = nullptr,
+                  int64_t ld_dx_add3 = 0) {
   if (!X || !dY || !workspace) return rdst_fail(RDST_EINVAL, "rdst_ln_linear_bwd: null pointer");
   if (M < 0 || K <= 0 || N <= 0) return rdst_fail(RDST_EINVAL, "rdst_ln_linear_bwd: bad dimensions");
   if (ln_w && !stats) return rdst_fail(RDST_EINVAL, "rdst_ln_linear_bwd: LayerNorm needs the forward's stats");
@@ -659,17 +684,31 @@
   if (M == 0) return 0;
   float* wsp = (float*)workspace;
   if (dX_add2 && (!Wt || (dtype != RDST_BF16 && !(split && lnlin3x_bwd_kind(K, N, ln_w != nullptr, in_act))))) return RDST_ENOTSUP;
+  if (dX_add3 && (dtype != RDST_BF16 || !dX || ld_dx_add3 < K || small_launches_off())) return RDST_ENOTSUP;
   if (!Wt) {
     if (dtype == RDST_F32)
       return ln_only_bwd<float>((const float*)X, ld_x, ln_w, stats, (const float*)dY, ld_dy, (float*)dX, ld_dx, (const float*)dX_add, ld_dx_add, dln_w, dln_b, wsp, M, K, out_scale, st);
-    return ln_only_bwd<bf16>((const bf16*)X, ld_x, ln_w, stats, (const bf16*)dY, ld_dy, (bf16*)dX, ld_dx, (const bf16*)dX_add, ld_dx_add, dln_w, dln_b, wsp, M, K, out_scale, st);
+    return ln_only_bwd<bf16>((const bf16*)X, ld_x, ln_w, stats, (const bf16*)dY, ld_dy, (bf16*)dX, ld_dx, (const bf16*)dX_add, ld_dx_add, dln_w, dln_b, wsp, M, K, out_scale, st,
+                             (const bf16*)dX_add3, ld_dx_add3);
   }
   if (dtype == RDST_F32)
     return bwd_t<float>((const float*)X, ld_x, ln_w, ln_b, stats, in_act, Wt, (const float*)dY, ld_dy, (float*)dX, ld_dx, (const float*)dX_add, ld_dx_add, dW, dbias, dln_w, dln_b, wsp, M, K, N, out_scale, split, st,
                       (const float*)dX_add2, ld_dx_add2);
   return bwd_t<bf16>((const bf16*)X, ld_x, ln_w, ln_b, stats, in_act, Wt, (const bf16*)dY, ld_dy, (bf16*)dX, ld_dx, (const bf16*)dX_add, ld_dx_add, dW, dbias, dln_w, dln_b, wsp, M, K, N, out_scale, false, st,
-                     (const bf16*)dX_add2, ld_dx_add2);
-}
+                     (const bf16*)dX_add2, ld_dx_add2, (const bf16*)dX_add3, ld_dx_add3);
+}
+}
+
+extern "C" int rdst_ln_linear_bwd3(const void* X, int64_t ld_x, const float* ln_w, const float* ln_b, const float* stats,
+                                  int in_act, const float* Wt, const void* dY, int64_t ld_dy, void* dX, int64_t ld_dx,
+                                  const void* dX_add, int64_t ld_dx_add, float* dW, float* dbias, float* dln_w, float* dln_b,
+                                  void* workspace,
+                                  size_t workspace_bytes, int64_t M, int K, int N, float out_scale, int dtype,
+                                  void* stream, const void* dX_add2, int64_t ld_dx_add2, const void* dX_add3, int64_t ld_dx_add3) {
+  bool split;
+  if (int rc = rdst_dtype(dtype, split, "rdst_ln_linear_bwd")) return rc;
+  return ln_linear_bwd(X, ld_x, ln_w, ln_b, stats, in_act, Wt, dY, ld_dy, dX, ld_dx, dX_add, ld_dx_add, dW, dbias, dln_w, dln_b, workspace,
+                       workspace_bytes, M, K, N, out_scale, dtype, split, (hipStream_t)stream, dX_add2, ld_dx_add2, dX_add3, ld_dx_add3);
 }
 
 extern "C" int rdst_ln_linear_bwd2(const void* X, int64_t ld_x, const float* ln_w, const float* ln_b, const float* stats,
diff --git a/rdst_amd/csrc/lnlin3_mfma.hip b/rdst_amd/csrc/lnlin3_mfma.hip
--- a/rdst_amd/csrc/lnlin3_mfma.hip
+++ b/rdst_amd/csrc/lnlin3_mfma.hip
@@ -26,6 +26,7 @@
   const bf16* X; int64_t ldx; const float* stats; const float* lnw; const float* W;
   const bf16* dY; int64_t lddy; bf16* dX; int64_t lddx; const bf16* Acc; int64_t ldacc;
   const bf16* Acc2; int64_t ldacc2;
+  const bf16* Acc3; int64_t ldacc3;
   float* slab; int64_t slab_stride;
   int64_t M; int64_t ntiles; int tiles_per_wg;
 };
@@ -144,7 +145,7 @@
   }
 };
 
-template <int K, int N, bool LN>
+template <int K, int N, bool LN, bool A3 = false>
 __global__ void __launch_bounds__((LB3<K, N>::NT), (LB3<K, N>::WPS)) lnlin3_bwd_kernel(const LB3Args p) {
   extern __shared__ __attribute__((aligned(16))) char smem[];
   using CF = LB3<K, N>;
@@ -264,6 +265,7 @@
   float* red = reinterpret_cast<float*>(smem + CF::OFF_RED);
   f32x16 dx;
   u32x2_t xs[4], as[4];
+  u32x4_a4 a3[A3 ? 2 : 1];
   float rstd = 0.f;
   int64_t prow = -1;
   auto finish = [&](int pb) {
@@ -296,6 +298,17 @@
           c8[4 + e] = __uint_as_float(sw[1]);
         }
         const int cb = 32 * dct + 8 * (2 * gp2 + hh);
+        if constexpr (A3) {
+          static_assert(!A3 || K % 8 == 0 || K % 8 == 4, "the row's last chunk is loaded 4 channels early");
+          const bool late = cb + 8 > K;
+          const uint32_t w[4] = {late ? a3[gp2].z : a3[gp2].x, late ? a3[gp2].w : a3[gp2].y, a3[gp2].z, a3[gp2].w};
+#pragma unroll
+          for (int e = 0; e < 4; ++e) {
+            const uint32_t pk = pack_bf16x2(c8[2 * e], c8[2 * e + 1]);
+            c8[2 * e] = bf16lo(pk) + bf16lo(w[e]);
+            c8[2 * e + 1] = bf16hi(pk) + bf16hi(w[e]);
+          }
+        }
         if (cb + 8 <= K) {
           u32x4_a4 u;
           u.x = pack_bf16x2(c8[0], c8[1]); u.y = pack_bf16x2(c8[2], c8[3]);
@@ -353,6 +366,15 @@
       as[g4] = *reinterpret_cast<const LDS_AS u32x2_t*>(xrow + CF::OFF_AC + 16 * g4);
     }
     prow = tile * 32 + r;
+    if constexpr (A3) {
+      const int64_t arow = prow < p.M ? prow : p.M - 1;
+#pragma unroll
+      for (int gp2 = 0; gp2 < 2; ++gp2) {
+        int cb = 32 * dct + 8 * (2 * gp2 + hh);
+        cb = cb + 8 <= K ? cb : K - 8;
+        a3[gp2] = *reinterpret_cast<const u32x4_a4*>(p.Acc3 + arow * p.ldacc3 + cb);
+      }
+    }
     if (LN) {
       rstd = reinterpret_cast<const float*>(buf + CF::OFF_SM)[r];
       float s1 = 0.f, s2 = 0.f;
@@ -382,10 +404,10 @@
   }
 }
 
-template <int K, int N, bool LN>
+template <int K, int N, bool LN, bool A3 = false>
 int lb3_launch(LB3Args& p, const WsSlab& slab, int* grid_out, hipStream_t st) {
   using CF = LB3<K, N>;
-  auto kern = lnlin3_bwd_kernel<K, N, LN>;
+  auto kern = lnlin3_bwd_kernel<K, N, LN, A3>;
   static int percu_env = -1;
   if (percu_env < 0) { const char* e = rdst_dbg_getenv("RDST_LB3_PERCU"); percu_env = e ? atoi(e) : 0; }
   int per_cu = CF::PERCU;
@@ -400,7 +422,8 @@
 
 int lnlin3_bwd_bf16(const bf16* X, int64_t ldx, const float* ln_w, const float* stats, const float* Wt, const bf16* dY,
                     int64_t lddy, bf16* dX, int64_t lddx, const bf16* acc, int64_t ldacc, const bf16* acc2, int64_t ldacc2,
-                    const WsSlab& slab, int64_t slab_stride, int64_t M, int K, int N, int* grid_out, hipStream_t st) {
+                    const WsSlab& slab, int64_t slab_stride, int64_t M, int K, int N, int* grid_out, hipStream_t st,
+                    const bf16* acc3, int64_t ldacc3) {
   static int off = -1;
   if (off < 0) { const char* e = rdst_dbg_getenv("RDST_LB3_OFF"); off = e ? atoi(e) : 0; }
   if (off) return RDST_ENOTSUP;
@@ -409,6 +432,11 @@
   p.X = X; p.ldx = ldx; p.stats = stats; p.lnw = ln_w; p.W = Wt; p.dY = dY; p.lddy = lddy; p.dX = dX; p.lddx = lddx;
   p.Acc = acc; p.ldacc = ldacc; p.Acc2 = acc2; p.ldacc2 = ldacc2; p.slab = slab.p; p.slab_stride = slab_stride; p.M = M;
   p.ntiles = (M + 31) / 32;
+  if (acc3) {
+    if (!(K == 60 && N == 180 && ln) || ((uintptr_t)acc3 & 3) || (ldacc3 & 1) || ldacc3 < K) return RDST_ENOTSUP;
+    p.Acc3 = acc3; p.ldacc3 = ldacc3;
+    return lb3_launch<60, 180, true, true>(p, slab, grid_out, st);
+  }
 #define RDST_LB3(KK, NN, LL) if (K == KK && N == NN && ln == LL) return lb3_launch<KK, NN, LL>(p, slab, grid_out, st);
   RDST_LB3(60, 180, true) RDST_LB3(90, 270, true) RDST_LB3(120, 360, true)
   RDST_LB3(60, 30, true) RDST_LB3(90, 30, true) RDST_LB3(120, 30, true)
diff --git a/rdst_amd/csrc/lnlin_mfma.hip b/rdst_amd/csrc/lnlin_mfma.hip
--- a/rdst_amd/csrc/lnlin_mfma.hip
+++ b/rdst_amd/csrc/lnlin_mfma.hip
@@ -342,7 +342,8 @@
 int linear_ln_bwd_fused_bf16(const bf16* X, int64_t ldx, const float* ln_w, const float* ln_b, const float* stats,
                              const float* Wt, const bf16* dY, int64_t lddy, bf16* dX, int64_t lddx, const bf16* acc,
                              int64_t ldacc, float* dW, float* dbias, float* dln_w, float* dln_b, const WsSlab& slab, float* G,
-                             int64_t M, int K, int N, float s, hipStream_t st, const bf16* acc2, int64_t ldacc2) {
+                             int64_t M, int K, int N, float s, hipStream_t st, const bf16* acc2, int64_t ldacc2, const bf16* acc3,
+                             int64_t ldacc3) {
   static int off = -1;
   if (off < 0) { const char* e = rdst_dbg_getenv("RDST_LNLIN_V1"); off = e ? atoi(e) : 0; }
   const bool ln = ln_w != nullptr;
@@ -366,9 +367,9 @@
     int g3 = 0;
     if (acc2 && (((uintptr_t)acc2 & 3) || (ldacc2 & 1) || (uint64_t)M * (uint64_t)ldacc2 * 2 >= (1ull << 31))) return RDST_ENOTSUP;
     const int rc3 = lnlin3_bwd_bf16(X, ldx, ln_w, stats, Wt, dY, lddy, dX, lddx, acc, ldacc, acc2, ldacc2, slab, slab_stride, M, K,
-                                    N, &g3, st);
+                                    N, &g3, st, acc3, ldacc3);
     if (rc3 == 0) return lnlin_bwd_reduce(slab.p, g3, slab_stride, ln, Wt, ln_w, ln_b, dW, dbias, dln_w, dln_b, G, N, K, st);
-    if (rc3 != RDST_ENOTSUP || acc2) return rc3;
+    if (rc3 != RDST_ENOTSUP || acc2 || acc3) return rc3;
   }
   const int CP = 32 * nct, LDW = nct == 4 ? 288 : CP * 2 + 16, LDX = nct == 4 ? 336 : CP * 2 + 16, NP = 32 * NW, LDY = lnlin_ldy(NP);
   const int smem = NP * LDW + 2 * 32 * LDX + 32 * LDY + 128 + nct * 32 * 8;
diff --git a/rdst_amd/fold.py b/rdst_amd/fold.py
--- /dev/null
+++ b/rdst_amd/fold.py
@@ -0,0 +1,54 @@
+from __future__ import annotations
+
+import os
+
+import torch
+
+from . import _lib
+
+RES_SINK = os.environ.get("RDST_RES_SINK", "1") != "0"
+L1_FUSED = os.environ.get("RDST_L1_FUSED", "1") != "0"
+
+
+class ResSink:
+
+    def __init__(self):
+        self.res = None
+
+    def take_res(self):
+        r, self.res = self.res, None
+        return r
+
+
+def ln_linear_bwd3(lib, args, dx_add2, ld_add2, dx_add3, ld_add3):
+    rc = lib.rdst_ln_linear_bwd3(*args, None if dx_add2 is None else dx_add2.data_ptr(), ld_add2, dx_add3.data_ptr(), ld_add3)
+    if rc == _lib.ENOTSUP:
+        return False
+    _lib.check(rc, "rdst_ln_linear_bwd3")
+    return True
+
+
+def l1_loss_usable(y: torch.Tensor, target: torch.Tensor) -> bool:
+    return (L1_FUSED and y.is_cuda and target.is_cuda and y.dtype == torch.float32 and target.dtype == torch.float32
+            and y.shape == target.shape and y.numel() > 0 and y.is_contiguous() and target.is_contiguous())
+
+
+def l1_loss(y: torch.Tensor, target: torch.Tensor, loss_out: torch.Tensor, workspace: torch.Tensor = None) -> torch.Tensor:
+    if not l1_loss_usable(y, target):
+        raise ValueError("rdst_amd.fold.l1_loss: fp32 contiguous device tensors of one shape")
+    if loss_out.dtype != torch.float32 or loss_out.numel() != 1 or loss_out.device != y.device:
+        raise ValueError("rdst_amd.fold.l1_loss: loss_out must be one fp32 element on y's device")
+    lib = _lib.load()
+    n = y.numel()
+    nbytes = lib.rdst_l1_loss_workspace(n)
+    if workspace is None or workspace.numel() * workspace.element_size() < nbytes:
+        workspace = torch.empty((nbytes + 7) // 8, dtype=torch.float64, device=y.device)
+    grad = torch.empty_like(y)
+    _lib.check(lib.rdst_l1_loss(y.data_ptr(), target.data_ptr(), n, grad.data_ptr(), loss_out.data_ptr(), workspace.data_ptr(),
+                                workspace.numel() * workspace.element_size(), torch.cuda.current_stream().cuda_stream),
+               "rdst_l1_loss")
+    return grad
+
+
+def l1_loss_workspace(n: int, device) -> torch.Tensor:
+    return torch.empty((_lib.load().rdst_l1_loss_workspace(n) + 7) // 8, dtype=torch.float64, device=device)
diff --git a/rdst_amd/networks/common.py b/rdst_amd/networks/common.py
--- a/rdst_amd/networks/common.py
+++ b/rdst_amd/networks/common.py
@@ -10,13 +10,13 @@
 
 class Conv2d(nn.Conv2d):
 
-    def forward_rows(self, x, *, in_act=ops.ACT_NONE, residual=None, out_scale=1.0, shuffle=1, out_slot=None):
+    def forward_rows(self, x, *, in_act=ops.ACT_NONE, residual=None, out_scale=1.0, shuffle=1, out_slot=None, res_sink=None):
         k = self.kernel_size[0]
         if (self.kernel_size[0] != self.kernel_size[1] or k not in (1, 3) or self.stride != (1, 1)
                 or self.padding != (k // 2, k // 2) or self.dilation != (1, 1) or self.groups != 1):
             raise NotImplementedError("rdst_amd Conv2d: only k in {1,3}, stride 1, padding k//2, groups 1")
         return ops.conv_rows(x, self.weight, self.bias, in_act=in_act, residual=residual, out_scale=out_scale,
-                             shuffle=shuffle, out_slot=out_slot)
+                             shuffle=shuffle, out_slot=out_slot, res_sink=res_sink)
 
     def forward(self, x):
         return ops.rows_to_nchw(self.forward_rows(ops.nchw_to_rows(x, torch.float32)))
diff --git a/rdst_amd/networks/rdst_variations.py b/rdst_amd/networks/rdst_variations.py
--- a/rdst_amd/networks/rdst_variations.py
+++ b/rdst_amd/networks/rdst_variations.py
@@ -3,7 +3,7 @@
 import torch
 import torch.nn as nn
 
-from .. import ops
+from .. import fold, ops
 from .common import Conv2d, MeanShift, UpSampler, default_conv
 from .swin_transformer_sr import (BasicLayer, Mlp, PatchEmbed, PatchUnEmbed, SwinTransformerBlock,
                                   WindowAttention, _drop_p, _ln_params, _norm_only, trunc_normal_, window_partition,
@@ -84,8 +84,9 @@
     def forward(self, x, x_size):
         return torch.cat((x, self.new_features(x, x_size)), 2)
 
-    def forward_dense(self, x, x_size, buf):
-        sink = self._grad_sink(x)
+    def forward_dense(self, x, x_size, buf, sink=None):
+        if sink is None:
+            sink = self._grad_sink(x)
         if not _slot_ok(self.tail):
             new = self.new_features(x, x_size, sink=sink)
             buf.fill(x.shape[-1], new)
@@ -106,12 +107,13 @@
     return None
 
 
-def _apply_res_connection(conv, x, residual=None, out_scale=1.0, out_slot=None):
+def _apply_res_connection(conv, x, residual=None, out_scale=1.0, out_slot=None, res_sink=None):
     if isinstance(conv, Conv2d):
-        return conv.forward_rows(x, residual=residual, out_scale=out_scale, out_slot=out_slot)
+        return conv.forward_rows(x, residual=residual, out_scale=out_scale, out_slot=out_slot, res_sink=res_sink)
     y = conv[0].forward_rows(x)
     y = conv[2].forward_rows(y, in_act=ops.ACT_LEAKY02)
-    return conv[4].forward_rows(y, in_act=ops.ACT_LEAKY02, residual=residual, out_scale=out_scale, out_slot=out_slot)
+    return conv[4].forward_rows(y, in_act=ops.ACT_LEAKY02, residual=residual, out_scale=out_scale, out_slot=out_slot,
+                                res_sink=res_sink)
 
 
 class RDSTB(nn.Module):
@@ -154,18 +156,21 @@
     def forward(self, x, x_size, buf=None, out_slot=None):
         B, L, C = x.shape
         H, W = x_size
+        rsink = None
         if x.is_cuda and len(self.body) > 0:
             if buf is None:
                 buf = self.make_buffer(B, L, x.dtype, x.device)
             y = ops.into_dense(x, buf)
-            for m in self.body:
-                y = m.forward_dense(y, x_size, buf)
+            if fold.RES_SINK and x.dtype == torch.bfloat16 and x.requires_grad and hasattr(self, "conv"):
+                rsink = self.body[0]._grad_sink(y)
+            for i, m in enumerate(self.body):
+                y = m.forward_dense(y, x_size, buf, sink=rsink if i == 0 else None)
         else:
             y = x
             for m in self.body:
                 y = m(y, x_size)
         out = _apply_res_connection(self.conv, y.view(B, H, W, y.shape[-1]), residual=x.view(B, H, W, C),
-                                    out_scale=self.residual_scale, out_slot=out_slot)
+                                    out_scale=self.residual_scale, out_slot=out_slot, res_sink=rsink)
         return out.view(B, L, C)
 
 
@@ -305,7 +310,7 @@
         self.compute_dtype, self.compute_code = ops.resolve_compute_dtype(dtype)
         return self
 
-    def forward_features_rows(self, feat):
+    def forward_features_rows(self, feat, res_sink=None):
         B, H, W, E = feat.shape
         x_size = (H, W)
         t = feat.view(B, H * W, E)
@@ -316,7 +321,9 @@
         pos_drop = self.training and self.pos_drop.p > 0.
         if self.patch_embed.norm is not None:
             first = (bufs[0], 0) if (chain and not self.ape and not pos_drop and isinstance(self.patch_embed.norm, nn.LayerNorm)) else None
-            t = _norm_only(t, self.patch_embed.norm, out_slot=first)
+            t = _norm_only(t, self.patch_embed.norm, out_slot=first, res_sink=res_sink)
+        elif res_sink is not None:
+            raise ValueError("RDSTSR.forward_features_rows: a residual sink needs the patch norm")
         if self.ape:
             t = t + self.absolute_pos_embed.to(t.dtype)
         if pos_drop:
@@ -344,10 +351,15 @@
         rows = self.sub_mean.forward_rows(rows)
         feat = self.head.forward_rows(rows)
         B, H, W, E = feat.shape
-        t = self.forward_features_rows(feat)
+        pn = self.patch_embed.norm
+        gsink = None
+        if (fold.RES_SINK and self.feature_last_operation and feat.is_cuda and feat.dtype == torch.bfloat16 and feat.requires_grad
+                and torch.is_grad_enabled() and isinstance(pn, nn.LayerNorm) and pn.weight is not None):
+            gsink = fold.ResSink()
+        t = self.forward_features_rows(feat, res_sink=gsink)
         if self.feature_last_operation:
             t = _norm_only(t, self.norm, out_scale=self.global_res_scale)
-            res = _apply_res_connection(self.conv_after_body, t.view(B, H, W, E), residual=feat)
+            res = _apply_res_connection(self.conv_after_body, t.view(B, H, W, E), residual=feat, res_sink=gsink)
         else:
             res = _norm_only(t, self.norm, out_scale=self.global_res_scale, residual=feat.view(B, H * W, E))
             res = res.view(B, H, W, E)
diff --git a/rdst_amd/networks/swin_transformer_sr.py b/rdst_amd/networks/swin_transformer_sr.py
--- a/rdst_amd/networks/swin_transformer_sr.py
+++ b/rdst_amd/networks/swin_transformer_sr.py
@@ -55,15 +55,17 @@
     raise NotImplementedError(f"rdst_amd: norm layer {type(norm).__name__} (nn.LayerNorm or nn.Identity)")
 
 
-def _norm_only(x, norm, out_scale=1.0, residual=None, out_slot=None):
+def _norm_only(x, norm, out_scale=1.0, residual=None, out_slot=None, res_sink=None):
     w, b = _ln_params(norm)
     if w is None:
         y = x if out_scale == 1.0 else x * out_scale
         y = y if residual is None else y + residual
         if out_slot is not None:
             raise NotImplementedError("rdst_amd: dense slot without a LayerNorm")
+        if res_sink is not None:
+            raise NotImplementedError("rdst_amd: residual sink without a LayerNorm")
         return y
-    return ops.ln_linear(x, w, b, None, None, out_scale=out_scale, residual=residual, out_slot=out_slot)
+    return ops.ln_linear(x, w, b, None, None, out_scale=out_scale, residual=residual, out_slot=out_slot, res_sink=res_sink)
 
 
 class Mlp(nn.Module):
diff --git a/rdst_amd/ops.py b/rdst_amd/ops.py
--- a/rdst_amd/ops.py
+++ b/rdst_amd/ops.py
@@ -8,7 +8,7 @@
 
 import torch
 
-from . import _lib, side
+from . import _lib, fold, side
 from ._lib import ACT_GELU, ACT_LEAKY001, ACT_LEAKY02, ACT_NONE, BF16, F32, F32X3
 
 
@@ -375,7 +375,9 @@
 
 
 def _linear_bwd_call(lib, x, ldx, lw, lb, stats, in_act, w, dy, lddy, dx, lddx, dx_add, ld_add, dw, db, dlw, dlb,
-                     M, K, N, out_scale, code, dev, keep=None, dx_add2=None, ld_add2=0):
+                     M, K, N, out_scale, code, dev, keep=None, dx_add2=None, ld_add2=0, dx_add3=None, ld_add3=0):
+    if dx is None:
+        dx_add3 = None
     if all(t is None for t in (dx, dlw, dlb, dw, db)):
         return
     nbytes = lib.rdst_ln_linear_bwd_workspace(M, K, N)
@@ -385,14 +387,20 @@
     args = (x.data_ptr(), ldx, _ptr(lw), _ptr(lb), _ptr(stats), in_act, _ptr(w), dy.data_ptr(), lddy, _ptr(dx), lddx,
             _ptr(dx_add), ld_add, _ptr(dw), _ptr(db), _ptr(dlw), _ptr(dlb), wsp.data_ptr(), nbytes, M, K, N, out_scale, code,
             _stream())
+    if dx_add3 is not None and fold.ln_linear_bwd3(lib, args, dx_add2 if dx is not None else None, ld_add2, dx_add3, ld_add3):
+        return
+    done = False
     if dx_add2 is not None and dx is not None:
         rc = lib.rdst_ln_linear_bwd2(*args, dx_add2.data_ptr(), ld_add2)
         if rc != _lib.ENOTSUP:
             _lib.check(rc, "rdst_ln_linear_bwd2")
-            return
-    _lib.check(lib.rdst_ln_linear_bwd(*args), "rdst_ln_linear_bwd")
-    if dx_add2 is not None and dx is not None:
-        dx.add_(dx_add2)
+            done = True
+    if not done:
+        _lib.check(lib.rdst_ln_linear_bwd(*args), "rdst_ln_linear_bwd")
+        if dx_add2 is not None and dx is not None:
+            dx.add_(dx_add2)
+    if dx_add3 is not None:
+        dx.add_(dx_add3.reshape(dx.shape))
 
 
 def _ln_linear_fwd(lib, x, ldx, lw, lb, in_act, w, b, res, ldr, y, ldy, stats, M, K, N, out_scale, code):
@@ -412,7 +420,8 @@
 
 class _LnLinear(torch.autograd.Function):
     @staticmethod
-    def forward(ctx, x, ln_w, ln_b, weight, bias, residual, in_act, out_scale, out_slot=None):
+    def forward(ctx, x, ln_w, ln_b, weight, bias, residual, in_act, out_scale, out_slot=None, res_sink=None):
+        ctx.res_sink = res_sink
         _need_gpu(x, ln_w, ln_b, weight, bias, residual)
         lib = _lib.load()
         K = x.shape[-1]
@@ -454,11 +463,13 @@
         dlb = _grad_like(lb) if (lb is not None and need[2]) else None
         dw = _grad_like(w) if (w is not None and need[3]) else None
         db = _bias_grad(ctx, need[4])
+        res3, ld3 = _sunk_rows(ctx.res_sink, need[0])
         _linear_bwd_call(lib, x, ldx, lw, lb, stats, in_act, w, dy_r, lddy, dx, K, None, 0, dw, db, dlw, dlb, M, K, N,
-                         out_scale, code, dev, keep=_ReduceBatch.keep if _ReduceBatch.depth > 0 else None)
+                         out_scale, code, dev, keep=_ReduceBatch.keep if _ReduceBatch.depth > 0 else None, dx_add3=res3,
+                         ld_add3=ld3)
         _ReduceBatch.settle(lib)
         dres = dy if (has_res and need[5]) else None
-        return dx, dlw, dlb, dw, db, dres, None, None, None
+        return dx, dlw, dlb, dw, db, dres, None, None, None, None
 
 
 class DenseBuffer:
@@ -577,9 +588,17 @@
     side.reset()
 
 
-class GradSink:
+def _sunk_rows(sink, wanted):
+    res = sink.take_res() if sink is not None else None
+    if res is None or not wanted:
+        return None, 0
+    return _rows(res)
+
+
+class GradSink(fold.ResSink):
 
     def __init__(self):
+        super().__init__()
         self.extra = None
         self.batch_open = False
 
@@ -624,8 +643,8 @@
 
 def ln_linear(x: torch.Tensor, ln_w: Optional[torch.Tensor], ln_b: Optional[torch.Tensor],
               weight: Optional[torch.Tensor], bias: Optional[torch.Tensor], *, in_act: int = ACT_NONE,
-              residual: Optional[torch.Tensor] = None, out_scale: float = 1.0, out_slot=None) -> torch.Tensor:
-    return _LnLinear.apply(x, ln_w, ln_b, weight, bias, residual, in_act, out_scale, out_slot)
+              residual: Optional[torch.Tensor] = None, out_scale: float = 1.0, out_slot=None, res_sink=None) -> torch.Tensor:
+    return _LnLinear.apply(x, ln_w, ln_b, weight, bias, residual, in_act, out_scale, out_slot, res_sink)
 
 
 class _SwinBlock(torch.autograd.Function):
@@ -785,9 +804,12 @@
             keep.append(extra)
         else:
             extra, ld_extra = None, 0
+        res3, ld3 = _sunk_rows(ctx.sink, need[0])
+        if res3 is not None:
+            keep.append(res3)
         _linear_bwd_call(lib, x, ldx, n1w, n1b, stats1, ACT_NONE, qkvw, dqkv, 3 * C, dx, C, dx1 if need[0] else None, C,
                          dqkvw, dqkvb, dn1w, dn1b, M, C, 3 * C, 1.0, code, dev, keep=keep, dx_add2=extra,
-                         ld_add2=ld_extra)
+                         ld_add2=ld_extra, dx_add3=res3, ld_add3=ld3)
         if not need[5]:
             dtab = None
         return (dx, dn1w, dn1b, dqkvw, dqkvb, dtab, dprojw, dprojb, dn2w, dn2b, dfc1w, dfc1b, dfc2w, dfc2b,
@@ -802,7 +824,8 @@
 
 class _ConvRows(torch.autograd.Function):
     @staticmethod
-    def forward(ctx, x, weight, bias, residual, in_act, out_scale, shuffle, out_slot=None):
+    def forward(ctx, x, weight, bias, residual, in_act, out_scale, shuffle, out_slot=None, res_sink=None):
+        ctx.res_sink = res_sink if residual is not None else None
         _need_gpu(x, weight, bias, residual)
         lib = _lib.load()
         if x.dim() != 4:
@@ -864,12 +887,15 @@
                 side.join()
         _ReduceBatch.settle(lib)
         dres = dy if (has_res and need[3]) else None
-        return dx, dw, db, dres, None, None, None, None
+        if dres is not None and ctx.res_sink is not None:
+            ctx.res_sink.res, dres = dres, None
+        return dx, dw, db, dres, None, None, None, None, None
 
 
 def conv_rows(x: torch.Tensor, weight: torch.Tensor, bias: Optional[torch.Tensor], *, in_act: int = ACT_NONE,
-              residual: Optional[torch.Tensor] = None, out_scale: float = 1.0, shuffle: int = 1, out_slot=None) -> torch.Tensor:
-    return _ConvRows.apply(x, weight, bias, residual, in_act, out_scale, shuffle, out_slot)
+              residual: Optional[torch.Tensor] = None, out_scale: float = 1.0, shuffle: int = 1, out_slot=None,
+              res_sink=None) -> torch.Tensor:
+    return _ConvRows.apply(x, weight, bias, residual, in_act, out_scale, shuffle, out_slot, res_sink)
 
 
 class _NchwToRows(torch.autograd.Function):
diff --git a/rdst_amd/trainer.py b/rdst_amd/trainer.py
--- a/rdst_amd/trainer.py
+++ b/rdst_amd/trainer.py
@@ -9,7 +9,7 @@
 import torch.distributed as dist
 import torch.nn.functional as F
 
-from . import dp, side
+from . import dp, fold, side
 from .optim import FlatAdam
 
 GUARD_OFF = 1e8
@@ -58,6 +58,7 @@
         self._static = None
         self._eager_seen = 0
         self._loss_buf = None
+        self._plain_l1, self._l1_ws = loss_fn is None, None
         self.capture_hook = None
         self.training_loss_names = ["L1"] if loss_fn is None else list(getattr(loss_fn, "loss_components", ["loss"]))
         self.training_loss_records: Dict[str, list] = {n: [] for n in self.training_loss_names}
@@ -132,13 +133,19 @@
         self._refuse_averaged("fwd_bwd")
         self.bucket.detach_grads()
         out = self.net(inputs)
-        loss = self._loss(out, targets)
         if self._loss_buf is None:
             self._loss_buf = torch.zeros((), dtype=torch.float32, device=inputs.device)
-        self._loss_buf.copy_(loss.detach())
+        fused_l1 = self._plain_l1 and fold.l1_loss_usable(out, targets)
+        if fused_l1:
+            if self._l1_ws is None or self._l1_ws[0] != out.numel():
+                self._l1_ws = (out.numel(), fold.l1_loss_workspace(out.numel(), out.device))
+            root, grad = out, fold.l1_loss(out.detach(), targets, self._loss_buf, self._l1_ws[1])
+        else:
+            root, grad = self._loss(out, targets), None
+            self._loss_buf.copy_(root.detach())
         side.enable()
         try:
-            loss.backward()
+            root.backward(grad)
         finally:
             try:
                 side.join()
```

Measured after the change: 1868 patches/s (median of 6 runs). About the same (+0.5%).
